# Rickyeeeeee/ParallelRayTracing

Hardware: AMD Instinct MI355X
Metric: Mrays/sec at 1920x1080, 4 bounces, ~1M-tri scene (higher is better)
Workload: dtype f32; 1 GPU; C3: dragon.ply refined by longest-edge bisection = 870000 triangles + ground quad + emissive quad, 1920x1080, max_depth 5 segments (= 4 bounces), 256 spp per step (15360 spp timed of the config's 256), image tiled over 1 GPU(s) + per-step gather to rank 0; triangles=870000, bvh_nodes=681504, bvh_max_depth=25, bvh8_nodes=137301, bvh8_depth=9, width=1920, height=1080, max_depth=5, samples_in_flight=256, seed=0, jitter=0, variant=0, gather=render stream

## Files before the change

include/prt.h:

```cpp
#ifndef PRT_H
#define PRT_H

#include <stddef.h>
#include <stdint.h>

#ifdef __cplusplus
extern "C" {
#endif

#define PRT_VERSION 1

enum {
    PRT_OK = 0,
    PRT_ERR_INVALID = 1,
    PRT_ERR_NO_DEVICE = 2,
    PRT_ERR_HIP = 3,
    PRT_ERR_IO = 4,
    PRT_ERR_NOMEM = 5
};

enum { PRT_SHAPE_CIRCLE = 0, PRT_SHAPE_QUAD = 1, PRT_SHAPE_TRIANGLE = 2 };
enum { PRT_MAT_NONE = 0, PRT_MAT_LAMBERTIAN = 1, PRT_MAT_METAL = 2, PRT_MAT_DIELECTRIC = 3, PRT_MAT_EMISSIVE = 4 };
enum {
    PRT_PRESET_DEFAULT = 0, PRT_PRESET_LIGHT_TEST = 1, PRT_PRESET_MATERIAL_TEST = 2, PRT_PRESET_CORNELL = 3,
// ... 205 lines not shown
} PrtInstanceUpdateInfo;
int prt_instance_update_info(PrtContext* ctx, PrtInstanceUpdateInfo* out);
int prt_instances_read(PrtContext* ctx, uint32_t capacity, uint32_t* n_instances, uint32_t* slot_instance, uint32_t* root,
                       uint32_t* slot_base, uint32_t* prim_base);
int prt_set_camera(PrtContext* ctx, const PrtCameraDesc* cam);
int prt_set_film(PrtContext* ctx, uint32_t width, uint32_t height, uint32_t rank, uint32_t world_size);
int prt_film_clear(PrtContext* ctx);

int prt_render(PrtContext* ctx, uint32_t spp, uint32_t max_depth, uint32_t seed, uint32_t first_sample);
int prt_render_async(PrtContext* ctx, uint32_t spp, uint32_t max_depth, uint32_t seed, uint32_t first_sample);
int prt_synchronize(PrtContext* ctx);
int prt_set_sampling(PrtContext* ctx, const PrtSampling* sampling);
int prt_set_lens(PrtContext* ctx, const PrtLens* lens);
int prt_get_lens(PrtContext* ctx, PrtLens* out);
int prt_set_samples_in_flight(PrtContext* ctx, uint32_t n);
int prt_set_lighting(PrtContext* ctx, const PrtLighting* l);
int prt_get_light_stats(PrtContext* ctx, PrtLightStats* out);
int prt_set_light_sources(PrtContext* ctx, uint32_t mask);
int prt_set_environment(PrtContext* ctx, const PrtEnvironment* env);
int prt_environment_info(PrtContext* ctx, PrtEnvironmentInfo* out);
int prt_environment_intervals(PrtContext* ctx, uint64_t* row_width, uint64_t* col_width);
int prt_environment_eval(PrtContext* ctx, uint32_t n, const float* dirs, float* rgb, uint32_t* texel, float* pdf_w);
int prt_set_textures(PrtContext* ctx, const PrtTextureSet* set);
int prt_texture_info(PrtContext* ctx, PrtTextureInfo* out);
int prt_texture_eval(PrtContext* ctx, uint32_t n, const uint32_t* texture, const float* uv, float* rgb);
int prt_hit_uv(PrtContext* ctx, uint32_t n, const float* origins, const float* dirs, PrtHit* hits, float* uv, float* albedo);
int prt_light_intervals(PrtContext* ctx, uint32_t capacity, uint32_t* n_lights, uint64_t* width);
int prt_light_info(PrtContext* ctx, uint32_t capacity, uint32_t* n_lights, uint32_t* prim, float* pmf);
int prt_sample_light(PrtContext* ctx, uint32_t n, const float* in_dirs, const PrtHit* hits, const uint32_t* keys,
                     float* shadow_dirs, float* tmax, uint32_t* light, float* contrib, float* pdf_light, float* pdf_bsdf,
                     float* w_light, float* w_bsdf);

typedef struct PrtAdaptive {
    uint32_t min_spp, step_spp, max_spp;
    float threshold, noise_floor;
} PrtAdaptive;
typedef struct PrtAdaptiveInfo {
    uint32_t passes;
    uint32_t tiles_local;
    uint32_t tiles_converged;
    uint32_t tiles_capped;
    uint32_t min_tile_spp;
    uint32_t max_tile_spp;
    uint64_t pixel_samples;
} PrtAdaptiveInfo;
int prt_set_film_statistics(PrtContext* ctx, int on);
int prt_get_film_statistics(const PrtContext* ctx);
int prt_film_statistics_read(PrtContext* ctx, float* sum_y, float* sum_y2);
int prt_film_noise_read(PrtContext* ctx, float noise_floor, float* rel_err);
int prt_adaptive_unconverged(float n, float A, float Q, float threshold, float noise_floor);
int prt_render_adaptive(PrtContext* ctx, const PrtAdaptive* cfg, uint32_t max_depth, uint32_t seed, uint32_t first_sample,
                        PrtAdaptiveInfo* out );

int prt_film_read(PrtContext* ctx, float* rgb_sum, float* weight);
int prt_film_local(PrtContext* ctx, void** d_ptr, uint64_t* n_floats);
int prt_film_resolve(PrtContext* ctx, const void* d_gathered, uint32_t world_size, void* d_rgb_sum, void* d_weight);
int prt_film_resolve_on(PrtContext* ctx, void* hip_stream, const void* d_gathered, uint32_t world_size, void* d_rgb_sum,
                        void* d_weight);
int prt_film_tonemap(PrtContext* ctx, const void* d_rgb_sum, const void* d_weight, float exposure, float gamma, void* d_rgba8);
int prt_film_display(PrtContext* ctx, float exposure, float gamma, uint8_t* rgba8);

int prt_camera_rays(PrtContext* ctx, uint32_t n, const float* px, const float* py, float* origins, float* dirs);
int prt_camera_rays_lens(PrtContext* ctx, uint32_t n, const float* px, const float* py, uint32_t* keys, float* origins,
                         float* dirs);
int prt_closest_hit(PrtContext* ctx, uint32_t n, const float* origins, const float* dirs, PrtHit* hits);
int prt_closest_hit_device(PrtContext* ctx, uint32_t n, const void* d_origins, const void* d_dirs, void* d_hits);
int prt_occluded(PrtContext* ctx, uint32_t n, const float* origins, const float* dirs, const float* tmax,
                 uint8_t* occluded);
int prt_occluded_device(PrtContext* ctx, uint32_t n, const void* d_origins, const void* d_dirs, const void* d_tmax,
                        void* d_occluded);
int prt_scatter(PrtContext* ctx, uint32_t n, const float* in_dirs, const PrtHit* hits, uint32_t* rng_state,
                uint32_t* scattered, float* attenuation, float* emitted, float* out_origins, float* out_dirs);

int prt_enable_timing(PrtContext* ctx, int on);
int prt_get_stats(PrtContext* ctx, PrtStats* out);
int prt_reset_stats(PrtContext* ctx);
int prt_measure_traversal(PrtContext* ctx, uint32_t max_depth, uint32_t seed, uint32_t sample, PrtStats* out);
int prt_measure_shade_divergence(PrtContext* ctx, uint32_t max_depth, uint32_t seed, uint32_t sample, uint64_t* out);
int prt_bvh_info(PrtContext* ctx, PrtBvhInfo* out);
uint32_t prt_spill_rows(uint32_t max_stack4, uint32_t max_depth);
int prt_kernel_occupancy(PrtContext* ctx, PrtOccupancy* out);
int prt_kernel_instance(PrtContext* ctx, char* name, uint32_t capacity);
int prt_shade_instance(PrtContext* ctx, char* name, uint32_t capacity);
int prt_bvh_read(PrtContext* ctx, float* nodes, float* tris);
int prt_bvh_read4(PrtContext* ctx, float* nodes4);
int prt_bvh_read8(PrtContext* ctx, uint32_t* nodes8);
int prt_set_variant(PrtContext* ctx, int variant);
int prt_set_param(PrtContext* ctx, const char* name, int value);

typedef struct PrtGroup PrtGroup;
int prt_group_create(const int* device_ids, uint32_t n, PrtGroup** out);
void prt_group_destroy(PrtGroup* g);
const char* prt_group_last_error(const PrtGroup* g);
uint32_t prt_group_size(const PrtGroup* g);
const char* prt_group_transport(const PrtGroup* g);
PrtContext* prt_group_context(PrtGroup* g, uint32_t rank);
int prt_group_set_scene(PrtGroup* g, const PrtSceneDesc* scene);
int prt_group_refit_meshes(PrtGroup* g, const PrtMesh* meshes, uint32_t n_meshes);
int prt_group_set_instance_transforms(PrtGroup* g, const PrtInstance* instances, uint32_t n, uint32_t mode);
int prt_group_set_camera(PrtGroup* g, const PrtCameraDesc* cam);
int prt_group_set_film(PrtGroup* g, uint32_t width, uint32_t height);
int prt_group_film_clear(PrtGroup* g);
int prt_group_set_sampling(PrtGroup* g, const PrtSampling* s);
int prt_group_set_lens(PrtGroup* g, const PrtLens* lens);
int prt_group_set_samples_in_flight(PrtGroup* g, uint32_t n);
int prt_group_set_lighting(PrtGroup* g, const PrtLighting* l);
int prt_group_set_light_sources(PrtGroup* g, uint32_t mask);
int prt_group_set_environment(PrtGroup* g, const PrtEnvironment* env);
int prt_group_set_textures(PrtGroup* g, const PrtTextureSet* set);
int prt_group_get_light_stats(PrtGroup* g, PrtLightStats* out);
int prt_group_set_param(PrtGroup* g, const char* name, int value);
int prt_group_render(PrtGroup* g, uint32_t spp, uint32_t max_depth, uint32_t seed, uint32_t first_sample);
int prt_group_set_film_statistics(PrtGroup* g, int on);
int prt_group_render_adaptive(PrtGroup* g, const PrtAdaptive* cfg, uint32_t max_depth, uint32_t seed, uint32_t first_sample,
                              PrtAdaptiveInfo* out);
int prt_group_film_read(PrtGroup* g, float* rgb_sum, float* weight);
int prt_group_film_display(PrtGroup* g, float exposure, float gamma, uint8_t* rgba8);
int prt_group_get_stats(PrtGroup* g, PrtStats* out);

typedef struct PrtMeshData PrtMeshData;
int prt_mesh_load_ply(const char* path, PrtMeshData** out, char* err, size_t err_len);
int prt_mesh_create(const float* positions, const float* normals, uint32_t n_vertices, const uint32_t* indices,
                    uint32_t n_triangles, PrtMeshData** out);
void prt_mesh_free(PrtMeshData* m);
uint32_t prt_mesh_vertex_count(const PrtMeshData* m);
uint32_t prt_mesh_triangle_count(const PrtMeshData* m);
const float* prt_mesh_positions(const PrtMeshData* m);
const float* prt_mesh_normals(const PrtMeshData* m);
const uint32_t* prt_mesh_indices(const PrtMeshData* m);
int prt_mesh_had_normals(const PrtMeshData* m);
int prt_mesh_refine(PrtMeshData* m, uint32_t target_triangles);
int prt_mesh_transform(PrtMeshData* m, const float mat[16], const float inv[16]);
int prt_mesh_append(PrtMeshData* dst, const PrtMeshData* src);
const float* prt_mesh_uvs(const PrtMeshData* m);
int prt_mesh_had_uvs(const PrtMeshData* m);
int prt_mesh_set_uvs(PrtMeshData* m, const float* uvs);

int prt_scene_preset(int preset, PrtMaterial* materials, uint32_t* n_materials, PrtPrimitive* primitives,
                     uint32_t* n_primitives);
void prt_make_transform(const float scale[3], const float euler_deg[3], const float translation[3], float mat[16],
                        float inv[16]);

int prt_write_ppm(const char* path, const uint8_t* rgba8, uint32_t width, uint32_t height);
int prt_write_pfm(const char* path, const float* rgb, uint32_t width, uint32_t height);
int prt_read_pfm(const char* path, float** rgb, uint32_t* width, uint32_t* height);
void prt_image_free(float* rgb);

#ifdef __cplusplus
}
#endif
#endif
```

parallelraytracing_amd/capi.py:

```python
from __future__ import annotations

import ctypes as C
import os

_HERE = os.path.dirname(os.path.abspath(__file__))
LIB_PATH = os.environ.get("PRT_LIB_PATH") or os.path.join(_HERE, "csrc", "libprt.so")

PRT_MAX_DEPTH = 64

SHAPE_CIRCLE, SHAPE_QUAD, SHAPE_TRIANGLE = 0, 1, 2
MAT_NONE, MAT_LAMBERTIAN, MAT_METAL, MAT_DIELECTRIC, MAT_EMISSIVE = 0, 1, 2, 3, 4
(PRESET_DEFAULT, PRESET_LIGHT_TEST, PRESET_MATERIAL_TEST, PRESET_CORNELL, PRESET_RANDOM_BALLS_SMALL,
 PRESET_RANDOM_BALLS_MEDIUM, PRESET_RANDOM_BALLS_LARGE) = range(7)
PRESET_NAMES = {
    "DEFAULT": PRESET_DEFAULT, "LIGHT_TEST": PRESET_LIGHT_TEST, "MATERIAL_TEST": PRESET_MATERIAL_TEST,
    "CORNELL": PRESET_CORNELL, "RANDOM_BALLS_SMALL": PRESET_RANDOM_BALLS_SMALL,
    "RANDOM_BALLS_MEDIUM": PRESET_RANDOM_BALLS_MEDIUM, "RANDOM_BALLS_LARGE": PRESET_RANDOM_BALLS_LARGE,
}


class PrtMaterial(C.Structure):
    _fields_ = [("type", C.c_uint32), ("rgb", C.c_float * 3), ("scalar", C.c_float)]


# ... 144 lines not shown
    "prt_group_create": (C.c_int, [C.POINTER(C.c_int), C.c_uint32, C.POINTER(_vp)]),
    "prt_group_destroy": (None, [_vp]),
    "prt_group_last_error": (C.c_char_p, [_vp]),
    "prt_group_size": (C.c_uint32, [_vp]),
    "prt_group_transport": (C.c_char_p, [_vp]),
    "prt_group_context": (_vp, [_vp, C.c_uint32]),
    "prt_group_set_scene": (C.c_int, [_vp, C.POINTER(PrtSceneDesc)]),
    "prt_group_refit_meshes": (C.c_int, [_vp, C.POINTER(PrtMesh), C.c_uint32]),
    "prt_group_set_camera": (C.c_int, [_vp, C.POINTER(PrtCameraDesc)]),
    "prt_group_set_film": (C.c_int, [_vp, C.c_uint32, C.c_uint32]),
    "prt_group_film_clear": (C.c_int, [_vp]),
    "prt_group_set_sampling": (C.c_int, [_vp, C.POINTER(PrtSampling)]),
    "prt_group_set_samples_in_flight": (C.c_int, [_vp, C.c_uint32]),
    "prt_group_set_lens": (C.c_int, [_vp, C.POINTER(PrtLens)]),
    "prt_set_lens": (C.c_int, [_vp, C.POINTER(PrtLens)]),
    "prt_get_lens": (C.c_int, [_vp, C.POINTER(PrtLens)]),
    "prt_camera_rays_lens": (C.c_int, [_vp, C.c_uint32, _fp, _fp, _u32p, _fp, _fp]),
    "prt_group_set_param": (C.c_int, [_vp, C.c_char_p, C.c_int]),
    "prt_group_render": (C.c_int, [_vp, C.c_uint32, C.c_uint32, C.c_uint32, C.c_uint32]),
    "prt_group_film_read": (C.c_int, [_vp, _fp, _fp]),
    "prt_group_film_display": (C.c_int, [_vp, C.c_float, C.c_float, C.POINTER(C.c_uint8)]),
    "prt_group_get_stats": (C.c_int, [_vp, C.POINTER(PrtStats)]),
    "prt_group_set_lighting": (C.c_int, [_vp, C.POINTER(PrtLighting)]),
    "prt_group_get_light_stats": (C.c_int, [_vp, C.POINTER(PrtLightStats)]),
    "prt_group_set_light_sources": (C.c_int, [_vp, C.c_uint32]),
    "prt_set_light_sources": (C.c_int, [_vp, C.c_uint32]),
    "prt_light_intervals": (C.c_int, [_vp, C.c_uint32, _u32p, C.POINTER(C.c_uint64)]),
    "prt_set_environment": (C.c_int, [_vp, C.POINTER(PrtEnvironment)]),
    "prt_group_set_environment": (C.c_int, [_vp, C.POINTER(PrtEnvironment)]),
    "prt_environment_info": (C.c_int, [_vp, C.POINTER(PrtEnvironmentInfo)]),
    "prt_environment_intervals": (C.c_int, [_vp, C.POINTER(C.c_uint64), C.POINTER(C.c_uint64)]),
    "prt_environment_eval": (C.c_int, [_vp, C.c_uint32, _fp, _fp, _u32p, _fp]),
    "prt_set_textures": (C.c_int, [_vp, C.POINTER(PrtTextureSet)]),
    "prt_group_set_textures": (C.c_int, [_vp, C.POINTER(PrtTextureSet)]),
    "prt_texture_info": (C.c_int, [_vp, C.POINTER(PrtTextureInfo)]),
    "prt_texture_eval": (C.c_int, [_vp, C.c_uint32, _u32p, _fp, _fp]),
    "prt_hit_uv": (C.c_int, [_vp, C.c_uint32, _fp, _fp, C.POINTER(PrtHit), _fp, _fp]),
    "prt_mesh_uvs": (_fp, [_vp]),
    "prt_mesh_had_uvs": (C.c_int, [_vp]),
    "prt_mesh_set_uvs": (C.c_int, [_vp, _fp]),
    "prt_read_pfm": (C.c_int, [C.c_char_p, C.POINTER(_fp), _u32p, _u32p]),
    "prt_image_free": (None, [_fp]),
    "prt_set_film_statistics": (C.c_int, [_vp, C.c_int]),
    "prt_get_film_statistics": (C.c_int, [_vp]),
    "prt_film_statistics_read": (C.c_int, [_vp, _fp, _fp]),
    "prt_film_noise_read": (C.c_int, [_vp, C.c_float, _fp]),
    "prt_adaptive_unconverged": (C.c_int, [C.c_float, C.c_float, C.c_float, C.c_float, C.c_float]),
    "prt_render_adaptive": (C.c_int, [_vp, C.POINTER(PrtAdaptive), C.c_uint32, C.c_uint32, C.c_uint32, C.POINTER(PrtAdaptiveInfo)]),
    "prt_group_set_film_statistics": (C.c_int, [_vp, C.c_int]),
    "prt_group_render_adaptive": (C.c_int, [_vp, C.POINTER(PrtAdaptive), C.c_uint32, C.c_uint32, C.c_uint32, C.POINTER(PrtAdaptiveInfo)]),
    "prt_set_lighting": (C.c_int, [_vp, C.POINTER(PrtLighting)]),
    "prt_get_light_stats": (C.c_int, [_vp, C.POINTER(PrtLightStats)]),
    "prt_light_info": (C.c_int, [_vp, C.c_uint32, _u32p, _u32p, _fp]),
    "prt_sample_light": (C.c_int, [_vp, C.c_uint32, _fp, C.POINTER(PrtHit), _u32p, _fp, _fp, _u32p, _fp, _fp, _fp, _fp, _fp]),
    "prt_set_scene": (C.c_int, [_vp, C.POINTER(PrtSceneDesc)]),
    "prt_set_camera": (C.c_int, [_vp, C.POINTER(PrtCameraDesc)]),
    "prt_set_film": (C.c_int, [_vp, C.c_uint32, C.c_uint32, C.c_uint32, C.c_uint32]),
    "prt_film_clear": (C.c_int, [_vp]),
    "prt_render": (C.c_int, [_vp, C.c_uint32, C.c_uint32, C.c_uint32, C.c_uint32]),
    "prt_render_async": (C.c_int, [_vp, C.c_uint32, C.c_uint32, C.c_uint32, C.c_uint32]),
    "prt_synchronize": (C.c_int, [_vp]),
    "prt_set_samples_in_flight": (C.c_int, [_vp, C.c_uint32]),
    "prt_film_read": (C.c_int, [_vp, _fp, _fp]),
    "prt_film_local": (C.c_int, [_vp, C.POINTER(_vp), C.POINTER(C.c_uint64)]),
    "prt_film_resolve": (C.c_int, [_vp, _vp, C.c_uint32, _vp, _vp]),
    "prt_film_resolve_on": (C.c_int, [_vp, _vp, _vp, C.c_uint32, _vp, _vp]),
    "prt_film_tonemap": (C.c_int, [_vp, _vp, _vp, C.c_float, C.c_float, _vp]),
    "prt_film_display": (C.c_int, [_vp, C.c_float, C.c_float, C.POINTER(C.c_uint8)]),
    "prt_camera_rays": (C.c_int, [_vp, C.c_uint32, _fp, _fp, _fp, _fp]),
    "prt_closest_hit": (C.c_int, [_vp, C.c_uint32, _fp, _fp, C.POINTER(PrtHit)]),
    "prt_closest_hit_device": (C.c_int, [_vp, C.c_uint32, _vp, _vp, _vp]),
    "prt_occluded": (C.c_int, [_vp, C.c_uint32, _fp, _fp, _fp, C.POINTER(C.c_uint8)]),
    "prt_occluded_device": (C.c_int, [_vp, C.c_uint32, _vp, _vp, _vp, _vp]),
    "prt_scatter": (C.c_int, [_vp, C.c_uint32, _fp, C.POINTER(PrtHit), _u32p, _u32p, _fp, _fp, _fp, _fp]),
    "prt_enable_timing": (C.c_int, [_vp, C.c_int]),
    "prt_get_stats": (C.c_int, [_vp, C.POINTER(PrtStats)]),
    "prt_reset_stats": (C.c_int, [_vp]),
    "prt_measure_traversal": (C.c_int, [_vp, C.c_uint32, C.c_uint32, C.c_uint32, C.POINTER(PrtStats)]),
    "prt_bvh_info": (C.c_int, [_vp, C.POINTER(PrtBvhInfo)]),
    "prt_spill_rows": (C.c_uint32, [C.c_uint32, C.c_uint32]),
    "prt_kernel_occupancy": (C.c_int, [_vp, C.POINTER(PrtOccupancy)]),
    "prt_kernel_instance": (C.c_int, [_vp, C.c_char_p, C.c_uint32]),
    "prt_shade_instance": (C.c_int, [_vp, C.c_char_p, C.c_uint32]),
    "prt_measure_shade_divergence": (C.c_int, [_vp, C.c_uint32, C.c_uint32, C.c_uint32, C.POINTER(C.c_uint64)]),
    "prt_refit_meshes": (C.c_int, [_vp, C.POINTER(PrtMesh), C.c_uint32]),
    "prt_set_instance_transforms": (C.c_int, [_vp, C.POINTER(PrtInstance), C.c_uint32, C.c_uint32]),
    "prt_group_set_instance_transforms": (C.c_int, [_vp, C.POINTER(PrtInstance), C.c_uint32, C.c_uint32]),
    "prt_instance_update_info": (C.c_int, [_vp, C.POINTER(PrtInstanceUpdateInfo)]),
    "prt_instances_read": (C.c_int, [_vp, C.c_uint32, _u32p, _u32p, _u32p, _u32p, _u32p]),
    "prt_bvh_read": (C.c_int, [_vp, _fp, _fp]),
    "prt_set_sampling": (C.c_int, [_vp, C.POINTER(PrtSampling)]),
    "prt_bvh_read4": (C.c_int, [_vp, _fp]),
    "prt_bvh_read8": (C.c_int, [_vp, C.POINTER(C.c_uint32)]),
    "prt_set_variant": (C.c_int, [_vp, C.c_int]),
    "prt_set_param": (C.c_int, [_vp, C.c_char_p, C.c_int]),
    "prt_mesh_load_ply": (C.c_int, [C.c_char_p, C.POINTER(_vp), C.c_char_p, C.c_size_t]),
    "prt_mesh_create": (C.c_int, [_fp, _fp, C.c_uint32, _u32p, C.c_uint32, C.POINTER(_vp)]),
    "prt_mesh_free": (None, [_vp]),
    "prt_mesh_vertex_count": (C.c_uint32, [_vp]),
    "prt_mesh_triangle_count": (C.c_uint32, [_vp]),
    "prt_mesh_positions": (_fp, [_vp]),
    "prt_mesh_normals": (_fp, [_vp]),
    "prt_mesh_indices": (_u32p, [_vp]),
    "prt_mesh_had_normals": (C.c_int, [_vp]),
    "prt_mesh_refine": (C.c_int, [_vp, C.c_uint32]),
    "prt_mesh_transform": (C.c_int, [_vp, _fp, _fp]),
    "prt_mesh_append": (C.c_int, [_vp, _vp]),
    "prt_scene_preset": (C.c_int, [C.c_int, C.POINTER(PrtMaterial), _u32p, C.POINTER(PrtPrimitive), _u32p]),
    "prt_make_transform": (None, [_fp, _fp, _fp, _fp, _fp]),
    "prt_write_ppm": (C.c_int, [C.c_char_p, C.POINTER(C.c_uint8), C.c_uint32, C.c_uint32]),
    "prt_write_pfm": (C.c_int, [C.c_char_p, _fp, C.c_uint32, C.c_uint32]),
}


def load(path: str = LIB_PATH) -> C.CDLL:
    if not os.path.exists(path):
        raise ImportError(
            f"{path} is missing: the HIP extension is the product and has no fallback. "
            "Build it with `python -c 'import __graft_entry__ as g; g.build()'` "
            "(or `make -C parallelraytracing_amd/csrc`).")
    try:
        import torch
    except Exception:
        pass
    lib = C.CDLL(path)
    for name, (res, args) in SIGNATURES.items():
        fn = getattr(lib, name)
        fn.restype = res
        fn.argtypes = args
    return lib


_lib = None


def lib() -> C.CDLL:
    global _lib
    if _lib is None:
        _lib = load()
    return _lib
```

parallelraytracing_amd/csrc/prt_api.cpp:

```cpp
#include <hip/hip_runtime.h>

#include <algorithm>
#include <cfloat>
#include <chrono>
#include <cmath>
#include <cstdarg>
#include <cstdio>
#include <cstdlib>
#include <cstring>
#include <limits>
#include <string>
#include <utility>
#include <vector>

#include "../../include/prt.h"
#include "bvh.h"
#include "bvh_gpu.h"
#include "prt_adaptive.h"
#include "prt_kernels.h"
#include "prt_scene.h"

namespace {

constexpr float kPadCoeff = 1.0f / 262144.0f;
constexpr size_t kRayStatWords = (size_t)PRT_RAY_STAT_SLOTS * PRT_MAX_DEPTH;
constexpr uint32_t kTravStatsWords = 16 + PRT_TIMELINE_WORDS * (PRT_MAX_DEPTH + 1);
constexpr size_t kLightStatWords = 2 * (size_t)PRT_RAY_STAT_SLOTS;

struct EventPair {
    hipEvent_t a, b;
    int kind;
};

}

struct PrtContext {
    int device = -1;
    bool has_device = false;
    hipStream_t own_stream = nullptr;
    hipStream_t stream = nullptr;
    std::string err;

    bool has_scene = false;
    PrtHostScene hs;
    double refit_ms = 0.0;
    PrtInstanceUpdateInfo inst_info{};
    DevScene dsc{};
    void* d_prims = nullptr;
    void* d_mat_rgbs = nullptr;
    void* d_mat_type = nullptr;
    void* d_nodes = nullptr;
    void* d_nodes4 = nullptr;
    void* d_nodes8 = nullptr;
    void* d_insts = nullptr;
    void* d_tlas_inst = nullptr;
    void* d_abvh_nodes = nullptr;
    void* d_abvh_order = nullptr;
    void* d_tris = nullptr;
    void* d_nrms = nullptr;

    bool has_camera = false;
    DevCamera cam{};

    bool has_film = false;
    PrtTileMap tm{};
    uint32_t valid_local = 0;
    float4* d_film_local = nullptr;
    bool film_stats = false;
    float2* d_film_stat = nullptr;
    uint32_t* d_tile_sel = nullptr;
    uint32_t tile_sel_entries = 0;
    uint32_t* h_tile_count = nullptr;

    uint32_t S = 1;
    uint64_t cap_paths = 0;
    PrtRayBuf rb[2] = {{nullptr, nullptr, nullptr, nullptr, nullptr}, {nullptr, nullptr, nullptr, nullptr, nullptr}};
    float4* d_rad = nullptr;
    uint32_t* d_counts = nullptr;
    unsigned long long* d_ray_stats = nullptr;
    unsigned long long* ray_stats_target = nullptr;
    bool pix_records_blank = false;
    uint32_t* h_flag = nullptr;
    unsigned long long* d_trav_stats = nullptr;

    void* d_scratch = nullptr;
    size_t scratch_bytes = 0;

    bool timing = false;
    std::vector<EventPair> events;
    std::vector<EventPair> event_pool;
    PrtStats stats{};
    uint64_t dead_paths = 0;
    int variant = 0;
    int abvh_enabled = 1;
    int measure_spp = 1;
    float pad_coeff = kPadCoeff;
    int node_stride = 0;
    int compact_primary = 1;
    int primary_walk = 1;
    const char* shade_instance = "";
    bool batch_walked = false;
    int gpu_build = 0;
    PrtSampling sampling{0u, 0u, 0.0f};
    PrtLens lens{0.0f, 0.0f, 0.0f};
    PrtTravTuning tune{1024u, 256u, 16u, 0xFFFFFFFFu , 0u, 2u, 0u , 0u, 0u, 0u, 1u, 8u, 1u, 0u, nullptr, 0u, 2500000u, 2u , 8u , 96u , 32u , 1u};
    unsigned long long* d_shade_div = nullptr;
    uint32_t sort_rays = 0;
    uint32_t* d_sort = nullptr;
    size_t sort_entries = 0, sort_temp = 0;
    uint32_t* h_counts = nullptr;
    hipEvent_t ev_counts[PRT_MAX_DEPTH + 2] = {};
    hipEvent_t ev_prod[PRT_MAX_DEPTH + 2] = {};
    hipStream_t count_stream = nullptr;
    uint32_t* d_work = nullptr;
    float4* d_pix = nullptr;
    uint32_t pix_entries = 0;
    uint32_t* d_spill = nullptr;
    size_t spill_entries = 0;

    uint32_t lighting = PRT_LIGHTING_OFF;
    void* d_lights = nullptr;
    void* d_prim_light = nullptr;
    uint32_t light_sources = PRT_LIGHT_SOURCES_ANALYTIC;
    int light_buckets = 1;
    void* d_ml_records = nullptr;
    void* d_ml_thr = nullptr;
    void* d_ml_bucket = nullptr;
    void* d_ml_runs = nullptr;
    PrtLightBufs lb{};
    uint64_t cap_light = 0;
    unsigned long long* d_light_stats = nullptr;

    PrtEnvTables env;
    void* d_env_texels = nullptr;
    void* d_env_row = nullptr;
    void* d_env_col = nullptr;
    void* d_env_last = nullptr;
    uint64_t t_env_dev = 0;

    PrtTexTables tex;
    void* d_tex_texels = nullptr;
    void* d_tex_desc = nullptr;
    void* d_tex_mat = nullptr;
    void* d_tex_uvs = nullptr;
    void* d_tex_inst = nullptr;
    uint64_t tex_bytes = 0;
};

namespace {

int fail(PrtContext* c, int code, const char* fmt, ...) {
    if (c) {
        char buf[512];
        va_list ap;
        va_start(ap, fmt);
        vsnprintf(buf, sizeof(buf), fmt, ap);
        va_end(ap);
        c->err = buf;
    }
    return code;
}

#define HIPCHECK(c, call)                                                                              \
    do {                                                                                               \
        hipError_t e_ = (call);                                                                        \
        if (e_ != hipSuccess) return fail((c), PRT_ERR_HIP, "%s failed: %s", #call, hipGetErrorString(e_)); \
    } while (0)

int need_device(PrtContext* c) {
    if (!c) return PRT_ERR_INVALID;
    if (!c->has_device)
        return fail(c, PRT_ERR_NO_DEVICE,
                    "no HIP device bound to this context: the MI355X kernels are the only compute path (no CPU fallback)");
    const hipError_t e = hipSetDevice(c->device);
    if (e != hipSuccess) return fail(c, PRT_ERR_HIP, "hipSetDevice(%d) failed: %s", c->device, hipGetErrorString(e));
    return PRT_OK;
}

void free_dev(void*& p) {
    if (p) {
        (void)hipFree(p);
        p = nullptr;
    }
}
template <class T>
void free_dev(T*& p) {
    if (p) {
        (void)hipFree((void*)p);
        p = nullptr;
// ... 227 lines not shown
    HIPCHECK(c, hipMalloc(&c->d_scratch, bytes));
    c->scratch_bytes = bytes;
    return PRT_OK;
}

void free_scene(PrtContext* c) {
    free_dev(c->d_prims);
    free_dev(c->d_mat_rgbs);
    free_dev(c->d_mat_type);
    free_dev(c->d_nodes);
    free_dev(c->d_nodes4);
    free_dev(c->d_nodes8);
    free_dev(c->d_insts);
    free_dev(c->d_tlas_inst);
    free_dev(c->d_abvh_nodes);
    free_dev(c->d_abvh_order);
    free_dev(c->d_tris);
    free_dev(c->d_nrms);
    free_dev(c->d_lights);
    free_dev(c->d_prim_light);
    free_mesh_lights(c);
    c->has_scene = false;
}

int read_ray_stats(PrtContext* c, const unsigned long long* d_set, unsigned long long (&out)[PRT_MAX_DEPTH]) {
    std::vector<unsigned long long> h(kRayStatWords);
    HIPCHECK(c, hipMemcpy(h.data(), d_set, kRayStatWords * sizeof(unsigned long long), hipMemcpyDeviceToHost));
    for (int d = 0; d < PRT_MAX_DEPTH; ++d) {
        out[d] = 0;
        for (size_t sl = 0; sl < PRT_RAY_STAT_SLOTS; ++sl) out[d] += h[sl * PRT_MAX_DEPTH + (size_t)d];
    }
    return PRT_OK;
}

int begin_event(PrtContext* c, int kind, EventPair* ep) {
    if (!c->timing) return PRT_OK;
    if (!c->event_pool.empty()) {
        *ep = c->event_pool.back();
        c->event_pool.pop_back();
    } else {
        HIPCHECK(c, hipEventCreate(&ep->a));
        HIPCHECK(c, hipEventCreate(&ep->b));
    }
    ep->kind = kind;
    HIPCHECK(c, hipEventRecord(ep->a, c->stream));
    return PRT_OK;
}
int end_event(PrtContext* c, EventPair* ep) {
    if (!c->timing) return PRT_OK;
    HIPCHECK(c, hipEventRecord(ep->b, c->stream));
    c->events.push_back(*ep);
    return PRT_OK;
}
int drain_events(PrtContext* c) {
    for (EventPair& ep : c->events) {
        float ms = 0.0f;
        HIPCHECK(c, hipEventSynchronize(ep.b));
        HIPCHECK(c, hipEventElapsedTime(&ms, ep.a, ep.b));
        switch (ep.kind) {
            case 0: c->stats.raygen_ms += ms; break;
            case 1: c->stats.intersect_ms += ms; break;
            case 2: c->stats.shade_ms += ms; break;
            case 4: c->stats.scan_ms += ms; break;
            default: c->stats.accumulate_ms += ms; break;
        }
        c->event_pool.push_back(ep);
    }
    c->events.clear();
    return PRT_OK;
}

float lens_tan_fov_y(const PrtLens& l) { return l.fov_y == 0.0f ? tanf(0.5f) : tanf(0.5f * l.fov_y); }

f3 h_normalize(f3 v) {
    const float d = (v.x * v.x + v.y * v.y) + v.z * v.z;
    const float s = 1.0f / std::sqrt(d);
    return f3{v.x * s, v.y * s, v.z * s};
}
f3 h_cross(f3 a, f3 b) { return f3{a.y * b.z - b.y * a.z, a.z * b.x - b.z * a.x, a.x * b.y - b.x * a.y}; }

PrtBatchView whole_film(const PrtContext* c) { return PrtBatchView{c->tm, nullptr}; }

void walk_rays(PrtContext* c, const PrtRayBuf& rays, const uint32_t* count, uint32_t max_rays, bool any, const PrtTravTuning& tune,
               unsigned long long* stats, const PrtPrimary* primary) {
    if (!prt_route_walk8(c->variant == 0, c->dsc.n_insts != 0u, c->dsc.nodes != nullptr))
        prt_launch_intersect(c->stream, c->dsc, rays, count, max_rays, c->hs.bvh.max_depth <= 31 ? 31 : 63, c->variant, stats);
    else if (any)
        prt_launch_occluded(c->stream, c->dsc, rays, count, c->d_work, c->d_spill, max_rays, c->hs.bvh.max_depth, c->hs.bvh.max_stack4, tune);
    else
        prt_launch_traverse(c->stream, c->dsc, rays, count, c->d_work, c->d_spill, max_rays, c->hs.bvh.max_depth, c->hs.bvh.max_stack4,
                            tune, stats, primary);
}

int sort_front_rays(PrtContext* c, const PrtRayBuf& in, const uint32_t* front_count, uint32_t n_paths, EventPair* ep, PrtTravTuning* tune) {
    int rc;
    uint32_t n_front = 0;
    HIPCHECK(c, hipMemcpyAsync(&n_front, front_count, sizeof(uint32_t), hipMemcpyDeviceToHost, c->stream));
    HIPCHECK(c, hipStreamSynchronize(c->stream));
    if (n_front <= 1u) return PRT_OK;
    if (c->sort_entries < n_paths) {
        free_dev(c->d_sort);
        c->sort_entries = 0;
        c->sort_temp = prt_sort_rays_temp_bytes(n_paths);
        HIPCHECK(c, hipMalloc((void**)&c->d_sort, 4 * (size_t)n_paths * sizeof(uint32_t) + c->sort_temp));
        c->sort_entries = n_paths;
    }
    EventPair es{};
    if ((rc = begin_event(c, 4, &es))) return rc;
    uint32_t* q = c->d_sort;
    if (prt_sort_rays(c->stream, in.o, in.d, n_front, c->dsc.root_min, c->dsc.root_max, c->sort_rays, q, q + n_paths,
                      q + 2 * (size_t)n_paths, q + 3 * (size_t)n_paths, q + 4 * (size_t)n_paths, c->sort_temp))
        return fail(c, PRT_ERR_HIP, "ray sort failed");
    if ((rc = end_event(c, &es))) return rc;
    if (c->timing) HIPCHECK(c, hipEventRecord(ep->a, c->stream));
    tune->perm = q + 3 * (size_t)n_paths;
    return PRT_OK;
}

int run_batch(PrtContext* c, const PrtBatchView& view, uint32_t S_cur, uint32_t max_depth, uint32_t seed, uint32_t first_sample,
              bool accumulate, unsigned long long* trav_stats) {
    const PrtTileMap& tm = view.tm;
    if (view.list && !c->d_film_stat) return fail(c, PRT_ERR_INVALID, "a tile list needs film statistics");
    const uint64_t n_paths64 = (uint64_t)S_cur * tm.n_pix_local;
    c->batch_walked = false;
    if (n_paths64 == 0) return PRT_OK;
    if (n_paths64 > 0xFFFFFF00ull) return fail(c, PRT_ERR_INVALID, "too many paths in flight");
    const uint32_t n_paths = (uint32_t)n_paths64;
    int rc = ensure_path_state(c, n_paths);
    if (rc) return rc;
    if ((rc = ensure_spill(c))) return rc;
    if ((rc = sync_light_tables(c))) return rc;
    PrtRouteFacts f{};
    f.lit = c->lighting != PRT_LIGHTING_OFF;
    f.mesh_lights = mesh_lights_on(c);
    f.env = env_on(c);
    f.tex = tex_on(c);
    f.lens = c->lens.aperture > 0.0f;
    f.listed = view.list != nullptr;
    f.film_stats = c->film_stats;
    f.has_nodes = c->dsc.n_nodes != 0u;
    f.has_bvh2 = c->dsc.nodes != nullptr;
    f.insts = c->dsc.n_insts != 0u;
    f.abvh = c->dsc.abvh_nodes != nullptr;
    f.few_prims = c->dsc.n_prims <= 16u;
    f.jitter = c->sampling.jitter != 0u;
    f.sa = c->sampling.rr_depth != 0u || c->sampling.clamp > 0.0f;
    f.multi_sample = S_cur > 1u;
    f.variant0 = c->variant == 0;
    f.compact_primary = c->compact_primary;
    f.primary_walk = c->primary_walk;
    f.takes_primary = prt_traverse_takes_primary(c->dsc, c->tune);
    f.primary_hit = c->tune.primary_hit != 0u;
    f.path_gate = !trav_stats && !c->d_shade_div && c->sort_rays == 0u && n_paths <= c->tune.path_max && prt_path_kernel_applies(c->dsc, c->tune);
    f.path_kernel = c->tune.path_kernel;
    f.fuse = c->tune.fuse;
    const PrtRoutePlan plan = prt_plan_route(f);
    const bool lit = f.lit, compact = plan.compact, walk = plan.walk;
    const DevEnv denv = dev_env(c);
    const DevTex dtex = dev_tex(c);
    const DevLens dlens{c->lens.aperture, c->lens.focus_distance};
    const bool exact = c->dsc.n_nodes != 0u && c->tune.exact_grids != 0u && (n_paths > (16384u * 512u) || c->tune.exact_grids == 2u);
    if (exact && !c->h_counts) {
        HIPCHECK(c, hipHostMalloc((void**)&c->h_counts, (PRT_MAX_DEPTH + 2) * 64 * sizeof(uint32_t), hipHostMallocDefault));
        for (hipEvent_t& e : c->ev_counts) HIPCHECK(c, hipEventCreateWithFlags(&e, hipEventDisableTiming));
        for (hipEvent_t& e : c->ev_prod) HIPCHECK(c, hipEventCreateWithFlags(&e, hipEventDisableTiming));
        HIPCHECK(c, hipStreamCreateWithFlags(&c->count_stream, hipStreamNonBlocking));
    }
    auto read_back = [&](uint32_t d) -> hipError_t {
        hipError_t e = hipEventRecord(c->ev_prod[d], c->stream);
        if (e == hipSuccess) e = hipStreamWaitEvent(c->count_stream, c->ev_prod[d], 0);
        if (e == hipSuccess)
            e = hipMemcpyAsync(c->h_counts + 64 * (size_t)d, c->d_counts + (size_t)d * PRT_CNT_STRIDE, 33 * sizeof(uint32_t),
                               hipMemcpyDeviceToHost, c->count_stream);
        return e != hipSuccess ? e : hipEventRecord(c->ev_counts[d], c->count_stream);
    };
    EventPair ep{};
    auto accumulate_batch = [&]() -> int {
        if ((rc = begin_event(c, 3, &ep))) return rc;
        const PrtAccumulateArgs aa{c->d_rad, lit ? c->lb.lrad : nullptr, c->d_film_local, c->d_film_stat, tm, S_cur, max_depth,
                                   accumulate, c->ray_stats_target, compact ? c->d_pix + tm.n_pix_local : nullptr, view.list};
        if (!prt_launch_accumulate(c->stream, plan.accumulate, aa)) return fail(c, PRT_ERR_INVALID, "no such accumulate instance");
        if ((rc = end_event(c, &ep))) return rc;
        if (accumulate && !view.list) c->stats.samples += S_cur;
        HIPCHECK(c, hipGetLastError());
        return PRT_OK;
    };
    c->shade_instance = "";
    if (plan.path) {
        HIPCHECK(c, hipMemsetAsync(c->d_work, 0, 256 * sizeof(uint32_t), c->stream));
        PrtPathArgs pa{c->cam, tm, c->sampling, c->d_rad, first_sample, seed, max_depth, n_paths};
        if ((rc = begin_event(c, 1, &ep))) return rc;
        prt_launch_path(c->stream, c->dsc, pa, c->d_work, c->tune);
        if ((rc = end_event(c, &ep))) return rc;
        ++c->stats.intersect_launches;
        return accumulate_batch();
    }
    HIPCHECK(c, hipMemsetAsync(c->d_counts, 0, (size_t)(max_depth + 1) * PRT_CNT_STRIDE * sizeof(uint32_t), c->stream));
    if (compact && c->pix_entries < tm.n_pix_local) {
        free_dev(c->d_pix);
        c->pix_entries = 0;
        HIPCHECK(c, hipMalloc((void**)&c->d_pix, 4 * (size_t)tm.n_pix_local * sizeof(float4)));
        c->pix_entries = tm.n_pix_local;
        c->pix_records_blank = false;
    }
    const DevLights lt = dev_lights(c);
    const DevMeshLights mlt = dev_mesh_lights(c);
    if (lit) {
        if ((rc = ensure_light_state(c, n_paths))) return rc;
        HIPCHECK(c, hipMemsetAsync(c->lb.lrad, 0, (size_t)n_paths * sizeof(float4), c->stream));
    }
    c->batch_walked = walk;
    const PrtPrimary primary{(const uint32_t*)c->rb[0].t, c->d_pix, {c->cam.pos.x, c->cam.pos.y, c->cam.pos.z}, tm.n_pix_local,
                             1.0f / (float)tm.n_pix_local, first_sample, seed, walk ? 1u : 0u};
    PrtPrimary primary_list = primary;
    if (walk) primary_list.pid = (const uint32_t*)c->rb[0].hd2;
    if ((rc = begin_event(c, 0, &ep))) return rc;
    const PrtRaygenArgs ra{&c->dsc, c->cam, tm, n_paths, first_sample, seed, max_depth, c->rb[0], c->d_rad, c->d_counts, c->d_work, c->sampling,
                           compact ? c->d_pix : nullptr, walk, f.env ? &denv : nullptr, f.lens ? &dlens : nullptr, view.list};
    if (!prt_launch_raygen(c->stream, plan.raygen, ra)) return fail(c, PRT_ERR_INVALID, "no such raygen instance");
    if ((rc = end_event(c, &ep))) return rc;
    if (exact) HIPCHECK(c, read_back(0));
    for (uint32_t d = 0; d < max_depth; ++d) {
        const PrtRayBuf& in = c->rb[d & 1];
        const PrtRayBuf& out = c->rb[(d + 1) & 1];
        const uint32_t* front_count = c->d_counts + (size_t)d * PRT_CNT_STRIDE;
        const PrtPrimary* prim_d = (compact && d == 0) ? &primary : nullptr;
        if (c->dsc.n_nodes) {
            if ((rc = begin_event(c, 1, &ep))) return rc;
            PrtTravTuning tune = c->tune;
            tune.probe_slot = d;
            tune.perm = nullptr;
            if (plan.walk8 && c->sort_rays && !prim_d && (d > 0 || c->sampling.jitter || f.lens))
                if ((rc = sort_front_rays(c, in, front_count, n_paths, &ep, &tune))) return rc;
            if (walk && d == 0)
                walk_rays(c, in, c->d_counts + PRT_CNT_LIST, tm.n_pix_local, false, tune, trav_stats, &primary_list);
            else
                walk_rays(c, in, front_count, n_paths, false, tune, trav_stats, prim_d);
            if ((rc = end_event(c, &ep))) return rc;
            ++c->stats.intersect_launches;
            if (prim_d) {
                if (plan.primary_hit) {
                    if ((rc = begin_event(c, 2, &ep))) return rc;
                    prt_launch_primary_hit(c->stream, c->dsc, primary, in.hit, c->d_pix, c->d_counts);
                    if ((rc = end_event(c, &ep))) return rc;
                    c->pix_records_blank = false;
                } else if (!c->pix_records_blank) {
                    HIPCHECK(c, hipMemsetAsync(c->d_pix + 2 * (size_t)tm.n_pix_local, 0xFF, 2 * (size_t)tm.n_pix_local * sizeof(float4), c->stream));
                    c->pix_records_blank = true;
                }
            }
        }
        uint32_t n_rays_known = 0xFFFFFFFFu;
        if (exact) {
            HIPCHECK(c, hipEventSynchronize(c->ev_counts[d]));
            n_rays_known = c->h_counts[64 * (size_t)d] + c->h_counts[64 * (size_t)d + 32];
            if (n_rays_known == 0u) break;
        }
        if (c->d_shade_div) prt_launch_shade_divstats(c->stream, c->dsc, in, c->d_counts, d, n_paths, c->d_shade_div, prim_d);
        if ((rc = begin_event(c, 2, &ep))) return rc;
        const PrtShadeInst shade = d == 0 ? plan.shade0 : plan.shade;
        const PrtShadeArgs sa{&c->dsc, in, out, c->d_rad, c->d_counts, c->d_work, d, max_depth, n_paths, c->sampling, n_rays_known, prim_d,
                              f.env ? &denv : nullptr, f.tex ? &dtex : nullptr, lit ? &lt : nullptr, (lit && f.mesh_lights) ? &mlt : nullptr,
                              lit ? &c->lb : nullptr};
        if (!prt_launch_shade(c->stream, shade, sa)) return fail(c, PRT_ERR_INVALID, "no such shade instance");
        c->shade_instance = prt_shade_name(shade);
        if (lit && (lt.n_lights || (f.env && (denv.t_all | denv.t_env)))) {
            const uint32_t* scount = c->d_counts + (size_t)d * PRT_CNT_STRIDE + 48u;
            const uint32_t nmax = n_rays_known == 0xFFFFFFFFu ? n_paths : n_rays_known;
            prt_launch_scan_prims_bounded(c->stream, c->dsc, c->lb.sh, scount, c->d_work, nmax);
            if (c->dsc.n_nodes) walk_rays(c, c->lb.sh, scount, nmax, true, c->tune, nullptr, nullptr);
            prt_launch_light_accum(c->stream, c->dsc, c->lb, scount, c->d_work, nmax);
        }
        if ((rc = end_event(c, &ep))) return rc;
        if (exact && d + 1 < max_depth) HIPCHECK(c, read_back(d + 1));
    }
    return accumulate_batch();
}

void fill_dev_scene(PrtContext* c, uint32_t node_stride, uint32_t depth8) {
    const PrtSceneScalars& k = c->hs.sc;
    DevScene d{};
    d.prims = (const DevPrim*)c->d_prims;
    d.mat_rgbs = (const float4*)c->d_mat_rgbs;
    d.mat_type = (const uint32_t*)c->d_mat_type;
    d.nodes = (const float4*)c->d_nodes;
    d.nodes4 = (const float4*)c->d_nodes4;
    d.nodes8 = (const uint4*)c->d_nodes8;
    d.tris = (const float4*)c->d_tris;
    d.tri_normals = (const float4*)c->d_nrms;
    d.abvh_nodes = (const float4*)c->d_abvh_nodes;
    d.abvh_order = (const uint32_t*)c->d_abvh_order;
    d.insts = (const DevInstance*)c->d_insts;
    d.tlas_inst = (const uint32_t*)c->d_tlas_inst;
    d.n_insts = k.n_insts;
    d.node_stride = node_stride;
    d.depth8 = depth8;
    d.n_prims = k.n_prims;
    d.n_nodes = k.n_nodes;
    d.n_tris = k.n_tris;
    d.pad = k.pad;
    memcpy(d.abvh_q, k.abvh_q, sizeof(d.abvh_q));
    d.extent = k.extent;
    memcpy(d.root_min, k.root_min, sizeof(d.root_min));
    memcpy(d.root_max, k.root_max, sizeof(d.root_max));
    memcpy(d.sky, k.sky, sizeof(d.sky));
    c->dsc = d;
}

int upload_scene(PrtContext* c, PrtGpuBvh* gb) {
    HIPCHECK(c, hipSetDevice(c->device));
    HIPCHECK(c, hipStreamSynchronize(c->stream));
    free_scene(c);
    if (gb) {
        c->d_nodes8 = gb->d_nodes8;
        c->d_tris = gb->d_tris;
        c->d_nrms = gb->d_nrms;
    }
    const std::vector<uint32_t>& n8 = c->hs.nodes8_all.empty() ? c->hs.bvh.nodes8 : c->hs.nodes8_all;
    const size_t n_nodes8 = gb ? (size_t)gb->n_nodes : n8.size() / 20;
    const uint32_t node_stride = c->node_stride ? (uint32_t)c->node_stride : (n_nodes8 * 80 > ((size_t)64 << 20) ? 8u : 5u);
    if (node_stride == 8u && n_nodes8) {
        void* wide = nullptr;
        HIPCHECK(c, hipMalloc(&wide, 128 * n_nodes8));
        hipError_t e = hipMemset(wide, 0, 128 * n_nodes8);
        if (e == hipSuccess)
            e = gb ? hipMemcpy2D(wide, 128, c->d_nodes8, 80, 80, n_nodes8, hipMemcpyDeviceToDevice)
                   : hipMemcpy2D(wide, 128, n8.data(), 80, 80, n_nodes8, hipMemcpyHostToDevice);
        if (e == hipSuccess) e = hipDeviceSynchronize();
        if (e != hipSuccess) {
            (void)hipFree(wide);
            HIPCHECK(c, e);
        }
        free_dev(c->d_nodes8);
        c->d_nodes8 = wide;
    }
    auto upload = [&](void** dst, const void* src, size_t bytes) -> hipError_t {
        hipError_t e = hipMalloc(dst, std::max<size_t>(bytes, 16));
        if (e != hipSuccess) return e;
        if (bytes) e = hipMemcpy(*dst, src, bytes, hipMemcpyHostToDevice);
        return e;
    };
    std::vector<float> rgbs(4 * c->hs.materials.size());
    std::vector<uint32_t> mtype(c->hs.materials.size());
    for (size_t i = 0; i < c->hs.materials.size(); ++i) {
// ... 1454 lines not shown
    memset(out, 0, sizeof(*out));
    uint64_t front = 0;
    for (uint32_t d = 0; d < max_depth; ++d) {
        front += cnt[(size_t)d * PRT_CNT_STRIDE + ((d == 0 && c->batch_walked) ? PRT_CNT_LIST : 0u)];
        out->rays_per_depth[d] = after[d] - before[d];
        out->rays_total += out->rays_per_depth[d];
    }
    out->rays_traversed = front;
    out->samples = (uint64_t)std::max(1, c->measure_spp);
    out->bvh_node_visits = t[0];
    out->bvh_tri_tests = t[1];
    out->prim_tests = (uint64_t)c->hs.prims.size() * out->rays_total;
    out->node_lane_slots = t[3];
    out->tri_lane_slots = t[4];
    out->max_stack_used = t[5];
    out->wave_cycles_refill = t[6];
    out->wave_cycles_node = t[7];
    out->wave_cycles_tri = t[8];
    return PRT_OK;
}

int prt_measure_shade_divergence(PrtContext* c, uint32_t max_depth, uint32_t seed, uint32_t sample, uint64_t* out) {
    int rc = check_ready(c);
    if (rc) return rc;
    if (!out || max_depth == 0 || max_depth > PRT_MAX_DEPTH) return PRT_ERR_INVALID;
    HIPCHECK(c, hipStreamSynchronize(c->stream));
    const size_t bytes = 16 * (size_t)PRT_MAX_DEPTH * sizeof(unsigned long long);
    unsigned long long* buf = nullptr;
    HIPCHECK(c, hipMalloc((void**)&buf, bytes));
    hipError_t e = hipMemsetAsync(buf, 0, bytes, c->stream);
    if (e == hipSuccess) {
        c->d_shade_div = buf;
        c->ray_stats_target = c->d_ray_stats + kRayStatWords;
        const bool timing = c->timing;
        const uint64_t launches = c->stats.intersect_launches;
        c->timing = false;
        rc = run_batch(c, whole_film(c), (uint32_t)std::max(1, c->measure_spp), max_depth, seed, sample, false, nullptr);
        c->timing = timing;
        c->stats.intersect_launches = launches;
        c->d_shade_div = nullptr;
        c->ray_stats_target = c->d_ray_stats;
        if (!rc) e = hipStreamSynchronize(c->stream);
        if (!rc && e == hipSuccess) e = hipMemcpy(out, buf, 16 * (size_t)max_depth * sizeof(unsigned long long), hipMemcpyDeviceToHost);
    }
    (void)hipFree(buf);
    if (rc) return rc;
    HIPCHECK(c, e);
    return PRT_OK;
}

int prt_kernel_occupancy(PrtContext* c, PrtOccupancy* out) {
    int rc = need_device(c);
    if (rc) return rc;
    if (!out) return PRT_ERR_INVALID;
    if (!c->has_scene) return fail(c, PRT_ERR_INVALID, "prt_set_scene has not been called");
    int nb = 0, vg = 0, sg = 0, lds = 0;
    if (prt_traverse_occupancy(c->dsc, c->tune, &nb, &vg, &sg, &lds)) return fail(c, PRT_ERR_HIP, "occupancy query failed");
    hipDeviceProp_t prop;
    HIPCHECK(c, hipGetDeviceProperties(&prop, c->device));
    out->blocks_per_cu = (uint32_t)nb;
    out->waves_per_cu = (uint32_t)nb * 4u;
    out->max_waves_per_cu = (uint32_t)(prop.maxThreadsPerMultiProcessor / 64);
    out->vgprs = (uint32_t)vg;
    out->lds_bytes_per_block = (uint32_t)lds;
    out->compute_units = (uint32_t)prop.multiProcessorCount;
    out->resident_grid_blocks = !strcmp(prt_traverse_instance(c->dsc, c->tune), "lean8_5waves")
                                    ? c->tune.grid_blocks + c->tune.grid_blocks / 4u : c->tune.grid_blocks;
    return PRT_OK;
}

int prt_kernel_instance(PrtContext* c, char* name, uint32_t capacity) {
    if (!c || !name || capacity == 0u) return PRT_ERR_INVALID;
    if (!c->has_scene) return fail(c, PRT_ERR_INVALID, "prt_set_scene has not been called");
    snprintf(name, capacity, "%s", prt_traverse_instance(c->dsc, c->tune));
    return PRT_OK;
}

int prt_shade_instance(PrtContext* c, char* name, uint32_t capacity) {
    if (!c || !name || capacity == 0u) return PRT_ERR_INVALID;
    snprintf(name, capacity, "%s", c->shade_instance);
    return PRT_OK;
}

int prt_bvh_info(PrtContext* c, PrtBvhInfo* out) {
    if (!c || !out) return PRT_ERR_INVALID;
    if (!c->has_scene) return fail(c, PRT_ERR_INVALID, "prt_set_scene has not been called");
    *out = c->hs.bvh_info;
    return PRT_OK;
}

int prt_bvh_read4(PrtContext* c, float* nodes4) {
    if (!c) return PRT_ERR_INVALID;
    if (!c->has_scene) return fail(c, PRT_ERR_INVALID, "prt_set_scene has not been called");
    if (nodes4) memcpy(nodes4, c->hs.bvh.nodes4.data(), c->hs.bvh.nodes4.size() * 4);
    return PRT_OK;
}

int prt_bvh_read8(PrtContext* c, uint32_t* nodes8) {
    if (!c) return PRT_ERR_INVALID;
    if (!c->has_scene) return fail(c, PRT_ERR_INVALID, "prt_set_scene has not been called");
    const std::vector<uint32_t>& n8 = c->hs.nodes8_all.empty() ? c->hs.bvh.nodes8 : c->hs.nodes8_all;
    if (nodes8) memcpy(nodes8, n8.data(), n8.size() * 4);
    return PRT_OK;
}

int prt_bvh_read(PrtContext* c, float* nodes, float* tris) {
    if (!c) return PRT_ERR_INVALID;
    if (!c->has_scene) return fail(c, PRT_ERR_INVALID, "prt_set_scene has not been called");
    if (nodes) memcpy(nodes, c->hs.bvh.nodes.data(), c->hs.bvh.nodes.size() * 4);
    if (tris) memcpy(tris, c->hs.tri_records.data(), c->hs.tri_records.size() * 4);
    return PRT_OK;
}

int prt_set_param(PrtContext* c, const char* name, int value) {
    if (!c || !name) return PRT_ERR_INVALID;
    const std::string n = name;
    if (n == "variant") c->variant = value;
    else if (n == "grid_blocks" && value > 0 && value <= 8192) c->tune.grid_blocks = (uint32_t)value;
    else if (n == "chunk" && value >= 64 && value % 64 == 0) c->tune.chunk = (uint32_t)value;
    else if (n == "xcd_affinity" && (value == 0 || value == 1)) c->tune.xcd_affinity = (uint32_t)value;
    else if (n == "wide" && (value == 0 || value == 1 || value == 2)) c->tune.wide = (uint32_t)value;
    else if (n == "stack_lds" && (value == 0 || value == 1 || value == 2 || value == 3 || value == 4 || value == 5 || value == 6 || value == 24 || value == 39)) c->tune.stack_lds = (uint32_t)value;
    else if (n == "exact_grids" && (value == 0 || value == 1 || value == 2)) c->tune.exact_grids = (uint32_t)value;
    else if (n == "steal" && value >= 0 && value <= 64) c->tune.steal = (uint32_t)value;
    else if (n == "primary_hit" && (value == 0 || value == 1)) c->tune.primary_hit = (uint32_t)value;
    else if (n == "path_kernel" && value >= 0 && value <= 2) c->tune.path_kernel = (uint32_t)value;
    else if (n == "path_max" && value >= 1) c->tune.path_max = (uint32_t)value;
    else if (n == "sort_rays" && value >= 0 && value <= 2) c->sort_rays = (uint32_t)value;
    else if (n == "compact_primary" && (value == 0 || value == 1)) c->compact_primary = value;
    else if (n == "primary_walk" && (value == 0 || value == 1)) c->primary_walk = value;
    else if (n == "node_stride" && (value == 0 || value == 5 || value == 8)) c->node_stride = value;
    else if (n == "pad_log2" && value >= 8 && value <= 22) c->pad_coeff = std::ldexp(1.0f, -value);
    else if (n == "tail" && value >= 0 && value <= 64) c->tune.tail = (uint32_t)value;
    else if (n == "big" && value >= 1 && value <= 16) c->tune.big = (uint32_t)value;
    else if (n == "static_small" && value >= 0 && value <= 4096) c->tune.static_small = (uint32_t)value;
    else if (n == "big_min" && value >= 1 && value <= 100000) c->tune.big_min = (uint32_t)value;
    else if (n == "big_keep" && value >= 0 && value <= 1024) c->tune.big_keep = (uint32_t)value;
    else if (n == "stack_cap" && value >= 0 && value <= 64) c->tune.stack_cap = (uint32_t)value;
    else if (n == "prim_bvh" && (value == 0 || value == 1)) c->abvh_enabled = value;
    else if (n == "measure_spp" && value >= 1 && value <= 1024) c->measure_spp = value;
    else if (n == "gpu_build" && (value == 0 || value == 1 || value == 2)) c->gpu_build = value;
    else if (n == "fuse" && (value == 0 || value == 1)) c->tune.fuse = (uint32_t)value;
    else if (n == "tri_min" && value >= 0 && value <= 1024) c->tune.tri_min = (uint32_t)value;
    else if (n == "refill_min" && value >= 1 && value <= 64) c->tune.refill_min = (uint32_t)value;
    else if (n == "light_buckets" && (value == 0 || value == 1)) c->light_buckets = value;
    else if (n == "exit_max" && value >= 0 && value < 64) c->tune.exit_max = (uint32_t)value;
    else return fail(c, PRT_ERR_INVALID, "unknown parameter or bad value: %s = %d", name, value);
    return PRT_OK;
}

int prt_set_variant(PrtContext* c, int variant) {
    if (!c) return PRT_ERR_INVALID;
    c->variant = variant;
    return PRT_OK;
}

}
```

parallelraytracing_amd/csrc/prt_kernels.h:

```cpp
#pragma once
#include <hip/hip_runtime_api.h>
#include <hip/hip_vector_types.h>
#include <stdint.h>

#include "../../include/prt.h"
#include "prt_route.h"
#include "prt_scene_pod.h"

struct f3 {
    float x, y, z;
};

struct DevCamera {
    f3 pos, front, right, up;
    float W, H, tan_fov_y;
};
struct DevLens {
    float aperture, focus;
};

#define PRT_DIR_MIN 9.094947017729282e-13f

struct DevScene {
    const DevPrim* prims;
// ... 83 lines not shown
    DevCamera cam;
    PrtTileMap tm;
    PrtSampling sp;
    float4* rad;
    uint32_t first_sample, seed, max_depth, n_paths;
};

#define PRT_CNT_STRIDE 64u
#define PRT_CNT_LIST 8u

struct DevLights {
    const float4* lights;
    const uint32_t* prim_light;
    uint32_t n_lights;
    uint32_t mode;
};
struct DevLightRun {
    uint32_t prim_first, n_tris, light_first, world;
};
struct DevMeshLights {
    const uint32_t* thr;
    const uint32_t* bucket;
    const DevLightRun* runs;
    uint32_t bucket_shift;
    uint32_t n_runs;
};
struct DevEnv {
    const float4* texels;
    const uint32_t* row_thr;
    const uint32_t* col_thr;
    const uint32_t* col_last;
    uint32_t W, H;
    uint32_t row_last;
    uint32_t t_env;
    uint32_t t_all;
    float p_env;
};

struct DevTex {
    const float4* texels;
    const uint4* desc;
    const uint32_t* mat_tex;
    const float2* uvs;
    const uint32_t* inst_uv_base;
    uint32_t n_textures;
};

struct PrtLightBufs {
    PrtRayBuf sh;
    float* pdf_b;
    float4* lrad;
    unsigned long long* stats;
};

struct PrtRaygenArgs {
    const DevScene* sc;
    DevCamera cam;
    PrtTileMap tm;
    uint32_t n_paths, first_sample, seed, max_depth;
    PrtRayBuf out;
    float4* rad;
    uint32_t* counts;
    uint32_t* work;
    PrtSampling sp;
    float4* compact_pix;
    bool primary_walk;
    const DevEnv* env;
    const DevLens* lens;
    const uint32_t* list;
};
bool prt_launch_raygen(hipStream_t st, PrtRaygenInst inst, const PrtRaygenArgs& a);
void prt_launch_scan_prims(hipStream_t st, const DevScene& sc, const PrtRayBuf& in, const uint32_t* count_ptr,
                           uint32_t* work, uint32_t max_rays, unsigned long long* stats);
void prt_launch_traverse(hipStream_t st, const DevScene& sc, const PrtRayBuf& in, const uint32_t* count_ptr,
                         uint32_t* work, uint32_t* spill, uint32_t max_rays, uint32_t tree_depth, uint32_t stack4,
                         const PrtTravTuning& tune, unsigned long long* stats, const PrtPrimary* primary = nullptr);
void prt_launch_path(hipStream_t st, const DevScene& sc, const PrtPathArgs& pa, uint32_t* work, const PrtTravTuning& tune);
bool prt_path_kernel_applies(const DevScene& sc, const PrtTravTuning& tune);
bool prt_traverse_takes_primary(const DevScene& sc, const PrtTravTuning& tune);
int prt_traverse_occupancy(const DevScene& sc, const PrtTravTuning& tune, int* blocks_per_cu, int* vgprs, int* sgprs, int* lds_bytes);
const char* prt_traverse_instance(const DevScene& sc, const PrtTravTuning& tune);
void prt_launch_intersect(hipStream_t st, const DevScene& sc, const PrtRayBuf& in, const uint32_t* count_ptr,
                          uint32_t max_rays, int stack_depth, int variant, unsigned long long* stats);
struct PrtShadeArgs {
    const DevScene* sc;
    PrtRayBuf in, out;
    float4* rad;
    uint32_t* counts;
    uint32_t* work;
    uint32_t depth, max_depth, cap;
    PrtSampling sp;
    uint32_t n_rays_known;
    const PrtPrimary* primary;
    const DevEnv* env;
    const DevTex* tex;
    const DevLights* lights;
    const DevMeshLights* mesh_lights;
    const PrtLightBufs* lb;
};
bool prt_launch_shade(hipStream_t st, PrtShadeInst inst, const PrtShadeArgs& a);
void prt_launch_shade_divstats(hipStream_t st, const DevScene& sc, const PrtRayBuf& in, const uint32_t* counts, uint32_t iter,
                               uint32_t cap, unsigned long long* out, const PrtPrimary* primary = nullptr);
void prt_launch_primary_hit(hipStream_t st, const DevScene& sc, const PrtPrimary& pr, const uint32_t* hit, float4* pix,
                            const uint32_t* counts);
struct PrtAccumulateArgs {
    const float4* rad;
    const float4* lrad;
    float4* film_local;
    float2* stat;
    PrtTileMap tm;
    uint32_t S, max_depth;
    bool update_film;
    unsigned long long* ray_stats;
    const float4* pix_end;
    const uint32_t* list;
};
bool prt_launch_accumulate(hipStream_t st, PrtAccumulateInst inst, const PrtAccumulateArgs& a);
void prt_launch_resolve(hipStream_t st, const float4* gathered, uint32_t world, uint32_t stride, uint32_t W,
                        uint32_t H, float* rgb, float* weight);
void prt_launch_tonemap(hipStream_t st, const float* rgb, const float* weight, uint32_t n_pix, float exposure,
                        float inv_gamma, uint8_t* out);
void prt_launch_camera_rays(hipStream_t st, const DevCamera& cam, uint32_t n, const float* px, const float* py,
                            float* o, float* d);
void prt_launch_camera_rays_lens(hipStream_t st, const DevCamera& cam, const DevLens& lens, uint32_t n, const float* px,
                                 const float* py, uint32_t* keys, float* o, float* d);
void prt_launch_pack_rays(hipStream_t st, uint32_t n, const float* o, const float* d, const PrtRayBuf& out,
                          uint32_t* counts);
void prt_launch_hit_records(hipStream_t st, const DevScene& sc, uint32_t n, const PrtRayBuf& in, PrtHit* out);
void prt_launch_pack_occlusion_rays(hipStream_t st, uint32_t n, const float* o, const float* d, const float* tmax,
                                    const PrtRayBuf& out, uint32_t* counts);
void prt_launch_scan_prims_bounded(hipStream_t st, const DevScene& sc, const PrtRayBuf& in, const uint32_t* count_ptr,
                                   uint32_t* work, uint32_t max_rays);
void prt_launch_occluded(hipStream_t st, const DevScene& sc, const PrtRayBuf& in, const uint32_t* count_ptr, uint32_t* work,
                         uint32_t* spill, uint32_t max_rays, uint32_t tree_depth, uint32_t stack4, const PrtTravTuning& tune);
void prt_launch_occlusion_bytes(hipStream_t st, const DevScene& sc, uint32_t n, const PrtRayBuf& in, const float* tmax,
                                uint8_t* out);
void prt_launch_scatter_test(hipStream_t st, const DevScene& sc, uint32_t n, const float* in_d, const PrtHit* hits,
                             uint32_t* rng_io, uint32_t* scattered, float* atten, float* emitted, float* o_out,
                             float* d_out);
void prt_launch_light_accum(hipStream_t st, const DevScene& sc, const PrtLightBufs& lb, const uint32_t* count_ptr,
                            uint32_t* work, uint32_t max_rays);
void prt_launch_sample_light_test(hipStream_t st, const DevScene& sc, const DevLights& lt, uint32_t n, const float* in_d,
                                  const PrtHit* hits, const uint32_t* keys, float* out_f, uint32_t* out_light,
                                  const DevMeshLights* ml = nullptr, const DevEnv* env = nullptr);
void prt_launch_environment_eval(hipStream_t st, const DevEnv& env, uint32_t n, const float* dirs, float* rgb, uint32_t* texel,
                                 float* pdf_w);
void prt_launch_texture_eval(hipStream_t st, const DevTex& tex, uint32_t n, const uint32_t* texture, const float* uv, float* rgb);
void prt_launch_hit_uv(hipStream_t st, const DevScene& sc, const DevTex& tex, uint32_t n, const PrtRayBuf& in, float* uv, float* albedo);

void prt_launch_tile_select(hipStream_t st, const float4* film_local, const float2* stat, const PrtTileMap& tm, const uint32_t* prev,
                            uint32_t n_in, float threshold, float noise_floor, uint32_t* flags, uint32_t* out, uint32_t* count);
```

parallelraytracing_amd/csrc/prt_kernels.hip:

```cpp
#include "prt_kernels.h"

#include "prt_adaptive.h"
#include "prt_device.h"

#define HIT_MISS 0xFFFFFFFFu
#define HIT_DEAD 0xFFFFFFFEu

PRT_DEV uint32_t xcd_remap(uint32_t b, uint32_t n) {
    const uint32_t q = n >> 3, r = n & 7u;
    const uint32_t xcd = b & 7u, i = b >> 3;
    const uint32_t start = xcd < r ? xcd * (q + 1u) : r * (q + 1u) + (xcd - r) * q;
    return start + i;
}

#define CNT_STRIDE PRT_CNT_STRIDE
#define CNT_A(c, d) (c)[(d) * CNT_STRIDE]
#define CNT_B(c, d) (c)[(d) * CNT_STRIDE + 32u]
#define CNT_C(c, d) (c)[(d) * CNT_STRIDE + 16u]
#define PRODUCER_BLOCK 1024
#ifndef SHADE_BLOCK
#define SHADE_BLOCK 512
#endif

template <int BLOCK>
// ... 66 lines not shown
        for (uint32_t w = 0; w < BLOCK / 64; ++w) {
            ta += s_a[w];
            tb += s_b[w];
        }
        s_base_a = ta ? atomicAdd(cntA, ta) : 0u;
        s_base_b = tb ? atomicAdd(cntB, tb) : 0u;
    }
    __syncthreads();
    uint32_t wa = s_base_a, wb = s_base_b;
    for (uint32_t w = 0; w < wave; ++w) {
        wa += s_a[w];
        wb += s_b[w];
    }
#pragma unroll
    for (int k = 0; k < K; ++k) slot[k] = front[k] ? wa + ja[k] : back[k] ? cap - 1u - (wb + jb[k]) : 0xFFFFFFFFu;
}

PRT_DEV bool tile_pixel(const PrtTileMap& tm, uint32_t pl, uint32_t& x, uint32_t& y) {
    const uint32_t lt = pl >> 6, lane = pl & 63u;
    const uint32_t gt = lt * tm.world + tm.rank;
    const uint32_t tx = gt % tm.tiles_x, ty = gt / tm.tiles_x;
    x = tx * 8u + (lane & 7u);
    y = ty * 8u + (lane >> 3);
    return gt < tm.tiles_x * tm.tiles_y && x < tm.W && y < tm.H;
}

PRT_DEV void primary_ray(const PrtPrimary& pr, uint32_t i, f3& o, f3& d, uint32_t& pixel, uint32_t& sample, uint32_t* local_pixel = nullptr) {
    uint32_t q = (uint32_t)((float)i * pr.inv_n);
    uint32_t r = i - q * pr.n_pix_local;
    if ((int32_t)r < 0) {
        --q;
        r += pr.n_pix_local;
    }
    if (r >= pr.n_pix_local) {
        ++q;
        r -= pr.n_pix_local;
    }
    sample = q;
    if (local_pixel) *local_pixel = r;
    const float4 P = pr.pix[r];
    o = mk3(pr.origin[0], pr.origin[1], pr.origin[2]);
    d = mk3(P.x, P.y, P.z);
    pixel = __float_as_uint(P.w);
}

template <bool ABVH, int BLOCK>
__device__ bool classify_ray(const DevScene& sc, f3 o, f3 d, uint32_t& id0, float& d2_0);
__device__ bool ends_here(const DevScene& sc, bool front, uint32_t id0, f3 thr, f3& L);

PRT_DEV float4 path_result(f3 L, float clamp, uint32_t depth) {
    if (clamp > 0.0f) {
        L.x = L.x > clamp ? clamp : L.x;
        L.y = L.y > clamp ? clamp : L.y;
        L.z = L.z > clamp ? clamp : L.z;
    }
    return make_float4(L.x, L.y, L.z, __uint_as_float(depth));
}

#define PRT_ENV_INV_TWO_PI 0.159154943091895336f
#define PRT_ENV_INV_PI 0.318309886183790672f
PRT_DEV uint32_t env_texel(const DevEnv& env, f3 d) {
    const float x = __builtin_fmaf(atan2f(d.z, d.x), PRT_ENV_INV_TWO_PI, 0.5f) * (float)env.W;
    float cy = d.y < -1.0f ? -1.0f : d.y;
    cy = cy > 1.0f ? 1.0f : cy;
    const float y = (acosf(cy) * PRT_ENV_INV_PI) * (float)env.H;
    uint32_t j = x > 0.0f ? (uint32_t)x : 0u;
    uint32_t i = y > 0.0f ? (uint32_t)y : 0u;
    j = j < env.W - 1u ? j : env.W - 1u;
    i = i < env.H - 1u ? i : env.H - 1u;
    return i * env.W + j;
}
PRT_DEV f3 env_radiance(const DevEnv& env, f3 d, float& pdf_w) {
    const float4 t = env.texels[env_texel(env, d)];
    const float s2 = (1.0f - d.y) * (1.0f + d.y);
    const float sin_t = __builtin_sqrtf(s2 > 0.0f ? s2 : 0.0f);
    pdf_w = sin_t > 0.0f ? t.w / sin_t : 0.0f;
    return mk3(t.x, t.y, t.z);
}
PRT_DEV f3 env_radiance(const DevEnv& env, f3 d) {
    const float4 t = env.texels[env_texel(env, d)];
    return mk3(t.x, t.y, t.z);
}

template <int BUDGET, bool INST, bool ABVH, int BLOCK, bool PRE = false, bool ENV = false, bool TEX = false>
PRT_DEV int advance_path(const DevScene& sc, uint32_t id, f3& o, f3& d, f3& thr, uint32_t& rng, uint32_t& depth,
                         uint32_t max_depth, const PrtSampling& sp, float4* __restrict__ rad_slot, uint32_t& id0,
                         float& d2_0, float4 pre_a = float4{0.f, 0.f, 0.f, 0.f}, float4 pre_b = float4{0.f, 0.f, 0.f, 0.f},
                         const DevEnv* env = nullptr, const DevTex* tex = nullptr) {
#pragma unroll
    for (int it = 0; it <= BUDGET; ++it) {
        if (id == HIT_MISS) {
            st_stream(rad_slot, path_result(thr * (ENV ? env_radiance(*env, d) : mk3(sc.sky[0], sc.sky[1], sc.sky[2])), sp.clamp, depth));
            return 0;
        }
        if (it == BUDGET) {
            const uint32_t m = sc.prims[id].material;
            if (sc.mat_type[m] == 4u) {
                const float4 e = sc.mat_rgbs[m];
                st_stream(rad_slot, path_result(thr * mk3(e.x, e.y, e.z), sp.clamp, depth));
                return 0;
            }
            id0 = id;
            return 2;
        }
        WorldHit w;
        float uv[2] = {0.0f, 0.0f};
        if (PRE && it == 0 && __float_as_uint(pre_a.w) == id) {
            w.pos = mk3(pre_a.x, pre_a.y, pre_a.z);
            w.normal = mk3(pre_b.x, pre_b.y, pre_b.z);
            w.material = __float_as_uint(pre_b.w) & 0x7FFFFFFFu;
            w.front = (__float_as_uint(pre_b.w) >> 31) != 0u;
        } else if (TEX) {
            world_hit_from_id<INST, true>(sc, id, o, d, w, tex, uv);
        } else {
            world_hit_from_id<INST>(sc, id, o, d, w);
        }
        const uint32_t type = sc.mat_type[w.material];
        const float4 rgbs = TEX ? textured_rgbs(sc, *tex, w.material, uv) : sc.mat_rgbs[w.material];
        f3 atten, emitted, so, sd;
        bool scattered = false;
        if (depth + 1u >= max_depth) {
            emitted = (type == 4u) ? mk3(rgbs.x, rgbs.y, rgbs.z) : mk3(0.f, 0.f, 0.f);
        } else {
            scattered = material_scatter(type, rgbs, d, w.pos, w.normal, w.front, rng, atten, emitted, so, sd);
        }
        if (!scattered) {
            st_stream(rad_slot, path_result(thr * emitted, sp.clamp, depth));
            return 0;
        }
        thr = thr * atten;
        o = so;
        d = normalize3(sd);
        if (sp.rr_depth != 0u && depth + 1u >= sp.rr_depth) {
            float p = thr.x > thr.y ? thr.x : thr.y;
            p = p > thr.z ? p : thr.z;
            p = p > 1.0f ? 1.0f : p;
            p = p < 0.05f ? 0.05f : p;
            if (!(rnd01(rng) < p)) {
                st_stream(rad_slot, path_result(mk3(0.f, 0.f, 0.f), 0.0f, depth));
                return 0;
            }
            thr = mk3(thr.x / p, thr.y / p, thr.z / p);
        }
        ++depth;
        if (classify_ray<ABVH, BLOCK>(sc, o, d, id0, d2_0)) return 1;
        id = id0;
    }
    return 2;
}

#define RAYGEN_GROUP 8
#ifndef RAYGEN_ALLOC
#define RAYGEN_ALLOC 4
#endif
#define RAYGEN_GROUP_NOJITTER 64u
template <bool JITTER, bool SAMPLING, bool ABVH, bool COMPACT, bool ENV, bool LENS = false, bool LIST = false>
PRT_DEV void raygen_step(DevScene sc, DevCamera cam, PrtTileMap tm, uint32_t S, uint32_t first_sample, uint32_t seed,
                         float4* __restrict__ ro, float4* __restrict__ rd, float4* __restrict__ rt, uint32_t* __restrict__ hit,
                         float* __restrict__ hd2, float4* __restrict__ rad, uint32_t* __restrict__ counts,
                         uint32_t* __restrict__ work, uint32_t max_depth, PrtSampling sp_arg, float4* __restrict__ pix,
                         const DevEnv* env, const DevLens* lens = nullptr, const uint32_t* __restrict__ list = nullptr) {
    const PrtSampling sp = SAMPLING ? sp_arg : PrtSampling{0u, 0u, 0.0f};
    const uint32_t pl = blockIdx.x * (uint32_t)PRODUCER_BLOCK + threadIdx.x;
    if (blockIdx.y == 0 && pl < 8u) work[32u * pl] = 0u;
    if (blockIdx.y == 0 && pl == 8u) work[512] = 0u;
    const uint32_t n_paths = S * tm.n_pix_local;
    const bool in_range = pl < tm.n_pix_local;
    bool valid = false, front0 = false;
    f3 o0 = mk3(0.f, 0.f, 0.f), d0 = mk3(0.f, 0.f, 1.f);
    uint32_t id00 = HIT_MISS, pixel = 0, px = 0, py = 0;
    float d2_00 = 3.402823466e+38f;
    if (in_range) {
        valid = tile_pixel(tm, LIST ? (list[pl >> 6] << 6) | (pl & 63u) : pl, px, py);
        if (valid) {
            pixel = py * tm.W + px;
            if (!JITTER && !LENS) {
                camera_ray(cam, (float)px + 0.5f, (float)py + 0.5f, o0, d0);
                if (COMPACT && blockIdx.y == 0) pix[pl] = make_float4(d0.x, d0.y, d0.z, __uint_as_float(pixel));
                front0 = classify_ray<ABVH, PRODUCER_BLOCK>(sc, o0, d0, id00, d2_00);
            }
        }
    }
    const uint32_t group = (JITTER || LENS) ? RAYGEN_GROUP : RAYGEN_GROUP_NOJITTER;
    const uint32_t s0 = blockIdx.y * group;
    const uint32_t s1 = (s0 + group < S) ? s0 + group : S;
    if (!JITTER && !LENS) {
        f3 o = o0, d = d0, thr = mk3(1.f, 1.f, 1.f);
        uint32_t rng = 0, depth = 0, id0 = id00;
        float d2_0 = d2_00;
        float4 L0 = make_float4(0.f, 0.f, 0.f, __uint_as_float(0xFFFFFFFFu));
        bool front = false, back = false;
        if (valid) {
            front = front0;
            if (!front) {
                const int r = advance_path<0, false, ABVH, PRODUCER_BLOCK, false, ENV>(sc, id00, o, d, thr, rng, depth, max_depth, sp, &L0, id0, d2_0,
                                                                                         float4{0.f, 0.f, 0.f, 0.f}, float4{0.f, 0.f, 0.f, 0.f}, env);
                back = r == 2;
            }
        }
        uint32_t stride = 0, base = 0;
        const uint32_t slot0 = block_alloc2<PRODUCER_BLOCK>(front, back, false, &CNT_A(counts, 0), &CNT_B(counts, 0),
                                                            &CNT_C(counts, 0), n_paths, s1 - s0, &stride, &base);
        uint32_t first_slot = slot0;
        const bool walk = COMPACT && hd2 != nullptr;
        uint32_t list_slot = 0xFFFFFFFFu;
        if (walk && blockIdx.y == 0) {
            __shared__ uint32_t s_list_base;
            if (front && slot0 == base) s_list_base = atomicAdd(&counts[PRT_CNT_LIST], stride);
            __syncthreads();
            if (front) {
                list_slot = s_list_base + (slot0 - base);
                ((uint32_t*)hd2)[list_slot] = pl;
            }
        }
        if (s1 - s0 < 8u) {
            if (in_range && slot0 != 0xFFFFFFFFu) {
                for (uint32_t sl = s0; sl < s1; ++sl) {
                    const uint32_t i = sl * tm.n_pix_local + pl;
                    const uint32_t slot = front ? slot0 + (sl - s0) * stride : slot0 - (sl - s0) * stride;
                    if (COMPACT) {
                        ((uint32_t*)rt)[slot] = i;
                    } else {
                        ro[slot] = make_float4(o.x, o.y, o.z, __uint_as_float(i));
                        rd[slot] = make_float4(d.x, d.y, d.z, __uint_as_float(path_seed(pixel, first_sample + sl, seed)));
                        rt[slot] = make_float4(1.f, 1.f, 1.f, __uint_as_float(0u));
                    }
                    if (!COMPACT) {
                        hit[slot] = id0;
// ... 1103 lines not shown
                    if (cand && ((volatile unsigned long long*)s_key)[wbase + owner] == key) s_slot[wbase + owner] = slot;
                    __builtin_amdgcn_fence(__ATOMIC_SEQ_CST, "wavefront");
                }
                const unsigned long long won = ((volatile unsigned long long*)s_key)[my];
                if (won != key_best) {
                    best.d2 = __uint_as_float((uint32_t)(won >> 32));
                    best.prim = (uint32_t)won;
                    best.id = sc.n_prims + ((volatile uint32_t*)s_slot)[my];
                    tlimit = limit_from_d2(best.d2, pad);
                }
                leaf = LEAF_NONE;
                if (second) node = (st.sp > 0) ? st.pop() : NODE_DONE;
                if (node < 0) {
                    leaf = node;
                    node = (st.sp > 0) ? st.pop() : NODE_DONE;
                }
            }
        }
    }
    if (STATS) {
        atomicAdd(&stats[0], (unsigned long long)n_nodes);
        atomicAdd(&stats[1], (unsigned long long)n_tris);
        __syncthreads();
        if (threadIdx.x < 4) atomicAdd(&stats[3], 64ull * s_iters[threadIdx.x]);
        if (threadIdx.x < 4) atomicAdd(&stats[4], 64ull * s_iters[4 + threadIdx.x]);
        atomicMax(&stats[5], (unsigned long long)max_sp);
    }
}

#define T8_QCAP 256u
#define T8_QGROUPS 128u

#ifndef PRT_T8_BFI
#define PRT_T8_BFI 1
#endif
#if PRT_T8_BFI
#define T8_SEL(M, A, B) (((A) & (M)) | ((B) & ~(M)))
#else
#define T8_SEL(M, A, B) ((M) ? (A) : (B))
#endif
#define T8_CHILD(J, NX, FX, NY, FY, NZ, FZ)                                                                          \
    {                                                                                                                \
        const float tnx = __builtin_fmaf((float)(((NX) >> (8 * J)) & 0xFFu), Ax, Bnx);                               \
        const float tny = __builtin_fmaf((float)(((NY) >> (8 * J)) & 0xFFu), Ay, Bny);                               \
        const float tnz = __builtin_fmaf((float)(((NZ) >> (8 * J)) & 0xFFu), Az, Bnz);                               \
        const float tfx = __builtin_fmaf((float)(((FX) >> (8 * J)) & 0xFFu), Ax, Bfx);                               \
        const float tfy = __builtin_fmaf((float)(((FY) >> (8 * J)) & 0xFFu), Ay, Bfy);                               \
        const float tfz = __builtin_fmaf((float)(((FZ) >> (8 * J)) & 0xFFu), Az, Bfz);                               \
        const float tn = __builtin_fmaxf(__builtin_fmaxf(tnx, tny), __builtin_fmaxf(tnz, 0.0f));                     \
        const float tf = __builtin_fminf(__builtin_fminf(tfx, tfy), __builtin_fminf(tfz, tlimit));                   \
        const uint32_t cb = ((bits4 >> (8 * J)) & 0xFFu) << ((idx4 >> (8 * J)) & 0xFFu);                             \
        hitmask |= (tn <= tf) ? cb : 0u;                                                                             \
    }
#define T8_HALF(META4, NX, FX, NY, FY, NZ, FZ)                                                                       \
    {                                                                                                                \
        const uint32_t meta4 = (META4);                                                                              \
        const uint32_t in4 = ((meta4 & (meta4 << 1)) & 0x10101010u) >> 4;   \
        const uint32_t idx4 = (meta4 ^ (octinv4 & ((in4 << 3) - in4))) & 0x1F1F1F1Fu;                                \
        const uint32_t bits4 = (meta4 >> 5) & 0x07070707u;                                                           \
        T8_CHILD(0, NX, FX, NY, FY, NZ, FZ)                                                                          \
        T8_CHILD(1, NX, FX, NY, FY, NZ, FZ)                                                                          \
        T8_CHILD(2, NX, FX, NY, FY, NZ, FZ)                                                                          \
        T8_CHILD(3, NX, FX, NY, FY, NZ, FZ)                                                                          \
    }
#define T8_BOXTEST()                                                                                                 \
    const uint32_t eim = w0.w;                                                                                       \
    const float Ax = __uint_as_float((eim & 0xFFu) << 23) * ix;                                                      \
    const float Ay = __uint_as_float(((eim >> 8) & 0xFFu) << 23) * iy;                                               \
    const float Az = __uint_as_float(((eim >> 16) & 0xFFu) << 23) * iz;                                              \
    const float px = __uint_as_float(w0.x), py = __uint_as_float(w0.y), pz = __uint_as_float(w0.z);                  \
    const float Bnx = __builtin_fmaf(px, ix, -anx), Bny = __builtin_fmaf(py, iy, -any), Bnz = __builtin_fmaf(pz, iz, -anz); \
    const float Bfx = __builtin_fmaf(px, ix, -afx), Bfy = __builtin_fmaf(py, iy, -afy), Bfz = __builtin_fmaf(pz, iz, -afz); \
    uint32_t mx = (uint32_t)((int32_t)__float_as_uint(ix) >> 31), my = (uint32_t)((int32_t)__float_as_uint(iy) >> 31), \
             mz = (uint32_t)((int32_t)__float_as_uint(iz) >> 31);                                                    \
    asm("" : "+v"(mx), "+v"(my), "+v"(mz));   \
    const uint32_t nxa = T8_SEL(mx, w3.z, w2.x), nxb = T8_SEL(mx, w3.w, w2.y), fxa = T8_SEL(mx, w2.x, w3.z), fxb = T8_SEL(mx, w2.y, w3.w); \
    const uint32_t nya = T8_SEL(my, w4.x, w2.z), nyb = T8_SEL(my, w4.y, w2.w), fya = T8_SEL(my, w2.z, w4.x), fyb = T8_SEL(my, w2.w, w4.y); \
    const uint32_t nza = T8_SEL(mz, w4.z, w3.x), nzb = T8_SEL(mz, w4.w, w3.y), fza = T8_SEL(mz, w3.x, w4.z), fzb = T8_SEL(mz, w3.y, w4.w); \
    uint32_t hitmask = 0u;                                                                                           \
    T8_HALF(w1.z, nxa, fxa, nya, fya, nza, fza)                                                                      \
    T8_HALF(w1.w, nxb, fxb, nyb, fyb, nzb, fzb)

#define T8_SENTINEL 0xFFFFFFFFu
template <int STACK_L, int WAVES, bool STATS, bool INST, bool LEAN, bool PRIM, bool PATH, bool ANY>
__device__ __forceinline__ void traverse8_body(DevScene sc, const float4* __restrict__ ro, const float4* __restrict__ rd,
                                               uint32_t* __restrict__ hit, const float* __restrict__ hd2,
                                               const uint32_t* __restrict__ count_ptr, uint32_t* __restrict__ work,
                                               uint32_t* __restrict__ ovf, PrtTravTuning tune,
                                               unsigned long long* __restrict__ stats, PrtPrimary pr, PrtPathArgs pa) {
    __shared__ uint2 s_stack[(STACK_L + 1) * 256];
    __shared__ unsigned long long s_key[256];
    __shared__ uint32_t s_slot[256];
    __shared__ uint32_t s_queue[4 * T8_QCAP];
    __shared__ uint32_t s_qn[8];
    __shared__ uint32_t s_iters[8];
    __shared__ float s_wray[INST ? 6 * 256 : 1];
    __shared__ float s_lray[LEAN ? 6 * 256 : 1];
    constexpr bool STEAL = LEAN && !INST;
    static_assert(!PATH || (!LEAN && !INST && !PRIM && !STATS), "the path instance is the plain one-level kernel");
    static_assert(!ANY || (!PATH && !PRIM && !STATS), "the any-hit walk reads plain ray buffers");
    const uint32_t count = PATH ? pa.n_paths : *count_ptr;
    f3 pd = mk3(0.f, 0.f, 1.f), pthr = mk3(0.f, 0.f, 0.f);
    uint32_t prng = 0u, pdepth = 0u;
    bool need_shade = false;
    const int stack_cap = (tune.stack_cap != 0u && tune.stack_cap < (uint32_t)STACK_L) ? (int)tune.stack_cap : STACK_L;
    const uint32_t gran_per_chunk = tune.chunk >> 6;
    const uint32_t n_wv = gridDim.x * 4u;
    const uint32_t n_gran = (count + 63u) >> 6;
    const uint32_t tail_want = (n_gran < n_wv * 8u || n_gran < n_wv * tune.static_small) ? n_gran : n_wv * tune.tail;
    const uint32_t n_bulk = (n_gran - (tail_want < n_gran ? tail_want : n_gran)) / gran_per_chunk;
    const uint32_t big = (tune.big > 1u && n_gran >= n_wv * tune.big_min) ? tune.big : 1u;
    const uint32_t mid_keep = n_wv * tune.big_keep / gran_per_chunk;
    const uint32_t n_big = big > 1u ? (n_bulk - (mid_keep < n_bulk ? mid_keep : n_bulk)) / big : 0u;
    const uint32_t n_grabs = n_big + (n_bulk - n_big * big) + (n_gran - n_bulk * gran_per_chunk);
    bool first_grab = true;
    uint32_t my_grabs = 0u;
    const bool static_small = n_gran < n_wv * tune.static_small;
    const uint32_t my_xcd = xcc_id();
    const uint32_t tid = threadIdx.x;
    const uint32_t lane = lane_id();
    const uint32_t wv = tid >> 6;
    const uint32_t wbase = tid & ~63u;
    if (tid < 8) {
        s_iters[tid] = 0;
        s_qn[tid] = 0u;
    }
    __syncthreads();
    uint32_t* const queue = &s_queue[wv * T8_QCAP];
    uint32_t k = 0xFFFFFFFFu;
    f3 o = mk3(0.f, 0.f, 0.f), ld = mk3(0.f, 0.f, 1.f);
    float ix = 1.f, iy = 1.f, iz = 1.f, anx = 0.f, any = 0.f, anz = 0.f, afx = 0.f, afy = 0.f, afz = 0.f, pad = 0.f, tlimit = 0.f;
    uint32_t octinv4 = 0x07070707u;
    uint32_t gx = 0u, gy = 0u;
    bool pending = false;
    bool in_blas = false, stall = false;
    uint32_t inst = 0u, ipb = 0u, ipm = 0u;
    float lscale = 1.0f, padw4 = 0.0f;
    int sp = 0;
    bool overflow = false;
    Closest best;
    best.d2 = 3.402823466e+38f;
    best.id = HIT_MISS;
    best.prim = 0xFFFFFFFFu;
    uint32_t n_nodes = 0, n_tris = 0, max_sp = 0;
    uint32_t cur = 0, cur_end = 0;
    bool exhausted = false;
    const uint32_t tri_min = tune.tri_min < T8_QGROUPS - 64u ? tune.tri_min : T8_QGROUPS - 64u;
    unsigned long long cyc_refill = 0, cyc_node = 0, cyc_tri = 0, t_mark = STATS ? __builtin_amdgcn_s_memtime() : 0ull;
    const unsigned long long t_start = STATS ? __builtin_amdgcn_s_memrealtime() : 0ull;
    unsigned long long t_exh = 0ull;
    uint32_t ray_steps = 0u, ray_steps_max = 0u;
    for (uint32_t guard = 0;; ++guard) {
        if (guard > (1u << 22)) {
            if (lane == 0) atomicOr(work + 256, 1u);
            break;
        }
        unsigned long long helped = 0ull;
        if (STEAL && exhausted) {
            const bool helper = k >= 0xFFFFFF00u && k != 0xFFFFFFFFu;
            if (__ballot(helper) != 0ull) {
                const uint32_t r = k & 63u;
                const uint32_t lo = wave_scan_or((helper && r < 32u) ? 1u << r : 0u);
                const uint32_t hi = wave_scan_or((helper && r >= 32u) ? 1u << (r - 32u) : 0u);
                helped = ((unsigned long long)(uint32_t)__builtin_amdgcn_readlane((int)hi, 63) << 32) |
                         (uint32_t)__builtin_amdgcn_readlane((int)lo, 63);
            }
        }
        if (k != 0xFFFFFFFFu && !pending && !(INST && (in_blas || ipm != 0u))) {
            if (overflow) {
                if (PATH) {
                    atomicOr(work + 256, 2u);
                    need_shade = true;
                } else if (INST) {
                    atomicOr(work + 256, 2u);
                } else {
                    const uint32_t j = atomicAdd(ovf, 1u);
                    if (j < PRT_OVF_CAP)
                        ovf[1u + j] = k;
                    else
                        atomicOr(work + 256, 2u);
                }
                overflow = false;
                if (!PATH) k = 0xFFFFFFFFu;
// ... 170 lines not shown
                int r = 0;
                uint32_t id = HIT_MISS, id0 = HIT_MISS;
                float d2_0 = 3.402823466e+38f;
                if (fresh) {
                    const uint32_t smp = k / pa.tm.n_pix_local, pl = k - smp * pa.tm.n_pix_local;
                    uint32_t px, py;
                    if (!tile_pixel(pa.tm, pl, px, py)) {
                        pa.rad[k] = make_float4(0.f, 0.f, 0.f, __uint_as_float(0xFFFFFFFFu));
                    } else {
                        prng = path_seed(py * pa.tm.W + px, pa.first_sample + smp, pa.seed);
                        float fx = (float)px + 0.5f, fy = (float)py + 0.5f;
                        if (pa.sp.jitter) {
                            const float u1 = rnd01(prng);
                            const float u2 = rnd01(prng);
                            fx = (float)px + u1;
                            fy = (float)py + u2;
                        }
                        camera_ray(pa.cam, fx, fy, o, pd);
                        pthr = mk3(1.f, 1.f, 1.f);
                        pdepth = 0u;
                        r = classify_ray<false, 256>(sc, o, pd, id0, d2_0) ? 1 : 2;
                        id = id0;
                    }
                }
                if (need_shade) {
                    r = 2;
                    id = best.id;
                    need_shade = false;
                }
                while (r == 2) {
                    r = advance_path<1, false, false, 256>(sc, id, o, pd, pthr, prng, pdepth, pa.max_depth, pa.sp, &pa.rad[k], id0, d2_0);
                    id = id0;
                }
                if (r == 1) {
                    ld = normalize3(pd);
                    pad = sc.pad * (__builtin_fabsf(o.x) + __builtin_fabsf(o.y) + __builtin_fabsf(o.z) + sc.extent);
                    ix = __builtin_amdgcn_rcpf(__builtin_fabsf(ld.x) < PRT_DIR_MIN ? __builtin_copysignf(PRT_DIR_MIN, ld.x) : ld.x);
                    iy = __builtin_amdgcn_rcpf(__builtin_fabsf(ld.y) < PRT_DIR_MIN ? __builtin_copysignf(PRT_DIR_MIN, ld.y) : ld.y);
                    iz = __builtin_amdgcn_rcpf(__builtin_fabsf(ld.z) < PRT_DIR_MIN ? __builtin_copysignf(PRT_DIR_MIN, ld.z) : ld.z);
                    const bool nx = ix < 0.0f, ny = iy < 0.0f, nz = iz < 0.0f;
                    anx = (nx ? o.x - pad : o.x + pad) * ix; afx = (nx ? o.x + pad : o.x - pad) * ix;
                    any = (ny ? o.y - pad : o.y + pad) * iy; afy = (ny ? o.y + pad : o.y - pad) * iy;
                    anz = (nz ? o.z - pad : o.z + pad) * iz; afz = (nz ? o.z + pad : o.z - pad) * iz;
                    octinv4 = (7u - ((nx ? 1u : 0u) | (ny ? 2u : 0u) | (nz ? 4u : 0u))) * 0x01010101u;
                    best.id = id0;
                    best.prim = id0;
                    best.d2 = d2_0;
                    tlimit = limit_from_d2(best.d2, pad);
                    gx = 0u;
                    gy = 1u << (24u + (octinv4 & 7u));
                    sp = 0;
                } else if ((fresh || ((shade_m >> lane) & 1ull)) && r == 0) {
                    k = 0xFFFFFFFFu;
                }
            }
        }
        if (!PATH && !exhausted && (n_idle >= tune.refill_min || (INST && do_sw && n_idle != 0u))) {
            if (cur == cur_end) {
                uint32_t c = blockIdx.x * 4u + wv;
                if (!first_grab) {
                    if (n_grabs <= n_wv) c = n_grabs;
                    else if (static_small) c += my_grabs * n_wv;
                    else if (lane == 0) c = atomicAdd(work, 1u) + n_wv;
                    c = (uint32_t)__shfl((int)c, 0, 64);
                }
                first_grab = false;
                ++my_grabs;
                if (c >= n_grabs) {
                    exhausted = true;
                    if (STATS) t_exh = __builtin_amdgcn_s_memrealtime();
                } else {
                    const uint32_t cb = c - n_big + n_big * big;
                    const uint32_t g0 = c < n_big ? c * big * gran_per_chunk : cb < n_bulk ? cb * gran_per_chunk : n_bulk * gran_per_chunk + (cb - n_bulk);
                    const uint32_t g1 = c < n_big ? g0 + big * gran_per_chunk : cb < n_bulk ? g0 + gran_per_chunk : g0 + 1u;
                    cur = g0 << 6;
                    cur_end = (g1 << 6) < count ? (g1 << 6) : count;
                }
            }
            if (!exhausted) {
                const uint32_t qi_seq = cur + (uint32_t)__popcll(idle_mask & ((1ull << lane) - 1ull));
                if (idle && qi_seq < cur_end) {
                    const uint32_t qi = (!PRIM && tune.perm) ? tune.perm[qi_seq] : qi_seq;
                    uint32_t hid = PRIM ? HIT_MISS : ld_stream(&hit[qi]);
                    if (hid != HIT_DEAD && !(ANY && hid != HIT_MISS)) {
                        float4 O, D;
                        float hd2_0 = 0.0f;
                        if (PRIM) {
                            f3 po, pd;
                            uint32_t pixel, sample, lp;
                            primary_ray(pr, ld_stream(&pr.pid[qi]), po, pd, pixel, sample, &lp);
                            const float4 E = pr.pix[pr.n_pix_local + lp];
                            hid = __float_as_uint(E.y);
                            hd2_0 = E.z;
#ifndef PRT_NO_OPAQUE_ORIGIN
                            asm volatile("" : "+v"(po.x), "+v"(po.y), "+v"(po.z));
#endif
                            O = make_float4(po.x, po.y, po.z, 0.f);
                            D = make_float4(pd.x, pd.y, pd.z, 0.f);
                        } else {
                            O = ld_stream(&ro[qi]);
                            D = ld_stream(&rd[qi]);
                        }
                        o = mk3(O.x, O.y, O.z);
                        ld = normalize3(mk3(D.x, D.y, D.z));
                        pad = sc.pad * (__builtin_fabsf(o.x) + __builtin_fabsf(o.y) + __builtin_fabsf(o.z) + sc.extent);
                        ix = __builtin_amdgcn_rcpf(__builtin_fabsf(ld.x) < PRT_DIR_MIN ? __builtin_copysignf(PRT_DIR_MIN, ld.x) : ld.x);
                        iy = __builtin_amdgcn_rcpf(__builtin_fabsf(ld.y) < PRT_DIR_MIN ? __builtin_copysignf(PRT_DIR_MIN, ld.y) : ld.y);
                        iz = __builtin_amdgcn_rcpf(__builtin_fabsf(ld.z) < PRT_DIR_MIN ? __builtin_copysignf(PRT_DIR_MIN, ld.z) : ld.z);
                        const bool nx = ix < 0.0f, ny = iy < 0.0f, nz = iz < 0.0f;
                        anx = (nx ? o.x - pad : o.x + pad) * ix; afx = (nx ? o.x + pad : o.x - pad) * ix;
                        any = (ny ? o.y - pad : o.y + pad) * iy; afy = (ny ? o.y + pad : o.y - pad) * iy;
                        anz = (nz ? o.z - pad : o.z + pad) * iz; afz = (nz ? o.z + pad : o.z - pad) * iz;
                        octinv4 = (7u - ((nx ? 1u : 0u) | (ny ? 2u : 0u) | (nz ? 4u : 0u))) * 0x01010101u;
                        best.id = hid;
                        best.prim = hid;
                        best.d2 = PRIM ? hd2_0 : ld_stream(&hd2[qi]);
                        tlimit = limit_from_d2(best.d2, pad);
                        if (LEAN) {
                            s_lray[0 * 256 + tid] = o.x; s_lray[1 * 256 + tid] = o.y; s_lray[2 * 256 + tid] = o.z;
                            s_lray[3 * 256 + tid] = ld.x; s_lray[4 * 256 + tid] = ld.y; s_lray[5 * 256 + tid] = ld.z;
                            s_key[tid] = ((unsigned long long)__float_as_uint(best.d2) << 32) | (hid == HIT_MISS ? 0u : hid);
                            s_slot[tid] = hid;
                        }
                        k = qi;
                        if (STATS) ray_steps = 0u;
                        gx = 0u;
                        gy = 1u << (24u + (octinv4 & 7u));
                        sp = 0;
                        if (INST) {
                            in_blas = false;
                            stall = false;
                            ipm = 0u;
                            lscale = 1.0f;
                            padw4 = 0.0f;
                            s_wray[0 * 256 + tid] = O.x; s_wray[1 * 256 + tid] = O.y; s_wray[2 * 256 + tid] = O.z;
                            s_wray[3 * 256 + tid] = D.x; s_wray[4 * 256 + tid] = D.y; s_wray[5 * 256 + tid] = D.z;
                        }
                    }
                }
                cur = (cur + n_idle < cur_end) ? cur + n_idle : cur_end;
            }
        }
        if (__ballot(k != 0xFFFFFFFFu) == 0ull) {
            if (exhausted) break;
            continue;
        }
        if (STATS) {
            const unsigned long long t = __builtin_amdgcn_s_memtime();
            cyc_refill += t - t_mark;
            t_mark = t;
        }
        bool walk = (k != 0xFFFFFFFFu) && ((gy > 0x00FFFFFFu) || sp > 0 || (INST && ipm != 0u)) && !(INST && stall);
        uint32_t q_groups = 0u;
        while (walk) {
            uint32_t tm = 0u, tb = 0u;
            {
                const int spr = sp > 0 ? sp - 1 : 0;
                const uint2 top = s_stack[spr * 256 + tid];
                const bool has = gy > 0x00FFFFFFu;
                bool level_switch = false;
                if (INST) {
                    const bool enter = !in_blas && ipm != 0u;
                    const bool leave = in_blas && !has && top.x == T8_SENTINEL;
                    if (enter || leave) {
                        stall = true;
                        walk = false;
                        level_switch = true;
// ... 61 lines not shown
            const uint32_t G = ((volatile uint32_t*)s_qn)[wv];
            if (G != 0u) {
                const unsigned long long key_best =
                    LEAN ? 0ull : ((unsigned long long)__float_as_uint(best.d2) << 32) | (best.id == HIT_MISS ? 0u : best.prim);
                if (!LEAN) s_key[tid] = key_best;
                if (lane == 0) s_qn[wv] = 0u;
                for (uint32_t g0 = 0u; g0 < G; g0 += 64u) {
                const uint32_t cap = (G - g0 > 64u) ? T8_QCAP / 2u : T8_QCAP;
                const unsigned long long ga = g0 + lane < G ? ((volatile unsigned long long*)queue)[g0 + lane] : 0ull;
                const uint32_t base_a = (uint32_t)ga, own_a = (uint32_t)(ga >> 56);
                uint32_t ma = (uint32_t)(ga >> 32) & 0x00FFFFFFu;
                __builtin_amdgcn_fence(__ATOMIC_SEQ_CST, "wavefront");
                while (__ballot(ma != 0u) != 0ull) {
                    const uint32_t ca = (uint32_t)__popc(ma);
                    const uint32_t ia = wave_scan_add(ca);
                    const bool fit_a = ia <= cap;
                    const uint32_t nfa = (uint32_t)__popcll(__ballot(fit_a));
                    const uint32_t T = (uint32_t)__shfl((int)ia, (int)(nfa - 1u), 64);
                    if (fit_a && ca) {
                        uint32_t qp = ia - ca;
                        for (uint32_t m = ma; m; m &= m - 1u) queue[qp++] = (own_a << 26) | (base_a + (uint32_t)__builtin_ctz(m));
                        ma = 0u;
                    }
                    __builtin_amdgcn_fence(__ATOMIC_SEQ_CST, "wavefront");
                    for (uint32_t base = 0; base < T; base += 64u) {
                        const uint32_t kq = base + lane;
                        const bool act = kq < T;
                        const uint32_t item = ((volatile uint32_t*)queue)[act ? kq : 0u];
                        const uint32_t owner = act ? (item >> 26) : lane;
                        const uint32_t slot = item & 0x03FFFFFFu;
                        f3 qo, qd;
                        if (LEAN) {
                            const uint32_t oc = wbase + owner;
                            qo = mk3(s_lray[0 * 256 + oc], s_lray[1 * 256 + oc], s_lray[2 * 256 + oc]);
                            qd = mk3(s_lray[3 * 256 + oc], s_lray[4 * 256 + oc], s_lray[5 * 256 + oc]);
                        } else {
                            qo = mk3(__shfl(o.x, (int)owner, 64), __shfl(o.y, (int)owner, 64), __shfl(o.z, (int)owner, 64));
                            qd = mk3(__shfl(ld.x, (int)owner, 64), __shfl(ld.y, (int)owner, 64), __shfl(ld.z, (int)owner, 64));
                        }
                        uint32_t qinst = 0u, win = slot;
                        if (INST) qinst = (uint32_t)__shfl((int)inst, (int)owner, 64);
                        bool cand = false;
                        unsigned long long key = 0ull;
                        if (act) {
                            const float4 a = sc.tris[3 * (size_t)slot + 0];
                            const float4 b = sc.tris[3 * (size_t)slot + 1];
                            const float4 c = sc.tris[3 * (size_t)slot + 2];
                            if (STATS) ++n_tris;
                            f3 pos;
                            float b1, b2;
                            if (triangle_hit_pos(mk3(a.x, a.y, a.z), mk3(b.x, b.y, b.z), mk3(c.x, c.y, c.z), qo, qd, pos, b1, b2)) {
                                float d2;
                                uint32_t prim;
                                if (INST) {
                                    const DevInstance& I = sc.insts[qinst];
                                    const uint32_t oc = wbase + owner;
                                    d2 = dist2(mk3(s_wray[0 * 256 + oc], s_wray[1 * 256 + oc], s_wray[2 * 256 + oc]), transform_point(I.mat, pos));
                                    prim = I.prim_base + __float_as_uint(a.w);
                                    win = I.virt_base + (slot - I.slot_base);
                                } else {
                                    d2 = dist2(qo, pos);
                                    prim = __float_as_uint(a.w);
                                }
                                key = ((unsigned long long)__float_as_uint(d2) << 32) | prim;
                                if (ANY)
                                    cand = key < atomicMin(&s_key[wbase + owner], key);
                                else {
                                    cand = true;
                                    atomicMin(&s_key[wbase + owner], key);
                                }
                            }
                        }
                        if (STATS && lane == 0) ++s_iters[4 + wv];
                        __builtin_amdgcn_fence(__ATOMIC_SEQ_CST, "wavefront");
                        if (cand && ((volatile unsigned long long*)s_key)[wbase + owner] == key) s_slot[wbase + owner] = LEAN ? sc.n_prims + win : win;
                        __builtin_amdgcn_fence(__ATOMIC_SEQ_CST, "wavefront");
                    }
                }
                }
                const unsigned long long won =
                    ((volatile unsigned long long*)s_key)[(STEAL && k >= 0xFFFFFF00u && k != 0xFFFFFFFFu) ? wbase + (k & 63u) : tid];
                if (LEAN) {
                    tlimit = limit_from_d2(__uint_as_float((uint32_t)(won >> 32)), pad);
                    if (ANY && k != 0xFFFFFFFFu &&
                        ((volatile uint32_t*)s_slot)[(STEAL && k >= 0xFFFFFF00u) ? wbase + (k & 63u) : tid] != HIT_MISS) {
                        gy = 0u;
                        sp = 0;
                    }
                } else if (won != key_best) {
                    best.d2 = __uint_as_float((uint32_t)(won >> 32));
                    best.prim = (uint32_t)won;
                    best.id = sc.n_prims + ((volatile uint32_t*)s_slot)[tid];
                    tlimit = INST ? (limit_from_d2(best.d2, 0.0f) + padw4) * lscale + 4.0f * pad : limit_from_d2(best.d2, pad);
                    if (ANY && k != 0xFFFFFFFFu) {
                        gy = 0u;
                        sp = 0;
                        if (INST) {
                            ipm = 0u;
                            in_blas = false;
                            stall = false;
                        }
                    }
                }
                pending = false;
            }
        }
        if (STATS) {
            const unsigned long long t = __builtin_amdgcn_s_memtime();
            cyc_tri += t - t_mark;
            t_mark = t;
        }
    }
    if (STATS) {
        if (lane == 0) {
            atomicAdd(&stats[6], cyc_refill);
            atomicAdd(&stats[7], cyc_node);
            atomicAdd(&stats[8], cyc_tri);
            unsigned long long* tl = stats + 16 + PRT_TIMELINE_WORDS * tune.probe_slot;
            const unsigned long long t_end = __builtin_amdgcn_s_memrealtime();
            if (t_exh == 0ull) t_exh = t_end;
            if (my_xcd == 0u) {
                atomicMin(&tl[0], t_start);
                atomicMax(&tl[1], t_end);
                atomicMin(&tl[2], t_exh);
                atomicMax(&tl[3], t_exh);
            }
            atomicAdd(&tl[4], t_end - t_exh);
            atomicAdd(&tl[5], t_end - t_start);
            atomicAdd(&tl[6], 1ull);
        }
        uint32_t w_nodes = n_nodes, w_tris = n_tris, w_steps = ray_steps_max, w_sp = max_sp;
        for (int off = 32; off > 0; off >>= 1) {
            w_nodes += (uint32_t)__shfl_xor((int)w_nodes, off, 64);
            w_tris += (uint32_t)__shfl_xor((int)w_tris, off, 64);
            const uint32_t a = (uint32_t)__shfl_xor((int)w_steps, off, 64), b = (uint32_t)__shfl_xor((int)w_sp, off, 64);
            w_steps = a > w_steps ? a : w_steps;
            w_sp = b > w_sp ? b : w_sp;
        }
        if (lane == 0) {
            atomicMax(&stats[16 + PRT_TIMELINE_WORDS * tune.probe_slot + 7], (unsigned long long)w_steps);
            atomicAdd(&stats[0], (unsigned long long)w_nodes);
            atomicAdd(&stats[1], (unsigned long long)w_tris);
            atomicMax(&stats[5], (unsigned long long)w_sp);
        }
        __syncthreads();
        if (threadIdx.x < 4) atomicAdd(&stats[3], 64ull * s_iters[threadIdx.x]);
        if (threadIdx.x < 4) atomicAdd(&stats[4], 64ull * s_iters[4 + threadIdx.x]);
    }
}

template <int STACK_L, int WAVES, bool STATS, bool INST, bool LEAN = false, bool PRIM = false, bool PATH = false>
__global__ void __launch_bounds__(256, WAVES) k_traverse8_persistent(DevScene sc, const float4* __restrict__ ro,
                                                                    const float4* __restrict__ rd,
                                                                    uint32_t* __restrict__ hit,
                                                                    const float* __restrict__ hd2,
                                                                    const uint32_t* __restrict__ count_ptr,
                                                                    uint32_t* __restrict__ work,
                                                                    uint32_t* __restrict__ ovf, PrtTravTuning tune,
                                                                    unsigned long long* __restrict__ stats, PrtPrimary pr,
                                                                    PrtPathArgs pa) {
    traverse8_body<STACK_L, WAVES, STATS, INST, LEAN, PRIM, PATH, false>(sc, ro, rd, hit, hd2, count_ptr, work, ovf, tune,
                                                                         stats, pr, pa);
}

template <int STACK_L, int WAVES, bool INST, bool LEAN = false>
__global__ void __launch_bounds__(256, WAVES) k_occluded8_persistent(DevScene sc, const float4* __restrict__ ro,
                                                                    const float4* __restrict__ rd,
                                                                    uint32_t* __restrict__ hit,
                                                                    const float* __restrict__ hd2,
                                                                    const uint32_t* __restrict__ count_ptr,
                                                                    uint32_t* __restrict__ work,
                                                                    uint32_t* __restrict__ ovf, PrtTravTuning tune) {
    traverse8_body<STACK_L, WAVES, false, INST, LEAN, false, false, true>(sc, ro, rd, hit, hd2, count_ptr, work, ovf, tune,
                                                                          nullptr, PrtPrimary{}, PrtPathArgs{});
}

template <int FUSE, bool SAMPLING, bool INST, bool ABVH, bool PRIM, bool ENV, bool TEX = false>
PRT_DEV void shade_step(DevScene sc, const float4* __restrict__ ro, const float4* __restrict__ rd, const float4* __restrict__ rt,
                        const uint32_t* __restrict__ hit, float4* __restrict__ no, float4* __restrict__ nd, float4* __restrict__ nt,
                        uint32_t* __restrict__ nhit, float* __restrict__ nhd2, float4* __restrict__ rad, uint32_t* __restrict__ counts,
                        uint32_t* __restrict__ work, uint32_t iter, uint32_t max_depth, uint32_t cap, PrtSampling sp_arg, PrtPrimary pr,
                        const DevEnv* env, const DevTex* tex = nullptr) {
    const PrtSampling sp = SAMPLING ? sp_arg : PrtSampling{0u, 0u, 0.0f};
    const uint32_t nA = CNT_A(counts, iter), nB = CNT_B(counts, iter);
    const uint32_t count = nA + nB;
    if (blockIdx.x * (uint32_t)SHADE_BLOCK >= count) return;
    const uint32_t k = blockIdx.x * (uint32_t)SHADE_BLOCK + threadIdx.x;
    if (k < 8u) work[32u * k] = 0u;
    if (k == 8u) work[512] = 0u;
    bool front = false, back = false;
    f3 o = mk3(0.f, 0.f, 0.f), d = mk3(0.f, 0.f, 1.f), thr = mk3(0.f, 0.f, 0.f);
    uint32_t id0 = HIT_MISS, rng = 0, depth = 0, pid = 0;
    float d2_0 = 3.402823466e+38f;
    float4 pre_a = make_float4(0.f, 0.f, 0.f, 0.f), pre_b = pre_a;
    if (k < count) {
        const uint32_t src = k < nA ? k : cap - 1u - (k - nA);
        uint32_t id = (PRIM && (k >= nA || pr.walk)) ? HIT_MISS : ld_stream(&hit[src]);
        if (PRIM) {
            pid = ld_stream(&pr.pid[src]);
            uint32_t pixel, sample, lp;
            primary_ray(pr, pid, o, d, pixel, sample, &lp);
            if (k >= nA) id = __float_as_uint(pr.pix[pr.n_pix_local + lp].y);
            else if (pr.walk) id = hit[__float_as_uint(pr.pix[pr.n_pix_local + lp].x)];
            rng = path_seed(pixel, pr.first_sample + sample, pr.seed);
            depth = 0u;
            thr = mk3(1.f, 1.f, 1.f);
            pre_a = pr.pix[2u * pr.n_pix_local + lp];
            pre_b = pr.pix[3u * pr.n_pix_local + lp];
        } else {
            const float4 O = ld_stream(&ro[src]);
            const float4 D = ld_stream(&rd[src]);
            const float4 T = ld_stream(&rt[src]);
            pid = __float_as_uint(O.w);
            rng = __float_as_uint(D.w);
            depth = __float_as_uint(T.w);
            thr = mk3(T.x, T.y, T.z);
            o = mk3(O.x, O.y, O.z);
            d = mk3(D.x, D.y, D.z);
        }
        if (id != HIT_DEAD) {
            const int r = advance_path<1 + FUSE, INST, ABVH, SHADE_BLOCK, PRIM, ENV, TEX>(sc, id, o, d, thr, rng, depth, max_depth, sp, &rad[pid], id0, d2_0, pre_a, pre_b, env, tex);
            front = r == 1;
            back = r == 2;
        }
    }
    const uint32_t slot = block_alloc2<SHADE_BLOCK>(front, back, false, &CNT_A(counts, iter + 1u), &CNT_B(counts, iter + 1u),
                                                    &CNT_C(counts, iter + 1u), cap);
    if (slot != 0xFFFFFFFFu) {
        st_stream(&no[slot], make_float4(o.x, o.y, o.z, __uint_as_float(pid)));
        st_stream(&nd[slot], make_float4(d.x, d.y, d.z, __uint_as_float(rng)));
        st_stream(&nt[slot], make_float4(thr.x, thr.y, thr.z, __uint_as_float(depth)));
        st_stream(&nhit[slot], id0);
        st_stream(&nhd2[slot], d2_0);
    }
}

template <int FUSE, bool SAMPLING, bool INST, bool ABVH, bool PRIM = false>
__global__ void __launch_bounds__(SHADE_BLOCK) k_shade(DevScene sc, const float4* __restrict__ ro,
                                                      const float4* __restrict__ rd, const float4* __restrict__ rt,
                                                      const uint32_t* __restrict__ hit, float4* __restrict__ no,
                                                      float4* __restrict__ nd, float4* __restrict__ nt,
                                                      uint32_t* __restrict__ nhit, float* __restrict__ nhd2,
                                                      float4* __restrict__ rad, uint32_t* __restrict__ counts,
                                                      uint32_t* __restrict__ work, uint32_t iter, uint32_t max_depth,
                                                      uint32_t cap, PrtSampling sp_arg, PrtPrimary pr) {
    shade_step<FUSE, SAMPLING, INST, ABVH, PRIM, false>(sc, ro, rd, rt, hit, no, nd, nt, nhit, nhd2, rad, counts, work, iter, max_depth,
                                                        cap, sp_arg, pr, nullptr);
}

template <bool INST, bool ABVH>
__global__ void __launch_bounds__(SHADE_BLOCK) k_shade_env(DevScene sc, DevEnv env, const float4* __restrict__ ro,
                                                          const float4* __restrict__ rd, const float4* __restrict__ rt,
                                                          const uint32_t* __restrict__ hit, float4* __restrict__ no,
                                                          float4* __restrict__ nd, float4* __restrict__ nt,
                                                          uint32_t* __restrict__ nhit, float* __restrict__ nhd2,
                                                          float4* __restrict__ rad, uint32_t* __restrict__ counts,
                                                          uint32_t* __restrict__ work, uint32_t iter, uint32_t max_depth,
                                                          uint32_t cap, PrtSampling sp_arg) {
    shade_step<0, true, INST, ABVH, false, true>(sc, ro, rd, rt, hit, no, nd, nt, nhit, nhd2, rad, counts, work, iter, max_depth, cap,
                                                 sp_arg, PrtPrimary{}, &env);
}

template <bool INST, bool ABVH, bool ENV>
__global__ void __launch_bounds__(SHADE_BLOCK) k_shade_tex(DevScene sc, DevTex tex, DevEnv env, const float4* __restrict__ ro,
                                                          const float4* __restrict__ rd, const float4* __restrict__ rt,
                                                          const uint32_t* __restrict__ hit, float4* __restrict__ no,
                                                          float4* __restrict__ nd, float4* __restrict__ nt,
                                                          uint32_t* __restrict__ nhit, float* __restrict__ nhd2,
                                                          float4* __restrict__ rad, uint32_t* __restrict__ counts,
                                                          uint32_t* __restrict__ work, uint32_t iter, uint32_t max_depth,
                                                          uint32_t cap, PrtSampling sp_arg) {
    shade_step<0, true, INST, ABVH, false, ENV, true>(sc, ro, rd, rt, hit, no, nd, nt, nhit, nhd2, rad, counts, work, iter, max_depth, cap,
                                                      sp_arg, PrtPrimary{}, ENV ? &env : nullptr, &tex);
}

__global__ void __launch_bounds__(256) k_primary_hit(DevScene sc, PrtPrimary pr, const uint32_t* __restrict__ hit,
                                                     float4* __restrict__ pix, const uint32_t* __restrict__ counts) {
    const uint32_t pl = blockIdx.x * 256u + threadIdx.x;
    if (pl >= pr.n_pix_local) return;
    const float4 E = pix[pr.n_pix_local + pl];
    float4 a = make_float4(0.f, 0.f, 0.f, __uint_as_float(HIT_DEAD)), b = make_float4(0.f, 0.f, 0.f, 0.f);
    if (__float_as_uint(E.w) == 0xFFFFFFFEu) {
        const uint32_t first = __float_as_uint(E.x);
        const bool walked = pr.walk ? first != 0xFFFFFFFFu : first < CNT_A(counts, 0);
        const uint32_t id = walked ? hit[first] : __float_as_uint(E.y);
        if (id != HIT_MISS && id != HIT_DEAD) {
            const float4 P = pix[pl];
            WorldHit w;
            world_hit_from_id<false>(sc, id, mk3(pr.origin[0], pr.origin[1], pr.origin[2]), mk3(P.x, P.y, P.z), w);
            if (w.has) {
                a = make_float4(w.pos.x, w.pos.y, w.pos.z, __uint_as_float(id));
                b = make_float4(w.normal.x, w.normal.y, w.normal.z, __uint_as_float(w.material | (w.front ? 0x80000000u : 0u)));
            }
        }
    }
    pix[2u * pr.n_pix_local + pl] = a;
    pix[3u * pr.n_pix_local + pl] = b;
}

__global__ void __launch_bounds__(SHADE_BLOCK) k_shade_divstats(DevScene sc, const uint32_t* __restrict__ hit,
                                                                 const uint32_t* __restrict__ counts, uint32_t iter, uint32_t cap,
                                                                 unsigned long long* __restrict__ out, PrtPrimary pr, int compact) {
    const uint32_t nA = CNT_A(counts, iter), nB = CNT_B(counts, iter);
    const uint32_t count = nA + nB;
// ... 1232 lines not shown
    }
#endif
    const dim3 grid(r.grid), block(256);
    uint32_t* ovf = work + 512;
    const uint32_t* no_list = nullptr;
#define PRT_LAUNCH_T(KERNEL, L, W, MODE, GRID, COUNT, LIST)                                                        \
    do {                                                                                                           \
        if (stats)                                                                                                 \
            hipLaunchKernelGGL((KERNEL<L, W, MODE, true>), GRID, block, 0, st, sc, in.o, in.d, in.hit, in.hd2,     \
                               COUNT, work, spill, LIST, ovf, tune, stats);                                        \
        else                                                                                                       \
            hipLaunchKernelGGL((KERNEL<L, W, MODE, false>), GRID, block, 0, st, sc, in.o, in.d, in.hit, in.hd2,    \
                               COUNT, work, spill, LIST, ovf, tune, stats);                                        \
    } while (0)
    const PrtT8Kind kind = r.kind;
    if (kind != T8_NONE) {
#define PRT_LAUNCH_8(L, W, IN)                                                                                     \
    do {                                                                                                           \
        if (stats)                                                                                                 \
            hipLaunchKernelGGL((k_traverse8_persistent<L, W, true, IN>), grid, block, 0, st, sc, in.o, in.d,       \
                               in.hit, in.hd2, count_ptr, work, ovf, tune, stats, PrtPrimary{}, PrtPathArgs{});    \
        else                                                                                                       \
            hipLaunchKernelGGL((k_traverse8_persistent<L, W, false, IN>), grid, block, 0, st, sc, in.o, in.d,      \
                               in.hit, in.hd2, count_ptr, work, ovf, tune, stats, PrtPrimary{}, PrtPathArgs{});    \
    } while (0)
        if (kind == T8_INST12_4) {
            PRT_LAUNCH_8(12, 4, true);
            return;
        }
        if (kind == T8_WIDE11_5) {
            PRT_LAUNCH_8(11, 5, false);
        } else if (kind == T8_LEAN8_5) {
            const dim3 grid5(r.grid5);
            const PrtTravTuning& t5 = r.t5;
            if (stats && primary)
                hipLaunchKernelGGL((k_traverse8_persistent<8, 5, true, false, true, true>), grid5, block, 0, st, sc, in.o, in.d,
                                   in.hit, in.hd2, count_ptr, work, ovf, t5, stats, *primary, PrtPathArgs{});
            else if (stats)
                hipLaunchKernelGGL((k_traverse8_persistent<8, 5, true, false, true>), grid5, block, 0, st, sc, in.o, in.d,
                                   in.hit, in.hd2, count_ptr, work, ovf, t5, stats, PrtPrimary{}, PrtPathArgs{});
            else if (primary)
                hipLaunchKernelGGL((k_traverse8_persistent<8, 5, false, false, true, true>), grid5, block, 0, st, sc, in.o, in.d,
                                   in.hit, in.hd2, count_ptr, work, ovf, t5, stats, *primary, PrtPathArgs{});
            else
                hipLaunchKernelGGL((k_traverse8_persistent<8, 5, false, false, true>), grid5, block, 0, st, sc, in.o, in.d,
                                   in.hit, in.hd2, count_ptr, work, ovf, t5, stats, PrtPrimary{}, PrtPathArgs{});
        } else {
            PRT_LAUNCH_8(15, 4, false);
        }
#undef PRT_LAUNCH_8
        if (r.rewalk) {
            hipLaunchKernelGGL(k_reset_cursors, dim3(1), dim3(64), 0, st, work);
            PRT_LAUNCH_T(k_traverse4_persistent, 27, 5, 1, dim3(8), ovf, ovf + 1);
        }
    } else if (tune.wide) {
        if (stack4 <= 22 && tune.stack_lds == 24) PRT_LAUNCH_T(k_traverse4_persistent, 22, 6, 0, grid, count_ptr, no_list);
        else if (stack4 <= 27) PRT_LAUNCH_T(k_traverse4_persistent, 27, 5, 0, grid, count_ptr, no_list);
        else if (tune.stack_lds == 39 && stack4 <= 35) PRT_LAUNCH_T(k_traverse4_persistent, 35, 4, 0, grid, count_ptr, no_list);
        else if (tune.stack_lds == 2) {
            PRT_LAUNCH_T(k_traverse4_persistent, 27, 5, 2, grid, count_ptr, no_list);
            hipLaunchKernelGGL(k_reset_cursors, dim3(1), dim3(64), 0, st, work);
            PRT_LAUNCH_T(k_traverse4_persistent, 27, 5, 1, dim3(8), ovf, ovf + 1);
        } else if (tune.stack_lds == 3) {
            PRT_LAUNCH_T(k_traverse4_persistent, 24, 5, 3, grid, count_ptr, no_list);
            hipLaunchKernelGGL(k_reset_cursors, dim3(1), dim3(64), 0, st, work);
            PRT_LAUNCH_T(k_traverse4_persistent, 27, 5, 1, dim3(8), ovf, ovf + 1);
        } else if (tune.stack_lds == 1) {
            PRT_LAUNCH_T(k_traverse4_persistent, 27, 5, 1, grid, count_ptr, no_list);
        } else {
            PRT_LAUNCH_T(k_traverse4_persistent, 32, 4, 3, grid, count_ptr, no_list);
            hipLaunchKernelGGL(k_reset_cursors, dim3(1), dim3(64), 0, st, work);
            PRT_LAUNCH_T(k_traverse4_persistent, 27, 5, 1, dim3(8), ovf, ovf + 1);
        }
    } else {
        const uint32_t pushes = tree_depth ? tree_depth - 1u : 0u;
        if (pushes <= 24 && tune.stack_lds == 24) PRT_LAUNCH_T(k_traverse_persistent, 24, 6, 0, grid, count_ptr, no_list);
        else if (pushes <= 31) PRT_LAUNCH_T(k_traverse_persistent, 31, 5, 0, grid, count_ptr, no_list);
        else PRT_LAUNCH_T(k_traverse_persistent, 31, 5, 1, grid, count_ptr, no_list);
    }
#undef PRT_LAUNCH_T
}

void prt_launch_occluded(hipStream_t st, const DevScene& sc, const PrtRayBuf& in, const uint32_t* count_ptr, uint32_t* work,
                         uint32_t* spill, uint32_t max_rays, uint32_t tree_depth, uint32_t stack4, const PrtTravTuning& tune_in) {
    if (t8_kind(sc, tune_in) == T8_NONE) {
        prt_launch_traverse(st, sc, in, count_ptr, work, spill, max_rays, tree_depth, stack4, tune_in, nullptr);
        return;
    }
    PrtTravTuning tune_o = tune_in;
    tune_o.perm = nullptr;
    const T8Launch r = t8_resolve(sc, tune_o, max_rays);
    const dim3 block(256);
    uint32_t* ovf = work + 512;
#define PRT_LAUNCH_O(L, W, IN, LN, GRID, TUNE)                                                                       \
    hipLaunchKernelGGL((k_occluded8_persistent<L, W, IN, LN>), dim3(GRID), block, 0, st, sc, in.o, in.d, in.hit, in.hd2,  \
                       count_ptr, work, ovf, TUNE)
    if (r.kind == T8_INST12_4) PRT_LAUNCH_O(12, 4, true, false, r.grid, r.tune);
    else if (r.kind == T8_WIDE11_5) PRT_LAUNCH_O(11, 5, false, false, r.grid, r.tune);
    else if (r.kind == T8_LEAN8_5) PRT_LAUNCH_O(8, 5, false, true, r.grid5, r.t5);
    else PRT_LAUNCH_O(15, 4, false, false, r.grid, r.tune);
#undef PRT_LAUNCH_O
    if (r.rewalk) {
        hipLaunchKernelGGL(k_reset_cursors, dim3(1), dim3(64), 0, st, work);
        hipLaunchKernelGGL((k_traverse4_persistent<27, 5, 1, false>), dim3(8), block, 0, st, sc, in.o, in.d, in.hit, in.hd2,
                           ovf, work, spill, ovf + 1, ovf, r.tune, (unsigned long long*)nullptr);
    }
}

bool prt_path_kernel_applies(const DevScene& sc, const PrtTravTuning& tune) {
    return sc.nodes8 && !sc.n_insts && !sc.abvh_nodes && sc.depth8 <= 16u && tune.wide == 2u && tune.stack_cap == 0u;
}
void prt_launch_path(hipStream_t st, const DevScene& sc, const PrtPathArgs& pa, uint32_t* work, const PrtTravTuning& tune_in) {
    PrtTravTuning tune = tune_in;
    if (tune.exit_max == 0xFFFFFFFFu) tune.exit_max = 16u;
    if (tune.tri_min == 0u) tune.tri_min = 24u;
    uint32_t g = tune.grid_blocks;
    const uint32_t need_blocks = blocks_for(pa.n_paths);
    if (g > need_blocks) g = need_blocks;
    if (g == 0) g = 1;
    hipLaunchKernelGGL((k_traverse8_persistent<15, 4, false, false, false, false, true>), dim3(g), dim3(256), 0, st, sc, (const float4*)nullptr,
                       (const float4*)nullptr, (uint32_t*)nullptr, (const float*)nullptr, (const uint32_t*)nullptr, work, work + 512, tune,
                       (unsigned long long*)nullptr, PrtPrimary{}, pa);
}

int prt_traverse_occupancy(const DevScene& sc, const PrtTravTuning& tune, int* blocks_per_cu, int* vgprs, int* sgprs, int* lds_bytes) {
    const PrtT8Kind kind = t8_kind(sc, tune);
    const void* fn = kind == T8_INST12_4 ? (const void*)k_traverse8_persistent<12, 4, false, true>
                     : kind == T8_WIDE11_5 ? (const void*)k_traverse8_persistent<11, 5, false, false>
                     : kind == T8_LEAN8_5 ? (const void*)k_traverse8_persistent<8, 5, false, false, true>
                     : kind == T8_DEEP15_4 ? (const void*)k_traverse8_persistent<15, 4, false, false>
                                           : (const void*)k_traverse4_persistent<32, 4, 3, false>;
    hipFuncAttributes at;
    hipError_t e = hipFuncGetAttributes(&at, fn);
    if (e != hipSuccess) return (int)e;
    int nb = 0;
    e = hipOccupancyMaxActiveBlocksPerMultiprocessor(&nb, fn, 256, 0);
    if (e != hipSuccess) return (int)e;
    *blocks_per_cu = nb;
    *vgprs = at.numRegs;
    *sgprs = 0;
    *lds_bytes = (int)at.sharedSizeBytes;
    return 0;
}

void prt_launch_intersect(hipStream_t st, const DevScene& sc, const PrtRayBuf& in, const uint32_t* count_ptr, uint32_t max_rays, int stack_depth, int variant,
                          unsigned long long* stats) {
    const dim3 grid(blocks_for(max_rays)), block(256);
#define PRT_LAUNCH_I(S, T, V) \
    hipLaunchKernelGGL((k_intersect<S, T, V>), grid, block, 0, st, sc, in.o, in.d, in.hit, count_ptr, stats)
    const bool deep = stack_depth > 31;
    if (stats) {
        if (variant == 2) { if (deep) PRT_LAUNCH_I(63, true, 1); else PRT_LAUNCH_I(31, true, 1); }
        else              { if (deep) PRT_LAUNCH_I(63, true, 0); else PRT_LAUNCH_I(31, true, 0); }
    } else {
        if (variant == 2) { if (deep) PRT_LAUNCH_I(63, false, 1); else PRT_LAUNCH_I(31, false, 1); }
        else              { if (deep) PRT_LAUNCH_I(63, false, 0); else PRT_LAUNCH_I(31, false, 0); }
    }
#undef PRT_LAUNCH_I
}

bool prt_launch_shade(hipStream_t st, PrtShadeInst inst, const PrtShadeArgs& a) {
    const uint32_t n_for_grid = a.n_rays_known == 0xFFFFFFFFu ? a.cap : (a.n_rays_known ? a.n_rays_known : 1u);
    const dim3 grid((uint32_t)((n_for_grid + SHADE_BLOCK - 1) / SHADE_BLOCK));
    const DevScene& sc = *a.sc;
    const PrtPrimary& pr = or_empty(a.primary);
    const DevEnv& e = or_empty(a.env);
    const DevTex& tex = or_empty(a.tex);
    const DevLights& lt = or_empty(a.lights);
    const DevMeshLights& m = or_empty(a.mesh_lights);
    const PrtLightBufs& lb = or_empty(a.lb);
#define PRT_SHADE_RAYS a.in.o, a.in.d, a.in.t, a.in.hit, a.out.o, a.out.d, a.out.t, a.out.hit, a.out.hd2
#define PRT_SHADE_TAIL a.rad, a.counts, a.work, a.depth, a.max_depth, a.cap, a.sp
#define PRT_SHADE_ARGS_PLAIN sc, PRT_SHADE_RAYS, PRT_SHADE_TAIL, pr
#define PRT_SHADE_ARGS_ENV sc, e, PRT_SHADE_RAYS, PRT_SHADE_TAIL
#define PRT_SHADE_ARGS_TEX sc, tex, e, PRT_SHADE_RAYS, PRT_SHADE_TAIL
#define PRT_SHADE_ARGS_NEE sc, lt, PRT_SHADE_RAYS, lb, PRT_SHADE_TAIL
#define PRT_SHADE_ARGS_NEE_ENV sc, lt, e, PRT_SHADE_RAYS, lb, PRT_SHADE_TAIL
#define PRT_SHADE_ARGS_NEE_MESH sc, lt, m, PRT_SHADE_RAYS, lb, PRT_SHADE_TAIL
#define PRT_SHADE_ARGS_NEE_MESH_ENV sc, lt, m, e, PRT_SHADE_RAYS, lb, PRT_SHADE_TAIL
#define PRT_SHADE_ARGS_NEE_TEX sc, tex, lt, m, e, PRT_SHADE_RAYS, lb, PRT_SHADE_TAIL
#define PRT_SHADE_CASE(sig, kernel, tag, ...) \
    case PRT_INST(kernel, tag): hipLaunchKernelGGL((kernel<__VA_ARGS__>), grid, dim3(SHADE_BLOCK), 0, st, PRT_SHADE_ARGS_##sig); return true;
    switch (inst) {
        PRT_SHADE_INSTANCES(PRT_SHADE_CASE)
        default: return false;
    }
#undef PRT_SHADE_CASE
#undef PRT_SHADE_ARGS_NEE_TEX
#undef PRT_SHADE_ARGS_NEE_MESH_ENV
#undef PRT_SHADE_ARGS_NEE_MESH
#undef PRT_SHADE_ARGS_NEE_ENV
#undef PRT_SHADE_ARGS_NEE
#undef PRT_SHADE_ARGS_TEX
#undef PRT_SHADE_ARGS_ENV
#undef PRT_SHADE_ARGS_PLAIN
#undef PRT_SHADE_TAIL
#undef PRT_SHADE_RAYS
}

void prt_launch_shade_divstats(hipStream_t st, const DevScene& sc, const PrtRayBuf& in, const uint32_t* counts, uint32_t iter,
                               uint32_t cap, unsigned long long* out, const PrtPrimary* primary) {
    hipLaunchKernelGGL(k_shade_divstats, dim3((cap + SHADE_BLOCK - 1u) / SHADE_BLOCK), dim3(SHADE_BLOCK), 0, st, sc, in.hit, counts, iter, cap, out,
                       primary ? *primary : PrtPrimary{}, primary ? 1 : 0);
}

void prt_launch_primary_hit(hipStream_t st, const DevScene& sc, const PrtPrimary& pr, const uint32_t* hit, float4* pix,
                            const uint32_t* counts) {
    hipLaunchKernelGGL(k_primary_hit, dim3(blocks_for(pr.n_pix_local)), dim3(256), 0, st, sc, pr, hit, pix, counts);
}

bool prt_launch_accumulate(hipStream_t st, PrtAccumulateInst inst, const PrtAccumulateArgs& a) {
    const uint32_t nb = blocks_for(a.tm.n_pix_local ? a.tm.n_pix_local : 1);
    const dim3 grid(nb < 8192u ? nb : 8192u);
    const int upd = a.update_film ? 1 : 0;
#define PRT_ACC_ARGS_PLAIN a.rad, a.film_local, a.tm, a.S, a.max_depth, upd, a.ray_stats, a.pix_end
#define PRT_ACC_ARGS_LIT a.rad, a.lrad, a.film_local, a.tm, a.S, a.max_depth, upd, a.ray_stats
#define PRT_ACC_ARGS_STAT a.rad, a.lrad, a.film_local, a.stat, a.tm, a.S, a.max_depth, upd, a.ray_stats, a.pix_end, a.list
#define PRT_ACC_CASE_N(sig, kernel) \
    case PRT_I_##kernel: hipLaunchKernelGGL(kernel, grid, dim3(256), 0, st, PRT_ACC_ARGS_##sig); return true;
#define PRT_ACC_CASE_T(sig, kernel, tag, ...) \
    case PRT_INST(kernel, tag): hipLaunchKernelGGL((kernel<__VA_ARGS__>), grid, dim3(256), 0, st, PRT_ACC_ARGS_##sig); return true;
    switch (inst) {
        PRT_ACCUMULATE_INSTANCES(PRT_ACC_CASE_N, PRT_ACC_CASE_T)
        default: return false;
    }
#undef PRT_ACC_CASE_T
#undef PRT_ACC_CASE_N
#undef PRT_ACC_ARGS_STAT
#undef PRT_ACC_ARGS_LIT
#undef PRT_ACC_ARGS_PLAIN
}

void prt_launch_resolve(hipStream_t st, const float4* gathered, uint32_t world, uint32_t stride, uint32_t W,
                        uint32_t H, float* rgb, float* weight) {
    hipLaunchKernelGGL(k_resolve, dim3(blocks_for((uint64_t)W * H)), dim3(256), 0, st, gathered, world, stride, W, H,
                       rgb, weight);
}

void prt_launch_tonemap(hipStream_t st, const float* rgb, const float* weight, uint32_t n_pix, float exposure,
                        float inv_gamma, uint8_t* out) {
    hipLaunchKernelGGL(k_tonemap, dim3(blocks_for((uint64_t)n_pix * 4u)), dim3(256), 0, st, rgb, weight, n_pix,
                       exposure, inv_gamma, out);
}

void prt_launch_camera_rays_lens(hipStream_t st, const DevCamera& cam, const DevLens& lens, uint32_t n, const float* px,
                                 const float* py, uint32_t* keys, float* o, float* d) {
    hipLaunchKernelGGL(k_camera_rays_lens, dim3(blocks_for(n)), dim3(256), 0, st, cam, lens, n, px, py, keys, o, d);
}
void prt_launch_camera_rays(hipStream_t st, const DevCamera& cam, uint32_t n, const float* px, const float* py,
                            float* o, float* d) {
    hipLaunchKernelGGL(k_camera_rays, dim3(blocks_for(n)), dim3(256), 0, st, cam, n, px, py, o, d);
}

void prt_launch_pack_rays(hipStream_t st, uint32_t n, const float* o, const float* d, const PrtRayBuf& out,
                          uint32_t* counts) {
    hipLaunchKernelGGL(k_pack_rays, dim3(blocks_for(n)), dim3(256), 0, st, n, o, d, out.o, out.d, counts);
}

void prt_launch_hit_records(hipStream_t st, const DevScene& sc, uint32_t n, const PrtRayBuf& in, PrtHit* out) {
    hipLaunchKernelGGL(k_hit_records, dim3(blocks_for(n)), dim3(256), 0, st, sc, n, in.o, in.d, in.hit, out);
}

void prt_launch_pack_occlusion_rays(hipStream_t st, uint32_t n, const float* o, const float* d, const float* tmax,
                                    const PrtRayBuf& out, uint32_t* counts) {
    hipLaunchKernelGGL(k_pack_occlusion_rays, dim3(blocks_for(n)), dim3(256), 0, st, n, o, d, tmax, out.o, out.d, out.hit,
                       out.hd2, counts);
}

void prt_launch_scan_prims_bounded(hipStream_t st, const DevScene& sc, const PrtRayBuf& in, const uint32_t* count_ptr,
                                   uint32_t* work, uint32_t max_rays) {
    hipLaunchKernelGGL(k_scan_prims_bounded, dim3(blocks_for(max_rays)), dim3(256), 0, st, sc, in.o, in.d, in.hit, in.hd2,
                       count_ptr, work);
}

void prt_launch_occlusion_bytes(hipStream_t st, const DevScene& sc, uint32_t n, const PrtRayBuf& in, const float* tmax,
                                uint8_t* out) {
    hipLaunchKernelGGL(k_occlusion_bytes, dim3(blocks_for(n)), dim3(256), 0, st, sc, n, in.o, in.d, in.hit, tmax, out);
}

// ... 50 lines not shown
```

parallelraytracing_amd/csrc/prt_route.h:

```cpp
#pragma once
#include <cstdint>

#define PRT_ROWS2(T, s, k) T(s, k, ff, false, false) T(s, k, ft, false, true) T(s, k, tf, true, false) T(s, k, tt, true, true)
#define PRT_ROWS3(T, s, k) \
    T(s, k, fff, false, false, false) T(s, k, fft, false, false, true) T(s, k, ftf, false, true, false) T(s, k, ftt, false, true, true) \
    T(s, k, tff, true, false, false) T(s, k, tft, true, false, true) T(s, k, ttf, true, true, false) T(s, k, ttt, true, true, true)
#define PRT_ROWS4(T, s, k) \
    T(s, k, ffff, false, false, false, false) T(s, k, ffft, false, false, false, true) T(s, k, fftf, false, false, true, false) T(s, k, fftt, false, false, true, true) \
    T(s, k, ftff, false, true, false, false) T(s, k, ftft, false, true, false, true) T(s, k, fttf, false, true, true, false) T(s, k, fttt, false, true, true, true) \
    T(s, k, tfff, true, false, false, false) T(s, k, tfft, true, false, false, true) T(s, k, tftf, true, false, true, false) T(s, k, tftt, true, false, true, true) \
    T(s, k, ttff, true, true, false, false) T(s, k, ttft, true, true, false, true) T(s, k, tttf, true, true, true, false) T(s, k, tttt, true, true, true, true)
#define PRT_RAYGEN_INSTANCES(T) \
    T(PLAIN, k_raygen, fttf, false, true, true, false) \
    T(PLAIN, k_raygen, tttf, true, true, true, false) \
    T(PLAIN, k_raygen, ffff, false, false, false, false) \
    T(PLAIN, k_raygen, ftff, false, true, false, false) \
    T(PLAIN, k_raygen, tfff, true, false, false, false) \
    T(PLAIN, k_raygen, ttff, true, true, false, false) \
    T(COMPACT, k_raygen, ffft, false, false, false, true) \
    PRT_ROWS2(T, ENV, k_raygen_env) \
    PRT_ROWS2(T, LENS, k_raygen_lens) \
    PRT_ROWS2(T, LENS_ENV, k_raygen_lens_env) \
    PRT_ROWS4(T, LIST, k_raygen_list)
#define PRT_SHADE_INSTANCES(T) \
    T(PLAIN, k_shade, 0ffft, 0, false, false, false, true) \
    T(PLAIN, k_shade, 0tftf, 0, true, false, true, false) \
    T(PLAIN, k_shade, 0tttf, 0, true, true, true, false) \
    T(PLAIN, k_shade, 0ttff, 0, true, true, false, false) \
    T(PLAIN, k_shade, 1ffff, 1, false, false, false, false) \
    T(PLAIN, k_shade, 1tfff, 1, true, false, false, false) \
    T(PLAIN, k_shade, 0ffff, 0, false, false, false, false) \
    T(PLAIN, k_shade, 0tfff, 0, true, false, false, false) \
    PRT_ROWS2(T, ENV, k_shade_env) \
    PRT_ROWS3(T, TEX, k_shade_tex) \
    PRT_ROWS2(T, NEE, k_shade_nee) \
    PRT_ROWS2(T, NEE_ENV, k_shade_nee_env) \
    PRT_ROWS2(T, NEE_MESH, k_shade_nee_mesh) \
    PRT_ROWS2(T, NEE_MESH_ENV, k_shade_nee_mesh_env) \
    PRT_ROWS4(T, NEE_TEX, k_shade_nee_tex)
#define PRT_ACCUMULATE_INSTANCES(N, T) \
    N(PLAIN, k_accumulate) \
    N(LIT, k_accumulate_lit) \
    PRT_ROWS2(T, STAT, k_accumulate_stat)

#define PRT_INST(kernel, tag) PRT_I_##kernel##_##tag
#define PRT_INST_ENUM_N(sig, kernel) PRT_I_##kernel,
#define PRT_INST_ENUM_T(sig, kernel, tag, ...) PRT_INST(kernel, tag),
#define PRT_INST_NAME_N(sig, kernel) #kernel,
#define PRT_INST_NAME_T(sig, kernel, tag, ...) #kernel "<" #__VA_ARGS__ ">",
enum PrtRaygenInst : uint32_t { PRT_RAYGEN_INSTANCES(PRT_INST_ENUM_T) PRT_RAYGEN_NONE };
enum PrtShadeInst : uint32_t { PRT_SHADE_INSTANCES(PRT_INST_ENUM_T) PRT_SHADE_NONE };
enum PrtAccumulateInst : uint32_t { PRT_ACCUMULATE_INSTANCES(PRT_INST_ENUM_N, PRT_INST_ENUM_T) PRT_ACCUMULATE_NONE };
inline const char* prt_raygen_name(PrtRaygenInst i) {
    static const char* const names[] = {PRT_RAYGEN_INSTANCES(PRT_INST_NAME_T) ""};
    return names[i <= PRT_RAYGEN_NONE ? i : PRT_RAYGEN_NONE];
}
inline const char* prt_shade_name(PrtShadeInst i) {
    static const char* const names[] = {PRT_SHADE_INSTANCES(PRT_INST_NAME_T) ""};
    return names[i <= PRT_SHADE_NONE ? i : PRT_SHADE_NONE];
}
inline const char* prt_accumulate_name(PrtAccumulateInst i) {
    static const char* const names[] = {PRT_ACCUMULATE_INSTANCES(PRT_INST_NAME_N, PRT_INST_NAME_T) ""};
    return names[i <= PRT_ACCUMULATE_NONE ? i : PRT_ACCUMULATE_NONE];
}

struct PrtRouteFacts {
    bool lit;
    bool mesh_lights;
    bool env;
    bool tex;
    bool lens;
    bool listed;
    bool film_stats;
    bool has_nodes;
    bool has_bvh2;
    bool insts;
    bool abvh;
    bool few_prims;
    bool jitter;
    bool sa;
    bool multi_sample;
    bool variant0;
    bool compact_primary;
    bool primary_walk;
    bool takes_primary;
    bool primary_hit;
    bool path_gate;
    uint32_t path_kernel;
    uint32_t fuse;
};

struct PrtRoutePlan {
    bool path;
    bool compact;
    bool walk;
    bool primary_hit;
    bool walk8;
    uint32_t fuse;
    PrtRaygenInst raygen;
    PrtShadeInst shade0, shade;
    PrtAccumulateInst accumulate;
};

inline bool prt_route_walk8(bool variant0, bool insts, bool has_bvh2) { return variant0 || insts || !has_bvh2; }

inline PrtRoutePlan prt_plan_route(const PrtRouteFacts& f) {
    PrtRoutePlan p{};
    const bool plain_shade = !f.lit && !f.env && !f.tex && !f.listed;
    const bool plain = plain_shade && !f.lens;
    p.fuse = (plain_shade && f.has_nodes && f.few_prims) ? f.fuse : 0u;
    p.path = plain && f.path_kernel != 0u && (f.path_kernel == 2u || !f.multi_sample) && f.path_gate && f.variant0 && p.fuse == 0u;
    p.compact = !p.path && plain && f.compact_primary && f.variant0 && f.has_nodes && !f.abvh && !f.jitter && !f.sa && p.fuse == 0u &&
                f.takes_primary;
    p.walk = p.compact && f.primary_walk && f.multi_sample;
    p.primary_hit = p.compact && f.primary_hit && f.multi_sample;
    p.walk8 = prt_route_walk8(f.variant0, f.insts, f.has_bvh2);

    const uint32_t j = f.jitter, ab = f.abvh, in = f.insts, en = f.env, ml = f.mesh_lights;
    if (p.path) p.raygen = PRT_RAYGEN_NONE;
    else if (f.listed) p.raygen = PrtRaygenInst(PRT_INST(k_raygen_list, ffff) + (j << 3 | ab << 2 | en << 1 | (uint32_t)f.lens));
    else if (f.lens) p.raygen = PrtRaygenInst((f.env ? PRT_INST(k_raygen_lens_env, ff) : PRT_INST(k_raygen_lens, ff)) + (j << 1 | ab));
    else if (f.env) p.raygen = PrtRaygenInst(PRT_INST(k_raygen_env, ff) + (j << 1 | ab));
    else if (f.abvh) p.raygen = f.jitter ? PRT_INST(k_raygen, tttf) : PRT_INST(k_raygen, fttf);
    else if (f.jitter) p.raygen = f.sa ? PRT_INST(k_raygen, ttff) : PRT_INST(k_raygen, tfff);
    else if (p.compact) p.raygen = PRT_INST(k_raygen, ffft);
    else p.raygen = f.sa ? PRT_INST(k_raygen, ftff) : PRT_INST(k_raygen, ffff);

    if (p.path) p.shade = PRT_SHADE_NONE;
    else if (f.lit && f.tex) p.shade = PrtShadeInst(PRT_INST(k_shade_nee_tex, ffff) + (in << 3 | ab << 2 | ml << 1 | en));
    else if (f.lit)
        p.shade = PrtShadeInst((f.mesh_lights ? (f.env ? PRT_INST(k_shade_nee_mesh_env, ff) : PRT_INST(k_shade_nee_mesh, ff))
                                              : (f.env ? PRT_INST(k_shade_nee_env, ff) : PRT_INST(k_shade_nee, ff))) + (in << 1 | ab));
    else if (f.tex) p.shade = PrtShadeInst(PRT_INST(k_shade_tex, fff) + (in << 2 | ab << 1 | en));
    else if (f.env) p.shade = PrtShadeInst(PRT_INST(k_shade_env, ff) + (in << 1 | ab));
    else if (f.abvh) p.shade = f.insts ? PRT_INST(k_shade, 0tttf) : PRT_INST(k_shade, 0tftf);
    else if (f.insts) p.shade = PRT_INST(k_shade, 0ttff);
    else if (p.fuse) p.shade = f.sa ? PRT_INST(k_shade, 1tfff) : PRT_INST(k_shade, 1ffff);
    else p.shade = f.sa ? PRT_INST(k_shade, 0tfff) : PRT_INST(k_shade, 0ffff);
    p.shade0 = p.compact ? PRT_INST(k_shade, 0ffft) : p.shade;

    if (f.film_stats || f.listed) p.accumulate = PrtAccumulateInst(PRT_INST(k_accumulate_stat, ff) + ((uint32_t)f.lit << 1 | (uint32_t)f.listed));
    else p.accumulate = f.lit ? PRT_I_k_accumulate_lit : PRT_I_k_accumulate;
    return p;
}
```

parallelraytracing_amd/csrc/prt_scene.cpp:

```cpp
#include "prt_scene.h"

#include <algorithm>
#include <array>
#include <cfloat>
#include <chrono>
#include <cmath>
#include <cstdarg>
#include <cstdio>
#include <cstring>
#include <utility>

extern "C" uint32_t prt_spill_rows(uint32_t max_stack4, uint32_t max_depth) {
    const uint32_t rows4 = max_stack4 > 27u ? max_stack4 - 27u : 0u;
    const uint32_t rows2 = max_depth > 32u ? max_depth - 32u : 0u;
    return std::max(64u, std::max(rows4, rows2) + 1u);
}

namespace {

constexpr uint32_t kMaxLeaf = 3;
constexpr uint32_t kMaxStack = 63;
constexpr int kHostBuildFailed = -1001;

using Clock = std::chrono::steady_clock;
// ... 24 lines not shown
    for (int a = 0; a < 3 && ok; ++a)
        for (int b = 0; b < 3; ++b)
            if (std::fabs(g[a][b] - (a == b ? s2 : 0.0)) > 1e-4 * s2) ok = false;
    *s2_out = s2;
    return ok;
}

bool affine_bottom_row(const float* M) { return M[3] == 0.0f && M[7] == 0.0f && M[11] == 0.0f && M[15] == 1.0f; }

bool is_similarity(const float* M, const float* inv, double* s2_out) {
    bool ok = gram_is_uniform_scale(M, s2_out);
    for (int r = 0; r < 4 && ok; ++r)
        for (int cc = 0; cc < 4; ++cc) {
            double acc = 0.0, mag = 1.0;
            for (int kk = 0; kk < 4; ++kk) {
                const double term = (double)inv[4 * kk + r] * (double)M[4 * cc + kk];
                acc += term;
                mag = std::max(mag, std::fabs(term));
            }
            if (!(std::fabs(acc - (r == cc ? 1.0 : 0.0)) <= (cc == 3 ? std::max(1e-3, 1e-5 * mag) : 1e-3 * mag))) ok = false;
        }
    return ok && affine_bottom_row(M);
}

void build_light_table(PrtHostScene* c, const PrtSceneDesc* s) {
    c->lights.clear();
    c->prim_light.assign(s->n_primitives, 0xFFFFFFFFu);
    c->n_emitters_unsampled = 0;
    auto emissive = [&](uint32_t m) { return m < s->n_materials && s->materials[m].type == PRT_MAT_EMISSIVE; };
    std::vector<double> power;
    for (uint32_t i = 0; i < s->n_primitives; ++i) {
        const PrtPrimitive& p = s->primitives[i];
        if (!emissive(p.material_id)) continue;
        const float* M = p.mat;
        double s2 = 0.0;
        if (!is_similarity(p.mat, p.inv, &s2)) {
            ++c->n_emitters_unsampled;
            continue;
        }
        const float* rgb = s->materials[p.material_id].rgb;
        const double mean = ((double)rgb[0] + (double)rgb[1] + (double)rgb[2]) / 3.0;
        const bool quad = p.shape_type == PRT_SHAPE_QUAD;
        const double w = p.shape_param[0], h = p.shape_param[1];
        const double area = quad ? std::fabs(w * h) * s2 : 4.0 * M_PI * w * w * s2;
        const double pw = (quad ? 2.0 * area : area) * mean;
        if (!(pw > 0.0) || !std::isfinite(pw)) continue;
        float rec[4 * PRT_LIGHT_F4] = {};
        rec[0] = M[12];
        rec[1] = M[13];
        rec[2] = M[14];
        rec[3] = quad ? (float)area : (float)(std::fabs(w) * std::sqrt(s2));
        const double nx = (double)M[1] * M[10] - (double)M[2] * M[9], ny = (double)M[2] * M[8] - (double)M[0] * M[10],
                     nz = (double)M[0] * M[9] - (double)M[1] * M[8];
        const double nl = std::sqrt(nx * nx + ny * ny + nz * nz);
        for (int a = 0; a < 3; ++a) {
            rec[4 + a] = quad ? (float)(w * M[a]) : 0.0f;
            rec[8 + a] = quad ? (float)(h * M[8 + a]) : 0.0f;
        }
        if (quad) {
            rec[12] = (float)(nx / nl);
            rec[13] = (float)(ny / nl);
            rec[14] = (float)(nz / nl);
        }
        const uint32_t kind = quad ? 1u : 0u;
        memcpy(&rec[15], &kind, 4);
        rec[16] = rgb[0];
        rec[17] = rgb[1];
        rec[18] = rgb[2];
        memcpy(&rec[19], &i, 4);
        c->prim_light[i] = (uint32_t)power.size();
        power.push_back(pw);
        c->lights.insert(c->lights.end(), rec, rec + 4 * PRT_LIGHT_F4);
    }
    double total = 0.0;
    for (double pw : power) total += pw;
    double acc = 0.0;
    for (size_t l = 0; l < power.size(); ++l) {
        acc += power[l];
        c->lights[4 * PRT_LIGHT_F4 * l + 7] = (float)(power[l] / total);
        c->lights[4 * PRT_LIGHT_F4 * l + 11] = l + 1 == power.size() ? 1.0f : (float)(acc / total);
    }
    c->light_power = power;
    const uint32_t n_not_similar = c->n_emitters_unsampled;
    for (uint32_t m = 0; m < s->n_meshes; ++m)
        if (emissive(s->meshes[m].material_id)) c->n_emitters_unsampled += s->meshes[m].n_triangles;
    for (uint32_t i = 0; i < s->n_instances; ++i) {
        const PrtInstance& pi = s->instances[i];
        if (emissive(pi.material_id) && pi.mesh < s->n_instanced_meshes) c->n_emitters_unsampled += s->instanced_meshes[pi.mesh].n_triangles;
    }
    c->ml_tris_counted = c->n_emitters_unsampled - n_not_similar;
}

void pack_records(const std::vector<uint32_t>& order, const float* verts, const float* norms, uint32_t n, uint32_t prim_base,
                  const uint32_t* tri_mat, float* tri_rec, float* nrm_rec) {
    for (size_t slot = 0; slot < (size_t)n; ++slot) {
        const uint32_t t = order[slot];
        float* r = &tri_rec[12 * slot];
        for (int v = 0; v < 3; ++v)
            for (int a = 0; a < 3; ++a) {
                r[4 * v + a] = verts[9 * (size_t)t + 3 * v + a];
                if (nrm_rec) nrm_rec[12 * slot + 4 * v + a] = norms[9 * (size_t)t + 3 * v + a];
            }
        const uint32_t prim = prim_base + t;
        memcpy(&r[3], &prim, 4);
        if (tri_mat) memcpy(&r[7], &tri_mat[t], 4);
    }
}

void box_triangle(const float* mn, const float* mx, float* tri) {
    const float t9[9] = {mn[0], mn[1], mn[2], mx[0], mx[1], mx[2], mn[0], mx[1], mn[2]};
    memcpy(tri, t9, sizeof(t9));
}

struct TreeInput {
    const float* verts;
    const float* norms;
    const uint32_t* tri_mat;
    uint32_t n, n_prims;
};

int build_tree(const PrtSceneOptions& opt, const TreeInput& in, float leaf_cost, bool keep, uint32_t device_depth_limit, bool host_fallback,
               int host_threads, BvhBuild* out, float* tri_rec, float* nrm_rec, bool* on_device, double* gpu_ms, std::string* err) {
    *on_device = false;
    if (opt.device_build && in.n > 0) {
        *out = BvhBuild();
        out->max_leaf = 3;
        const int brc = opt.device_build(in.verts, in.norms, in.tri_mat, in.n, in.n_prims, leaf_cost, keep, out->nodes8, out->depth8, tri_rec,
                                         nrm_rec, gpu_ms, err);
        if (brc && brc != kPrtDeviceBuildGaveUp) return brc;
        if (!brc && out->depth8 <= device_depth_limit) {
            *on_device = true;
            return PRT_OK;
        }
        if (!host_fallback) return kPrtDeviceBuildGaveUp;
        *out = BvhBuild();
        std::fill_n(tri_rec, 12 * (size_t)in.n, 0.0f);
        if (nrm_rec) std::fill_n(nrm_rec, 12 * (size_t)in.n, 0.0f);
    }
    return bvh_build(in.verts, in.n, kMaxLeaf, host_threads, kMaxStack, out) ? PRT_OK : kHostBuildFailed;
}

struct Work {
    std::vector<float> verts, norms;
    std::vector<uint32_t> tri_mat;
    uint32_t n_world = 0;
    bool world_on_device = false;
    Clock::time_point t_build0;
    double host_build_ms = 0.0;
    uint32_t depth8 = 0;
};


void write_tri_candidates(PrtMeshLights& ml, size_t at, const float* verts, uint32_t n, const float* rgb, uint32_t prim_first) {
    const double mean = ((double)rgb[0] + (double)rgb[1] + (double)rgb[2]) / 3.0;
    for (uint32_t t = 0; t < n; ++t) {
        const float* v = &verts[9 * (size_t)t];
        float* rec = &ml.records[4 * PRT_LIGHT_F4 * (at + t)];
        std::fill_n(rec, 4 * PRT_LIGHT_F4, 0.0f);
        double e1[3], e2[3];
        for (int a = 0; a < 3; ++a) {
            e1[a] = (double)v[3 + a] - (double)v[a];
            e2[a] = (double)v[6 + a] - (double)v[a];
            rec[a] = v[a];
            rec[4 + a] = (float)e1[a];
            rec[8 + a] = (float)e2[a];
        }
        const double cx = e1[1] * e2[2] - e1[2] * e2[1], cy = e1[2] * e2[0] - e1[0] * e2[2], cz = e1[0] * e2[1] - e1[1] * e2[0];
        const double cl = std::sqrt(cx * cx + cy * cy + cz * cz);
        const double area = 0.5 * cl;
        rec[3] = (float)area;
        if (cl > 0.0 && std::isfinite(cl)) {
// ... 884 lines not shown
```

parallelraytracing_amd/csrc/prt_scene.h:

```cpp
#pragma once
#include <stdint.h>

#include <array>
#include <functional>
#include <string>
#include <vector>

#include "../../include/prt.h"
#include "bvh.h"
#include "prt_scene_pod.h"

struct PrtSceneScalars {
    uint32_t n_insts;
    uint32_t n_prims;
    uint32_t n_nodes;
    uint32_t n_tris;
    float pad;
    float abvh_q[3];
    float extent;
    float root_min[3], root_max[3];
    float sky[3];
};

struct PrtLightRun {
    uint32_t prim_first, n_tris, light_first, world;
};

struct PrtMeshLights {
    std::vector<float> records;
    std::vector<double> power;
    std::vector<uint32_t> thr;
    uint32_t n_search = 0;
    std::vector<uint32_t> bucket;
    uint32_t bucket_shift = 32;
    std::vector<PrtLightRun> runs;
    std::vector<uint32_t> visible;
    std::vector<uint32_t> cand_visible;
    std::vector<uint64_t> width;
    uint32_t n_emitters_unsampled = 0;
};

struct PrtEnvTables {
    uint32_t W = 0, H = 0;
    float light_share = 0.0f;
    std::vector<float> texels;
    std::vector<uint64_t> row_width;
    std::vector<uint64_t> col_width;
    std::vector<uint32_t> row_thr;
    std::vector<uint32_t> col_thr;
    std::vector<uint32_t> col_last;
    uint32_t row_last = 0;
    uint32_t n_sampled = 0;
};
int prt_build_environment(const PrtEnvironment* env, PrtEnvTables* out, std::string* err);
uint64_t prt_environment_threshold(const PrtEnvTables& env, uint32_t n_lights);
float prt_scaled_pmf(double pmf, uint64_t t_env);

struct PrtPlacedMesh {
    float mn[3], mx[3];
    uint32_t slot_base;
    uint32_t node_base;
    uint32_t depth8;
    uint32_t n_tris;
};

struct PrtHostScene {
    std::vector<PrtMaterial> materials;
    std::vector<DevPrim> prims;
    BvhBuild bvh;
    std::vector<float> tri_records;
    std::vector<float> nrm_records;
    double gpu_build_ms = 0.0;
    bool scene_device_built = false;
    std::vector<uint32_t> mesh_sizes;
    std::vector<uint32_t> nodes8_all;
    std::vector<DevInstance> dev_insts;
    std::vector<uint32_t> tlas_inst;
    std::vector<PrtPlacedMesh> placed_meshes;
    std::vector<uint32_t> inst_mesh;
    std::array<float, 6> world_box{};
    uint32_t n_world_insts = 0;
    uint32_t top_nodes = 0;
    uint32_t top_depth = 0;
    uint32_t max_mesh_depth = 0;
    float extent_base = 0.0f;
    uint32_t builder = 0;
    BvhBuild abvh;
    PrtBvhInfo bvh_info{};
    PrtSceneScalars sc{};
    std::vector<float> lights;
    std::vector<uint32_t> prim_light;
    uint32_t n_emitters_unsampled = 0;
    std::vector<double> light_power;
    uint32_t ml_tris_counted = 0;
    PrtMeshLights ml;
    std::vector<uint32_t> mesh_indices;
    std::vector<uint32_t> mesh_material;
    std::vector<std::vector<uint32_t>> placed_indices;
    std::vector<uint32_t> placed_vertices;
    uint32_t n_instanced_meshes = 0;
};

struct PrtTexTables {
    bool is_set = false;
    uint32_t n_textures = 0;
    uint32_t n_textured_materials = 0;
    std::vector<float> texels;
    std::vector<uint32_t> desc;
    std::vector<uint32_t> mat_tex;
    std::vector<float> uvs;
    std::vector<uint32_t> inst_uv_base;
};
int prt_build_textures(const PrtHostScene& hs, const PrtTextureSet* set, PrtTexTables* out, std::string* err);

void prt_scaled_light_tables(const PrtHostScene& hs, uint64_t t_env, std::vector<float>* lights, std::vector<float>* ml_records);

constexpr int kPrtDeviceBuildGaveUp = -1000;
using PrtDeviceBuilder = std::function<int(const float* verts, const float* norms, const uint32_t* tri_mat, uint32_t n, uint32_t n_prims,
                                           float leaf_cost, bool keep, std::vector<uint32_t>& nodes8, uint32_t& depth, float* tri_rec,
                                           float* nrm_rec, double* ms, std::string* err)>;

struct PrtSceneOptions {
    float pad_coeff;
    bool prim_bvh;
    PrtDeviceBuilder device_build;
};

int prt_check_scene_arrays(const PrtSceneDesc* s, std::string* err);

int prt_compile_scene(const PrtSceneDesc* s, const PrtSceneOptions& opt, PrtHostScene* out, std::string* err);

void prt_rebuild_mesh_lights(PrtHostScene* hs, const float* verts, const PrtInstance* placed = nullptr);

struct PrtInstanceUpdate {
    std::vector<DevInstance> insts;
    std::vector<std::array<float, 6>> boxes;
    std::vector<uint32_t> top_nodes8, top_order;
    uint32_t top_depth = 0;
};

int prt_check_instance_update(const PrtHostScene& hs, const PrtInstance* instances, uint32_t n, std::string* err);
void prt_instance_tables(const PrtHostScene& hs, const PrtInstance* instances, PrtInstanceUpdate* up);
int prt_build_top_level(const PrtSceneOptions& opt, const PrtHostScene& hs, PrtInstanceUpdate* up, double* gpu_ms, std::string* err);
void prt_commit_top_level(PrtHostScene* hs, const PrtInstanceUpdate& up);
void prt_commit_instances(PrtHostScene* hs, const PrtInstanceUpdate& up, const PrtInstance* instances);

int prt_flatten_mesh(const PrtMesh& me, const char* what, uint32_t m, float* verts, float* norms, float* extent, float* mn, float* mx,
                     std::string* err);
```

parallelraytracing_amd/renderer.py:

```python
from __future__ import annotations

import ctypes as C
from typing import List, Optional, Tuple

import numpy as np

from . import capi
from .capi import (PrtBvhInfo, PrtCameraDesc, PrtHit, PrtInstance, PrtMaterial, PrtMesh, PrtPrimitive, PrtSampling,
                   PrtSceneDesc, PrtStats)

_fp = C.POINTER(C.c_float)
_u32p = C.POINTER(C.c_uint32)

SKY = (0.4, 0.3, 0.6)
DEFAULT_MAX_DEPTH = 20


class PrtError(RuntimeError):
    pass


def _f32(a) -> np.ndarray:
    return np.ascontiguousarray(a, dtype=np.float32)

# ... 662 lines not shown
        self._check(capi.lib().prt_occluded(self._ctx, n, o.ctypes.data_as(_fp), d.ctypes.data_as(_fp),
                                            t.ctypes.data_as(_fp), out.ctypes.data_as(C.POINTER(C.c_uint8))))
        return out.astype(bool)

    def scatter(self, in_dirs, hits: np.ndarray, rng_state):
        d = _f32(in_dirs).reshape(-1, 3)
        n = d.shape[0]
        hits = np.ascontiguousarray(hits)
        rng = np.ascontiguousarray(rng_state, dtype=np.uint32).copy()
        sc = np.zeros(n, np.uint32)
        att, em, oo, od = (np.zeros((n, 3), np.float32) for _ in range(4))
        self._check(capi.lib().prt_scatter(self._ctx, n, d.ctypes.data_as(_fp), hits.ctypes.data_as(C.POINTER(PrtHit)),
                                           rng.ctypes.data_as(_u32p), sc.ctypes.data_as(_u32p),
                                           att.ctypes.data_as(_fp), em.ctypes.data_as(_fp), oo.ctypes.data_as(_fp),
                                           od.ctypes.data_as(_fp)))
        return sc.astype(bool), att, em, oo, od, rng

    def enable_timing(self, on: bool = True):
        self._check(capi.lib().prt_enable_timing(self._ctx, int(on)))

    def stats(self) -> PrtStats:
        s = PrtStats()
        self._check(capi.lib().prt_get_stats(self._ctx, C.byref(s)))
        return s

    def reset_stats(self):
        self._check(capi.lib().prt_reset_stats(self._ctx))

    def measure_traversal(self, sample: int = 0) -> PrtStats:
        s = PrtStats()
        self._check(capi.lib().prt_measure_traversal(self._ctx, self.max_depth, self.seed, sample, C.byref(s)))
        return s

    def bvh_info(self) -> PrtBvhInfo:
        b = PrtBvhInfo()
        self._check(capi.lib().prt_bvh_info(self._ctx, C.byref(b)))
        return b

    def kernel_occupancy(self):
        o = capi.PrtOccupancy()
        self._check(capi.lib().prt_kernel_occupancy(self._ctx, C.byref(o)))
        return o

    def Refit(self, scene: "Scene"):
        d = scene.desc()
        scene._keep = d
        self._check(capi.lib().prt_refit_meshes(self._ctx, d.meshes, d.n_meshes))
        self._scene = scene

    def UpdateInstances(self, scene: "Scene", mode: str = "refit"):
        insts = (PrtInstance * max(1, len(scene.instances)))(*scene.instances)
        self._check(capi.lib().prt_set_instance_transforms(self._ctx, insts, len(scene.instances), capi.INSTANCE_MODES[mode]))
        self._scene = scene

    def instance_update_info(self) -> "capi.PrtInstanceUpdateInfo":
        info = capi.PrtInstanceUpdateInfo()
        self._check(capi.lib().prt_instance_update_info(self._ctx, C.byref(info)))
        return info

    def instances_read(self) -> dict:
        n = C.c_uint32(0)
        L = capi.lib()
        self._check(L.prt_instances_read(self._ctx, 0, C.byref(n), None, None, None, None))
        out = {k: np.zeros(n.value, np.uint32) for k in ("slot_instance", "root", "slot_base", "prim_base")}
        self._check(L.prt_instances_read(self._ctx, n.value, C.byref(n), *[out[k].ctypes.data_as(_u32p) for k in out]))
        return out

    def measure_shade_divergence(self, sample: int = 0) -> np.ndarray:
        out = np.zeros((self.max_depth, 16), np.uint64)
        self._check(capi.lib().prt_measure_shade_divergence(self._ctx, self.max_depth, self.seed, int(sample),
                                                            out.ctypes.data_as(C.POINTER(C.c_uint64))))
        return out

    def kernel_instance(self) -> str:
        buf = C.create_string_buffer(64)
        self._check(capi.lib().prt_kernel_instance(self._ctx, buf, 64))
        return buf.value.decode()

    def shade_instance(self) -> str:
        buf = C.create_string_buffer(96)
        self._check(capi.lib().prt_shade_instance(self._ctx, buf, 96))
        return buf.value.decode()

    def bvh_read(self):
        b = self.bvh_info()
        nodes = np.zeros((b.n_nodes, 16), np.float32)
        tris = np.zeros((b.n_triangles, 12), np.float32)
        self._check(capi.lib().prt_bvh_read(self._ctx, nodes.ctypes.data_as(_fp), tris.ctypes.data_as(_fp)))
        return nodes, tris

    def bvh_read4(self) -> np.ndarray:
        b = self.bvh_info()
        nodes4 = np.zeros((b.n_nodes4, 32), np.float32)
        self._check(capi.lib().prt_bvh_read4(self._ctx, nodes4.ctypes.data_as(_fp)))
        return nodes4

    def bvh_read8(self) -> np.ndarray:
        b = self.bvh_info()
        nodes8 = np.zeros((b.n_nodes8, 20), np.uint32)
        self._check(capi.lib().prt_bvh_read8(self._ctx, nodes8.ctypes.data_as(C.POINTER(C.c_uint32))))
        return nodes8

    def set_scene_host_only(self, scene: Scene):
        d = scene.desc()
        self._check(capi.lib().prt_set_scene(self._ctx, C.byref(d)))
        if scene.textures or scene.material_texture:
            self.set_textures(scene)


class HipWavefrontGroupRenderer:

    def __init__(self, devices, max_depth: int = DEFAULT_MAX_DEPTH, seed: int = 0):
        self._grp = C.c_void_p()
        L = capi.lib()
        devs = (C.c_int * len(devices))(*[int(d) for d in devices])
        rc = L.prt_group_create(devs, len(devices), C.byref(self._grp))
        if rc:
            msg = L.prt_group_last_error(self._grp).decode()
            L.prt_group_destroy(self._grp)
            self._grp = None
            raise PrtError(f"prt_group_create({list(devices)}) failed: {msg}")
        self.max_depth = int(max_depth)
        self.seed = int(seed)
        self.frame_index = 0
        self.film: Optional[Film] = None

    def __del__(self):
        if getattr(self, "_grp", None):
            capi.lib().prt_group_destroy(self._grp)
            self._grp = None

    def _check(self, rc: int):
        if rc:
            raise PrtError(capi.lib().prt_group_last_error(self._grp).decode())

    @property
    def transport(self) -> str:
        return capi.lib().prt_group_transport(self._grp).decode()

    @property
    def n_devices(self) -> int:
        return capi.lib().prt_group_size(self._grp)

    def Init(self, film: Film, scene: Scene, camera: Camera):
        L = capi.lib()
        d = scene.desc()
        self._check(L.prt_group_set_scene(self._grp, C.byref(d)))
        if scene.textures or scene.material_texture:
            self.set_textures(scene)
        self._check(L.prt_group_set_film(self._grp, film.width, film.height))
        self.film = film
        self.frame_index = 0
        self.SetCamera(camera)

    def SetCamera(self, camera: Camera):
        d = camera.desc()
        self._check(capi.lib().prt_group_set_camera(self._grp, C.byref(d)))

    def Refit(self, scene: Scene):
        d = scene.desc()
        scene._keep = d
        self._check(capi.lib().prt_group_refit_meshes(self._grp, d.meshes, d.n_meshes))

    def UpdateInstances(self, scene: Scene, mode: str = "refit"):
        insts = (PrtInstance * max(1, len(scene.instances)))(*scene.instances)
        self._check(capi.lib().prt_group_set_instance_transforms(self._grp, insts, len(scene.instances), capi.INSTANCE_MODES[mode]))
# ... 161 lines not shown
```

Baseline: 23300 Mrays/s.

## Trace the final path segment as an any-hit query seeded with primitive hits

On the last bounce, only emissive hits contribute radiance. The change handles that segment with an occlusion (any-hit) traversal instead of a closest-hit traversal. Shading writes zero early for non-emissive in-shade hits and for rays seeded with a non-primitive candidate, and the seeded any-hit walk stops early once it finds a mesh triangle. It is meant to cut BVH traversal cost on the final segment, at the risk of correctness subtleties when an emissive primitive lies behind a mesh hit. A route plan gates it to non-NEE, non-fused, non-mesh-emissive scenes, and it defaults to mode 2.

```diff
diff --git a/include/prt.h b/include/prt.h
--- a/include/prt.h
+++ b/include/prt.h
@@ -311,6 +311,7 @@
 int prt_kernel_occupancy(PrtContext* ctx, PrtOccupancy* out);
 int prt_kernel_instance(PrtContext* ctx, char* name, uint32_t capacity);
 int prt_shade_instance(PrtContext* ctx, char* name, uint32_t capacity);
+int prt_last_segment(PrtContext* ctx, uint32_t* active, uint32_t* front_rays);
 int prt_bvh_read(PrtContext* ctx, float* nodes, float* tris);
 int prt_bvh_read4(PrtContext* ctx, float* nodes4);
 int prt_bvh_read8(PrtContext* ctx, uint32_t* nodes8);
diff --git a/parallelraytracing_amd/capi.py b/parallelraytracing_amd/capi.py
--- a/parallelraytracing_amd/capi.py
+++ b/parallelraytracing_amd/capi.py
@@ -250,6 +250,7 @@
     "prt_kernel_occupancy": (C.c_int, [_vp, C.POINTER(PrtOccupancy)]),
     "prt_kernel_instance": (C.c_int, [_vp, C.c_char_p, C.c_uint32]),
     "prt_shade_instance": (C.c_int, [_vp, C.c_char_p, C.c_uint32]),
+    "prt_last_segment": (C.c_int, [_vp, C.POINTER(C.c_uint32), C.POINTER(C.c_uint32)]),
     "prt_measure_shade_divergence": (C.c_int, [_vp, C.c_uint32, C.c_uint32, C.c_uint32, C.POINTER(C.c_uint64)]),
     "prt_refit_meshes": (C.c_int, [_vp, C.POINTER(PrtMesh), C.c_uint32]),
     "prt_set_instance_transforms": (C.c_int, [_vp, C.POINTER(PrtInstance), C.c_uint32, C.c_uint32]),
diff --git a/parallelraytracing_amd/csrc/prt_api.cpp b/parallelraytracing_amd/csrc/prt_api.cpp
--- a/parallelraytracing_amd/csrc/prt_api.cpp
+++ b/parallelraytracing_amd/csrc/prt_api.cpp
@@ -105,6 +105,9 @@
     PrtLens lens{0.0f, 0.0f, 0.0f};
     PrtTravTuning tune{1024u, 256u, 16u, 0xFFFFFFFFu , 0u, 2u, 0u , 0u, 0u, 0u, 1u, 8u, 1u, 0u, nullptr, 0u, 2500000u, 2u , 8u , 96u , 32u , 1u};
     unsigned long long* d_shade_div = nullptr;
+    uint32_t last_segment = 2;
+    uint32_t last_segment_active = 0;
+    uint32_t last_batch_depth = 0;
     uint32_t sort_rays = 0;
     uint32_t* d_sort = nullptr;
     size_t sort_entries = 0, sort_temp = 0;
@@ -498,11 +501,11 @@
 PrtBatchView whole_film(const PrtContext* c) { return PrtBatchView{c->tm, nullptr}; }
 
 void walk_rays(PrtContext* c, const PrtRayBuf& rays, const uint32_t* count, uint32_t max_rays, bool any, const PrtTravTuning& tune,
-               unsigned long long* stats, const PrtPrimary* primary) {
+               unsigned long long* stats, const PrtPrimary* primary, bool seeded = false) {
     if (!prt_route_walk8(c->variant == 0, c->dsc.n_insts != 0u, c->dsc.nodes != nullptr))
         prt_launch_intersect(c->stream, c->dsc, rays, count, max_rays, c->hs.bvh.max_depth <= 31 ? 31 : 63, c->variant, stats);
     else if (any)
-        prt_launch_occluded(c->stream, c->dsc, rays, count, c->d_work, c->d_spill, max_rays, c->hs.bvh.max_depth, c->hs.bvh.max_stack4, tune);
+        prt_launch_occluded(c->stream, c->dsc, rays, count, c->d_work, c->d_spill, max_rays, c->hs.bvh.max_depth, c->hs.bvh.max_stack4, tune, seeded);
     else
         prt_launch_traverse(c->stream, c->dsc, rays, count, c->d_work, c->d_spill, max_rays, c->hs.bvh.max_depth, c->hs.bvh.max_stack4,
                             tune, stats, primary);
@@ -570,6 +573,10 @@
     f.path_gate = !trav_stats && !c->d_shade_div && c->sort_rays == 0u && n_paths <= c->tune.path_max && prt_path_kernel_applies(c->dsc, c->tune);
     f.path_kernel = c->tune.path_kernel;
     f.fuse = c->tune.fuse;
+    f.mesh_emissive = c->hs.mesh_emissive;
+    f.depth_ge2 = max_depth >= 2u;
+    f.sort_rays = c->sort_rays != 0u;
+    f.last_segment = c->last_segment;
     const PrtRoutePlan plan = prt_plan_route(f);
     const bool lit = f.lit, compact = plan.compact, walk = plan.walk;
     const DevEnv denv = dev_env(c);
@@ -602,6 +609,8 @@
         return PRT_OK;
     };
     c->shade_instance = "";
+    c->last_segment_active = plan.last_segment;
+    c->last_batch_depth = plan.path ? 0u : max_depth;
     if (plan.path) {
         HIPCHECK(c, hipMemsetAsync(c->d_work, 0, 256 * sizeof(uint32_t), c->stream));
         PrtPathArgs pa{c->cam, tm, c->sampling, c->d_rad, first_sample, seed, max_depth, n_paths};
@@ -650,6 +659,8 @@
                 if ((rc = sort_front_rays(c, in, front_count, n_paths, &ep, &tune))) return rc;
             if (walk && d == 0)
                 walk_rays(c, in, c->d_counts + PRT_CNT_LIST, tm.n_pix_local, false, tune, trav_stats, &primary_list);
+            else if (plan.last_segment == 2u && d + 1u == max_depth && !trav_stats)
+                walk_rays(c, in, front_count, n_paths, true, tune, nullptr, nullptr, true);
             else
                 walk_rays(c, in, front_count, n_paths, false, tune, trav_stats, prim_d);
             if ((rc = end_event(c, &ep))) return rc;
@@ -675,7 +686,7 @@
         if (c->d_shade_div) prt_launch_shade_divstats(c->stream, c->dsc, in, c->d_counts, d, n_paths, c->d_shade_div, prim_d);
         if ((rc = begin_event(c, 2, &ep))) return rc;
         const PrtShadeInst shade = d == 0 ? plan.shade0 : plan.shade;
-        const PrtShadeArgs sa{&c->dsc, in, out, c->d_rad, c->d_counts, c->d_work, d, max_depth, n_paths, c->sampling, n_rays_known, prim_d,
+        const PrtShadeArgs sa{&c->dsc, in, out, c->d_rad, c->d_counts, c->d_work, d, max_depth, n_paths, c->sampling, n_rays_known, prim_d, plan.last_segment,
                               f.env ? &denv : nullptr, f.tex ? &dtex : nullptr, lit ? &lt : nullptr, (lit && f.mesh_lights) ? &mlt : nullptr,
                               lit ? &c->lb : nullptr};
         if (!prt_launch_shade(c->stream, shade, sa)) return fail(c, PRT_ERR_INVALID, "no such shade instance");
@@ -2296,6 +2307,21 @@
     return PRT_OK;
 }
 
+int prt_last_segment(PrtContext* c, uint32_t* active, uint32_t* front_rays) {
+    if (!c || !active) return PRT_ERR_INVALID;
+    *active = c->last_segment_active;
+    if (front_rays) {
+        *front_rays = 0u;
+        if (c->last_batch_depth != 0u && c->d_counts) {
+            HIPCHECK(c, hipSetDevice(c->device));
+            HIPCHECK(c, hipStreamSynchronize(c->stream));
+            HIPCHECK(c, hipMemcpy(front_rays, c->d_counts + (size_t)(c->last_batch_depth - 1u) * PRT_CNT_STRIDE, sizeof(uint32_t),
+                                  hipMemcpyDeviceToHost));
+        }
+    }
+    return PRT_OK;
+}
+
 int prt_bvh_info(PrtContext* c, PrtBvhInfo* out) {
     if (!c || !out) return PRT_ERR_INVALID;
     if (!c->has_scene) return fail(c, PRT_ERR_INVALID, "prt_set_scene has not been called");
@@ -2341,6 +2367,7 @@
     else if (n == "path_kernel" && value >= 0 && value <= 2) c->tune.path_kernel = (uint32_t)value;
     else if (n == "path_max" && value >= 1) c->tune.path_max = (uint32_t)value;
     else if (n == "sort_rays" && value >= 0 && value <= 2) c->sort_rays = (uint32_t)value;
+    else if (n == "last_segment" && value >= 0 && value <= 2) c->last_segment = (uint32_t)value;
     else if (n == "compact_primary" && (value == 0 || value == 1)) c->compact_primary = value;
     else if (n == "primary_walk" && (value == 0 || value == 1)) c->primary_walk = value;
     else if (n == "node_stride" && (value == 0 || value == 5 || value == 8)) c->node_stride = value;
diff --git a/parallelraytracing_amd/csrc/prt_kernels.h b/parallelraytracing_amd/csrc/prt_kernels.h
--- a/parallelraytracing_amd/csrc/prt_kernels.h
+++ b/parallelraytracing_amd/csrc/prt_kernels.h
@@ -189,6 +189,7 @@
 const char* prt_traverse_instance(const DevScene& sc, const PrtTravTuning& tune);
 void prt_launch_intersect(hipStream_t st, const DevScene& sc, const PrtRayBuf& in, const uint32_t* count_ptr,
                           uint32_t max_rays, int stack_depth, int variant, unsigned long long* stats);
+#define PRT_LAST_SEGMENT_FLAG 0x80000000u
 struct PrtShadeArgs {
     const DevScene* sc;
     PrtRayBuf in, out;
@@ -199,6 +200,7 @@
     PrtSampling sp;
     uint32_t n_rays_known;
     const PrtPrimary* primary;
+    uint32_t last_segment;
     const DevEnv* env;
     const DevTex* tex;
     const DevLights* lights;
@@ -239,7 +241,8 @@
 void prt_launch_scan_prims_bounded(hipStream_t st, const DevScene& sc, const PrtRayBuf& in, const uint32_t* count_ptr,
                                    uint32_t* work, uint32_t max_rays);
 void prt_launch_occluded(hipStream_t st, const DevScene& sc, const PrtRayBuf& in, const uint32_t* count_ptr, uint32_t* work,
-                         uint32_t* spill, uint32_t max_rays, uint32_t tree_depth, uint32_t stack4, const PrtTravTuning& tune);
+                         uint32_t* spill, uint32_t max_rays, uint32_t tree_depth, uint32_t stack4, const PrtTravTuning& tune,
+                         bool seeded = false);
 void prt_launch_occlusion_bytes(hipStream_t st, const DevScene& sc, uint32_t n, const PrtRayBuf& in, const float* tmax,
                                 uint8_t* out);
 void prt_launch_scatter_test(hipStream_t st, const DevScene& sc, uint32_t n, const float* in_d, const PrtHit* hits,
diff --git a/parallelraytracing_amd/csrc/prt_kernels.hip b/parallelraytracing_amd/csrc/prt_kernels.hip
--- a/parallelraytracing_amd/csrc/prt_kernels.hip
+++ b/parallelraytracing_amd/csrc/prt_kernels.hip
@@ -172,15 +172,19 @@
     return mk3(t.x, t.y, t.z);
 }
 
-template <int BUDGET, bool INST, bool ABVH, int BLOCK, bool PRE = false, bool ENV = false, bool TEX = false>
+template <int BUDGET, bool INST, bool ABVH, int BLOCK, bool PRE = false, bool ENV = false, bool TEX = false, bool LASTSEG = false>
 PRT_DEV int advance_path(const DevScene& sc, uint32_t id, f3& o, f3& d, f3& thr, uint32_t& rng, uint32_t& depth,
                          uint32_t max_depth, const PrtSampling& sp, float4* __restrict__ rad_slot, uint32_t& id0,
                          float& d2_0, float4 pre_a = float4{0.f, 0.f, 0.f, 0.f}, float4 pre_b = float4{0.f, 0.f, 0.f, 0.f},
-                         const DevEnv* env = nullptr, const DevTex* tex = nullptr) {
+                         const DevEnv* env = nullptr, const DevTex* tex = nullptr, bool last_route = false) {
 #pragma unroll
     for (int it = 0; it <= BUDGET; ++it) {
         if (id == HIT_MISS) {
             st_stream(rad_slot, path_result(thr * (ENV ? env_radiance(*env, d) : mk3(sc.sky[0], sc.sky[1], sc.sky[2])), sp.clamp, depth));
+            return 0;
+        }
+        if (LASTSEG && last_route && it == 0 && depth + 1u >= max_depth && id >= sc.n_prims) {
+            st_stream(rad_slot, path_result(thr * mk3(0.f, 0.f, 0.f), sp.clamp, depth));
             return 0;
         }
         if (it == BUDGET) {
@@ -233,7 +237,14 @@
             thr = mk3(thr.x / p, thr.y / p, thr.z / p);
         }
         ++depth;
-        if (classify_ray<ABVH, BLOCK>(sc, o, d, id0, d2_0)) return 1;
+        if (LASTSEG) {
+            const bool front = classify_ray<ABVH, BLOCK>(sc, o, d, id0, d2_0);
+            if (last_route && depth + 1u >= max_depth && id0 != HIT_MISS && sc.mat_type[sc.prims[id0].material] != 4u) {
+                st_stream(rad_slot, path_result(thr * mk3(0.f, 0.f, 0.f), sp.clamp, depth));
+                return 0;
+            }
+            if (front) return 1;
+        } else if (classify_ray<ABVH, BLOCK>(sc, o, d, id0, d2_0)) return 1;
         id = id0;
     }
     return 2;
@@ -1503,7 +1514,7 @@
     T8_HALF(w1.w, nxb, fxb, nyb, fyb, nzb, fzb)
 
 #define T8_SENTINEL 0xFFFFFFFFu
-template <int STACK_L, int WAVES, bool STATS, bool INST, bool LEAN, bool PRIM, bool PATH, bool ANY>
+template <int STACK_L, int WAVES, bool STATS, bool INST, bool LEAN, bool PRIM, bool PATH, bool ANY, bool SEEDED = false>
 __device__ __forceinline__ void traverse8_body(DevScene sc, const float4* __restrict__ ro, const float4* __restrict__ rd,
                                                uint32_t* __restrict__ hit, const float* __restrict__ hd2,
                                                const uint32_t* __restrict__ count_ptr, uint32_t* __restrict__ work,
@@ -1520,6 +1531,7 @@
     constexpr bool STEAL = LEAN && !INST;
     static_assert(!PATH || (!LEAN && !INST && !PRIM && !STATS), "the path instance is the plain one-level kernel");
     static_assert(!ANY || (!PATH && !PRIM && !STATS), "the any-hit walk reads plain ray buffers");
+    static_assert(!SEEDED || ANY, "a seeded walk is an any-hit walk");
     const uint32_t count = PATH ? pa.n_paths : *count_ptr;
     f3 pd = mk3(0.f, 0.f, 1.f), pthr = mk3(0.f, 0.f, 0.f);
     uint32_t prng = 0u, pdepth = 0u;
@@ -1856,7 +1868,7 @@
                 if (idle && qi_seq < cur_end) {
                     const uint32_t qi = (!PRIM && tune.perm) ? tune.perm[qi_seq] : qi_seq;
                     uint32_t hid = PRIM ? HIT_MISS : ld_stream(&hit[qi]);
-                    if (hid != HIT_DEAD && !(ANY && hid != HIT_MISS)) {
+                    if (hid != HIT_DEAD && !(ANY && !SEEDED && hid != HIT_MISS)) {
                         float4 O, D;
                         float hd2_0 = 0.0f;
                         if (PRIM) {
@@ -2084,10 +2096,12 @@
                     ((volatile unsigned long long*)s_key)[(STEAL && k >= 0xFFFFFF00u && k != 0xFFFFFFFFu) ? wbase + (k & 63u) : tid];
                 if (LEAN) {
                     tlimit = limit_from_d2(__uint_as_float((uint32_t)(won >> 32)), pad);
-                    if (ANY && k != 0xFFFFFFFFu &&
-                        ((volatile uint32_t*)s_slot)[(STEAL && k >= 0xFFFFFF00u) ? wbase + (k & 63u) : tid] != HIT_MISS) {
-                        gy = 0u;
-                        sp = 0;
+                    if (ANY && k != 0xFFFFFFFFu) {
+                        const uint32_t sl = ((volatile uint32_t*)s_slot)[(STEAL && k >= 0xFFFFFF00u) ? wbase + (k & 63u) : tid];
+                        if (sl != HIT_MISS && (!SEEDED || sl >= sc.n_prims)) {
+                            gy = 0u;
+                            sp = 0;
+                        }
                     }
                 } else if (won != key_best) {
                     best.d2 = __uint_as_float((uint32_t)(won >> 32));
@@ -2177,12 +2191,25 @@
                                                                           nullptr, PrtPrimary{}, PrtPathArgs{});
 }
 
+template <int STACK_L, int WAVES, bool INST, bool LEAN = false>
+__global__ void __launch_bounds__(256, WAVES) k_occluded8_seeded(DevScene sc, const float4* __restrict__ ro,
+                                                                const float4* __restrict__ rd, uint32_t* __restrict__ hit,
+                                                                const float* __restrict__ hd2,
+                                                                const uint32_t* __restrict__ count_ptr,
+                                                                uint32_t* __restrict__ work, uint32_t* __restrict__ ovf,
+                                                                PrtTravTuning tune) {
+    traverse8_body<STACK_L, WAVES, false, INST, LEAN, false, false, true, true>(sc, ro, rd, hit, hd2, count_ptr, work, ovf, tune,
+                                                                                nullptr, PrtPrimary{}, PrtPathArgs{});
+}
+
 template <int FUSE, bool SAMPLING, bool INST, bool ABVH, bool PRIM, bool ENV, bool TEX = false>
 PRT_DEV void shade_step(DevScene sc, const float4* __restrict__ ro, const float4* __restrict__ rd, const float4* __restrict__ rt,
                         const uint32_t* __restrict__ hit, float4* __restrict__ no, float4* __restrict__ nd, float4* __restrict__ nt,
                         uint32_t* __restrict__ nhit, float* __restrict__ nhd2, float4* __restrict__ rad, uint32_t* __restrict__ counts,
-                        uint32_t* __restrict__ work, uint32_t iter, uint32_t max_depth, uint32_t cap, PrtSampling sp_arg, PrtPrimary pr,
+                        uint32_t* __restrict__ work, uint32_t iter, uint32_t max_depth_arg, uint32_t cap, PrtSampling sp_arg, PrtPrimary pr,
                         const DevEnv* env, const DevTex* tex = nullptr) {
+    const bool last_route = (max_depth_arg & PRT_LAST_SEGMENT_FLAG) != 0u;
+    const uint32_t max_depth = max_depth_arg & ~PRT_LAST_SEGMENT_FLAG;
     const PrtSampling sp = SAMPLING ? sp_arg : PrtSampling{0u, 0u, 0.0f};
     const uint32_t nA = CNT_A(counts, iter), nB = CNT_B(counts, iter);
     const uint32_t count = nA + nB;
@@ -2221,7 +2248,7 @@
             d = mk3(D.x, D.y, D.z);
         }
         if (id != HIT_DEAD) {
-            const int r = advance_path<1 + FUSE, INST, ABVH, SHADE_BLOCK, PRIM, ENV, TEX>(sc, id, o, d, thr, rng, depth, max_depth, sp, &rad[pid], id0, d2_0, pre_a, pre_b, env, tex);
+            const int r = advance_path<1 + FUSE, INST, ABVH, SHADE_BLOCK, PRIM, ENV, TEX, FUSE == 0>(sc, id, o, d, thr, rng, depth, max_depth, sp, &rad[pid], id0, d2_0, pre_a, pre_b, env, tex, last_route);
             front = r == 1;
             back = r == 2;
         }
@@ -3620,7 +3647,7 @@
 }
 
 void prt_launch_occluded(hipStream_t st, const DevScene& sc, const PrtRayBuf& in, const uint32_t* count_ptr, uint32_t* work,
-                         uint32_t* spill, uint32_t max_rays, uint32_t tree_depth, uint32_t stack4, const PrtTravTuning& tune_in) {
+                         uint32_t* spill, uint32_t max_rays, uint32_t tree_depth, uint32_t stack4, const PrtTravTuning& tune_in, bool seeded) {
     if (t8_kind(sc, tune_in) == T8_NONE) {
         prt_launch_traverse(st, sc, in, count_ptr, work, spill, max_rays, tree_depth, stack4, tune_in, nullptr);
         return;
@@ -3630,9 +3657,15 @@
     const T8Launch r = t8_resolve(sc, tune_o, max_rays);
     const dim3 block(256);
     uint32_t* ovf = work + 512;
-#define PRT_LAUNCH_O(L, W, IN, LN, GRID, TUNE)                                                                       \
-    hipLaunchKernelGGL((k_occluded8_persistent<L, W, IN, LN>), dim3(GRID), block, 0, st, sc, in.o, in.d, in.hit, in.hd2,  \
-                       count_ptr, work, ovf, TUNE)
+#define PRT_LAUNCH_O(L, W, IN, LN, GRID, TUNE)                                                                                 \
+    do {                                                                                                                       \
+        if (seeded)                                                                                                            \
+            hipLaunchKernelGGL((k_occluded8_seeded<L, W, IN, LN>), dim3(GRID), block, 0, st, sc, in.o, in.d, in.hit,           \
+                               in.hd2, count_ptr, work, ovf, TUNE);                                                            \
+        else                                                                                                                   \
+            hipLaunchKernelGGL((k_occluded8_persistent<L, W, IN, LN>), dim3(GRID), block, 0, st, sc, in.o, in.d, in.hit,        \
+                               in.hd2, count_ptr, work, ovf, TUNE);                                                            \
+    } while (0)
     if (r.kind == T8_INST12_4) PRT_LAUNCH_O(12, 4, true, false, r.grid, r.tune);
     else if (r.kind == T8_WIDE11_5) PRT_LAUNCH_O(11, 5, false, false, r.grid, r.tune);
     else if (r.kind == T8_LEAN8_5) PRT_LAUNCH_O(8, 5, false, true, r.grid5, r.t5);
@@ -3708,10 +3741,12 @@
     const DevMeshLights& m = or_empty(a.mesh_lights);
     const PrtLightBufs& lb = or_empty(a.lb);
 #define PRT_SHADE_RAYS a.in.o, a.in.d, a.in.t, a.in.hit, a.out.o, a.out.d, a.out.t, a.out.hit, a.out.hd2
-#define PRT_SHADE_TAIL a.rad, a.counts, a.work, a.depth, a.max_depth, a.cap, a.sp
-#define PRT_SHADE_ARGS_PLAIN sc, PRT_SHADE_RAYS, PRT_SHADE_TAIL, pr
-#define PRT_SHADE_ARGS_ENV sc, e, PRT_SHADE_RAYS, PRT_SHADE_TAIL
-#define PRT_SHADE_ARGS_TEX sc, tex, e, PRT_SHADE_RAYS, PRT_SHADE_TAIL
+#define PRT_SHADE_TAIL_D(D) a.rad, a.counts, a.work, a.depth, D, a.cap, a.sp
+#define PRT_SHADE_TAIL PRT_SHADE_TAIL_D(a.max_depth)
+#define PRT_SHADE_TAIL_LS PRT_SHADE_TAIL_D((a.last_segment ? a.max_depth | PRT_LAST_SEGMENT_FLAG : a.max_depth))
+#define PRT_SHADE_ARGS_PLAIN sc, PRT_SHADE_RAYS, PRT_SHADE_TAIL_LS, pr
+#define PRT_SHADE_ARGS_ENV sc, e, PRT_SHADE_RAYS, PRT_SHADE_TAIL_LS
+#define PRT_SHADE_ARGS_TEX sc, tex, e, PRT_SHADE_RAYS, PRT_SHADE_TAIL_LS
 #define PRT_SHADE_ARGS_NEE sc, lt, PRT_SHADE_RAYS, lb, PRT_SHADE_TAIL
 #define PRT_SHADE_ARGS_NEE_ENV sc, lt, e, PRT_SHADE_RAYS, lb, PRT_SHADE_TAIL
 #define PRT_SHADE_ARGS_NEE_MESH sc, lt, m, PRT_SHADE_RAYS, lb, PRT_SHADE_TAIL
@@ -3732,7 +3767,9 @@
 #undef PRT_SHADE_ARGS_TEX
 #undef PRT_SHADE_ARGS_ENV
 #undef PRT_SHADE_ARGS_PLAIN
+#undef PRT_SHADE_TAIL_LS
 #undef PRT_SHADE_TAIL
+#undef PRT_SHADE_TAIL_D
 #undef PRT_SHADE_RAYS
 }
 
diff --git a/parallelraytracing_amd/csrc/prt_route.h b/parallelraytracing_amd/csrc/prt_route.h
--- a/parallelraytracing_amd/csrc/prt_route.h
+++ b/parallelraytracing_amd/csrc/prt_route.h
@@ -88,6 +88,10 @@
     bool path_gate;
     uint32_t path_kernel;
     uint32_t fuse;
+    bool mesh_emissive;
+    bool depth_ge2;
+    bool sort_rays;
+    uint32_t last_segment;
 };
 
 struct PrtRoutePlan {
@@ -100,6 +104,7 @@
     PrtRaygenInst raygen;
     PrtShadeInst shade0, shade;
     PrtAccumulateInst accumulate;
+    uint32_t last_segment;
 };
 
 inline bool prt_route_walk8(bool variant0, bool insts, bool has_bvh2) { return variant0 || insts || !has_bvh2; }
@@ -141,5 +146,8 @@
 
     if (f.film_stats || f.listed) p.accumulate = PrtAccumulateInst(PRT_INST(k_accumulate_stat, ff) + ((uint32_t)f.lit << 1 | (uint32_t)f.listed));
     else p.accumulate = f.lit ? PRT_I_k_accumulate_lit : PRT_I_k_accumulate;
+
+    const bool last_ok = !p.path && p.fuse == 0u && !f.lit && !f.mesh_emissive && f.has_nodes && p.walk8 && !f.sort_rays && f.depth_ge2;
+    p.last_segment = last_ok ? f.last_segment : 0u;
     return p;
 }
diff --git a/parallelraytracing_amd/csrc/prt_scene.cpp b/parallelraytracing_amd/csrc/prt_scene.cpp
--- a/parallelraytracing_amd/csrc/prt_scene.cpp
+++ b/parallelraytracing_amd/csrc/prt_scene.cpp
@@ -130,11 +130,17 @@
     }
     c->light_power = power;
     const uint32_t n_not_similar = c->n_emitters_unsampled;
+    c->mesh_emissive = false;
     for (uint32_t m = 0; m < s->n_meshes; ++m)
-        if (emissive(s->meshes[m].material_id)) c->n_emitters_unsampled += s->meshes[m].n_triangles;
+        if (emissive(s->meshes[m].material_id)) {
+            c->n_emitters_unsampled += s->meshes[m].n_triangles;
+            c->mesh_emissive = true;
+        }
     for (uint32_t i = 0; i < s->n_instances; ++i) {
         const PrtInstance& pi = s->instances[i];
-        if (emissive(pi.material_id) && pi.mesh < s->n_instanced_meshes) c->n_emitters_unsampled += s->instanced_meshes[pi.mesh].n_triangles;
+        if (!emissive(pi.material_id)) continue;
+        c->mesh_emissive = true;
+        if (pi.mesh < s->n_instanced_meshes) c->n_emitters_unsampled += s->instanced_meshes[pi.mesh].n_triangles;
     }
     c->ml_tris_counted = c->n_emitters_unsampled - n_not_similar;
 }
diff --git a/parallelraytracing_amd/csrc/prt_scene.h b/parallelraytracing_amd/csrc/prt_scene.h
--- a/parallelraytracing_amd/csrc/prt_scene.h
+++ b/parallelraytracing_amd/csrc/prt_scene.h
@@ -93,6 +93,7 @@
     uint32_t n_emitters_unsampled = 0;
     std::vector<double> light_power;
     uint32_t ml_tris_counted = 0;
+    bool mesh_emissive = false;
     PrtMeshLights ml;
     std::vector<uint32_t> mesh_indices;
     std::vector<uint32_t> mesh_material;
diff --git a/parallelraytracing_amd/renderer.py b/parallelraytracing_amd/renderer.py
--- a/parallelraytracing_amd/renderer.py
+++ b/parallelraytracing_amd/renderer.py
@@ -768,6 +768,11 @@
         self._check(capi.lib().prt_shade_instance(self._ctx, buf, 96))
         return buf.value.decode()
 
+    def last_segment(self):
+        active, front = C.c_uint32(0), C.c_uint32(0)
+        self._check(capi.lib().prt_last_segment(self._ctx, C.byref(active), C.byref(front)))
+        return active.value, front.value
+
     def bvh_read(self):
         b = self.bvh_info()
         nodes = np.zeros((b.n_nodes, 16), np.float32)
```

New measurement: 24070 Mrays/s, median of 6. 1.03x the previous value.
